# LiuZhu-CV/PAIF

Hardware: AMD Instinct MI355X
Metric: fused image-pairs/sec at 480x640 bs=8 per GPU (fusion-net forward) (higher is better)
Workload: dtype f16 (IEEE fp16 maps and conv weights, one fp16 MFMA per product, f32 accumulate; stems, guided filter and the last map fp32)

## Files before the change

### include/paif_hip.h

```cpp
#ifndef PAIF_HIP_H
#define PAIF_HIP_H

#include <stddef.h>
#include <stdint.h>

#ifdef __cplusplus
extern "C" {
#endif

#define PAIF_ABI_VERSION 1
#define PAIF_EINVAL (-1)
#define PAIF_ENOSUP (-2)

typedef void* paif_stream_t;

int paif_version(void);
const char* paif_last_error(void);
int paif_device_cus(void);


int paif_rgb2ycrcb_fwd(const float* rgb, float* ycc, int B, int H, int W, paif_stream_t stream);

int paif_ycrcb2rgb_fwd(const float* ycc, float* rgb, int B, int H, int W, paif_stream_t stream);

int paif_minmax_blocks(int B, int H, int W);
int paif_recompose_clamp_fwd(const float* fused, const float* ycc, float* rgb_out, float* minmax_partial,
                             int B, int H, int W, paif_stream_t stream);
int paif_fused_uint8_fwd(const float* rgb, const float* minmax_partial, int npartial, unsigned char* out, int B, int H, int W,
                         paif_stream_t stream);
int paif_minmax_normalize_fwd(const float* rgb, const float* minmax_partial, int npartial, float* out,
                              float* minmax_out, int B, int H, int W, paif_stream_t stream);


int paif_stem_fwd(const float* img, size_t img_bstride, const float* w, const float* prelu, float* feat, float* guide,
                  int B, int H, int W, paif_stream_t stream);
int paif_stem_fwd_twin(const float* img, size_t img_bstride, const float* w, const float* prelu, float* feat, float* feat_bf16,
                       float* guide, int B, int H, int W, paif_stream_t stream);
int paif_stem_fwd_twin_f16(const float* img, size_t img_bstride, const float* w, const float* prelu, float* feat, float* feat_f16,
                           float* guide, int B, int H, int W, paif_stream_t stream);
int paif_channel_residue_fwd(const float* x, float* guide, int B, int H, int W, paif_stream_t stream);

int paif_guided_filter_ab_fwd(const float* guide, const float* y, float* ab, float eps0, float eps1,
                              int B, int H, int W, paif_stream_t stream);
int paif_guided_filter_lf_fwd(const float* guide, const float* ab, float* lf, int B, int H, int W,
                              paif_stream_t stream);
int paif_guided_filter_taped_fits(int B, int H, int W);
int paif_guided_filter_taped_fwd(const float* guide, const float* y, float* mc, float* lf, float eps0, float eps1,
                                 float* workspace, int B, int H, int W, paif_stream_t stream);
size_t paif_guided_filter_fused_workspace_floats(int B, int H, int W);
int paif_guided_filter_fused_fwd(const float* guide, const float* y, float* lf, float eps0, float eps1, float* workspace,
                                 int B, int H, int W, paif_stream_t stream);
int paif_guided_filter_fused_fwd_bf16(const float* guide, const float* y, float* lf, float eps0, float eps1, float* workspace, int B,
                                      int H, int W, paif_stream_t stream);
int paif_guided_filter_fused_fwd_hf16(const float* guide, const float* y, float* hf, float eps0, float eps1, float* workspace, int B,
                                      int H, int W, paif_stream_t stream);

int paif_guided_filter_fused_fwd_hf16_y16(const float* guide, const float* y16, float* hf, float eps0, float eps1, float* workspace,
                                          int B, int H, int W, paif_stream_t stream);

typedef struct {
  const float* src[3];
  int nsrc;
  int cin;
  const float* wpk;
  int kh;
  int dil;
  int in_act;
  const float* in_prelu;
  const float* scale;
  const float* shift;
  int act;
  const float* prelu;
  float alpha;
  const float* res[3];
  float* out;
  int cout;
  float* pool_partial;
  int precision;
  float* aux_out;
  const float* in_aux;
  const float* in_scale;
  float in_alpha;
  const float* epi_aux;
  int epi_dact;
  int reverse_tiles;
  int storage;
  float* cpool;
} paif_conv_desc;
#define PAIF_ST_F32 0
#define PAIF_ST_BF16 1
#define PAIF_ST_F32_BF16 2
#define PAIF_ST_F16 3
#define PAIF_ST_F16_F32 4
#define PAIF_CONV_F32 0
#define PAIF_CONV_BF16X3 1
#define PAIF_CONV_BF16 2
#define PAIF_CONV_F16 4
#define PAIF_CONV_F16X2 5
#define PAIF_CONV_F16X3 6
#define PAIF_CONV_BF16X6 3

int paif_dwconv_fwd_bf16(const float* x, const float* w, float* out, int k, int dil, int in_relu, int B, int H, int W,
                         paif_stream_t stream);
int paif_channel_pool2_fwd_bf16(const float* ir, const float* vis, float* comp, int B, int H, int W, paif_stream_t stream);
int paif_spa_blend_fwd_bf16(const float* comp, const float* w, const float* ir, const float* vis, float* agg, int B, int H, int W,
                            paif_stream_t stream);
int paif_eca_finish_fwd_bf16(const float* o, const float* r, const float* pool_partial, const float* w1d, int k,
                             const float* prelu, float* gate, float* out, int B, int H, int W, paif_stream_t stream);
int paif_tail_fwd_bf16(const float* x, const float* w, const float* prelu, float* fused, int B, int H, int W, paif_stream_t stream);
int paif_add_fwd_bf16(const float* a, const float* b, float* out, size_t n, paif_stream_t stream);
int paif_cast_storage_fwd(const float* src, float* dst, size_t n, int mode, paif_stream_t stream);
int paif_dwconv_fwd_f16(const float* x, const float* w, float* out, int k, int dil, int in_relu, int B, int H, int W,
                        paif_stream_t stream);
int paif_channel_pool2_fwd_f16(const float* ir, const float* vis, float* comp, int B, int H, int W, paif_stream_t stream);
int paif_spa_blend_fwd_f16(const float* comp, const float* w, const float* ir, const float* vis, float* agg, int B, int H, int W,
                           paif_stream_t stream);
int paif_eca_finish_fwd_f16(const float* o, const float* r, const float* pool_partial, const float* w1d, int k,
                            const float* prelu, float* gate, float* out, int B, int H, int W, paif_stream_t stream);
int paif_tail_fwd_f16(const float* x, const float* w, const float* prelu, float* fused, int B, int H, int W, paif_stream_t stream);
int paif_eca_conv2_gated_fits(int B, int H, int W);
int paif_eca_conv2_gated_fwd_f16(const float* r, const float* wpk, const float* in_prelu, float* pool_partial, const float* w1d, int k,
                                 const float* prelu, float* gate, float* out, int B, int H, int W, paif_stream_t stream);
int paif_eca_conv2_staged_f16(const float* r, const float* wpk, const float* in_prelu, float* out, int B, int H, int W, paif_stream_t stream);
int paif_add_fwd_f16(const float* a, const float* b, float* out, size_t n, paif_stream_t stream);

int paif_conv2d_blocks(int B, int H, int W);
int paif_conv2d_fwd(const paif_conv_desc* d, int B, int H, int W, paif_stream_t stream);
int paif_conv2d_can_cpool(const paif_conv_desc* d, int B, int H, int W);
int paif_channel_pool1_fwd(const float* x, float* comp_off, int B, int H, int W, paif_stream_t stream);
int paif_channel_pool1_fwd_bf16(const float* x, float* comp_off, int B, int H, int W, paif_stream_t stream);
int paif_channel_pool1_fwd_f16(const float* x, float* comp_off, int B, int H, int W, paif_stream_t stream);
int paif_conv2d_is_persistent(const paif_conv_desc* d, int B, int H, int W);
int paif_conv2d_kernel_name(const paif_conv_desc* d, int B, int H, int W, char* buf, int buflen);
size_t paif_conv_wpk_floats(int nsrc, int cin, int kh);
int paif_pack_conv_weight(const float* w, float* wpk, int cout, int nsrc, int cin, int kh, paif_stream_t stream);
int paif_pack_conv_weight_bf16x3(const float* w, float* wpk, int cout, int nsrc, int kh, paif_stream_t stream);
int paif_pack_conv_weight_f16x2(const float* w, float* wpk, int cout, int nsrc, int kh, paif_stream_t stream);
int paif_pack_conv_weight_bf16x6(const float* w, float* wpk, int cout, int nsrc, int kh, paif_stream_t stream);
int paif_compose_dw_pw_weight(const float* dw, const float* pw, float* out, int cout, int cin, int kh, paif_stream_t stream);
int paif_compose_pw_conv_weight(const float* pw, const float* w, float* out, int cout, int cmid, int cin, int kh, paif_stream_t stream);

size_t paif_rdb_fused_wpk_floats(void);
int paif_rdb_fused_pack(const float* w1, const float* w2, const float* w3, float* wpk, int f16, paif_stream_t stream);
int paif_rdb_fused_fwd(const float* x, const float* wpk, const float* prelu, float alpha, const float* res0, const float* res1, float* out,
                       float* cpool, int f16, int reverse_tiles, int B, int H, int W, paif_stream_t stream);

int paif_stem_out_pack_floats(void);
int paif_stem_out_pack(const float* w1, const float* w2, float* wpk, paif_stream_t stream);
int paif_stem_out_fwd_bf16(const float* x, const float* wpk, const float* prelu, float* fused, int B, int H, int W, paif_stream_t stream);
int paif_stem_out_fwd_f32(const float* x, const float* wpk, const float* prelu, float* fused, int B, int H, int W, paif_stream_t stream);
int paif_stem_out_fwd_guard(const float* x, int f32in, const float* wpk, const float* prelu, float* fused, unsigned* flag, int B, int H, int W,
                            paif_stream_t stream);
int paif_pack_decomp1x1_weight_bf16x6(const float* w, float* wpk, paif_stream_t stream);
int paif_pack_decomp1x1_weight_bf16x3(const float* w, float* wpk, paif_stream_t stream);
int paif_pack_decomp1x1_hf_weight_f16x2(const float* w, float* wpk, paif_stream_t stream);
int paif_pack_decomp1x1_weight(const float* w, float* wpk, paif_stream_t stream);
int paif_bn_fold(const float* gamma, const float* beta, const float* mean, const float* var, float eps,
                 float* scale, float* shift, int C, paif_stream_t stream);

int paif_dwconv_fwd(const float* x, const float* w, float* out, int k, int dil, int in_relu,
                    int B, int H, int W, paif_stream_t stream);

int paif_channel_pool2_fwd(const float* ir, const float* vis, float* comp, int B, int H, int W, paif_stream_t stream);
int paif_spa_blend_fwd(const float* comp, const float* w, const float* ir, const float* vis, float* agg,
                       float* scale_out, int B, int H, int W, paif_stream_t stream);

int paif_eca_finish_fwd(const float* o, const float* r, const float* pool_partial, const float* w1d, int k,
                        const float* prelu, float* gate , float* out,
                        float* u_out ,
                        int B, int H, int W, paif_stream_t stream);

int paif_tail_fwd(const float* x, const float* w, const float* prelu, float* fused,
                  float* z_out ,
                  int B, int H, int W, paif_stream_t stream);

int paif_add_fwd(const float* a, const float* b, float* out, size_t n, paif_stream_t stream);



int paif_gemm_fwd(const float* A, int lda, const float* W, const float* scale, const float* shift, int act,
// ... 282 lines not shown
```

### paif_amd/_lib.py

```python
import ctypes
import os
from ctypes import POINTER, Structure, c_char_p, c_float, c_int, c_size_t, c_ulonglong, c_void_p

HERE = os.path.dirname(os.path.abspath(__file__))
LIB_PATH = os.environ.get("PAIF_LIB") or os.path.join(HERE, "lib", "libpaif_hip.so")

F = c_void_p


class ConvDesc(Structure):

    _fields_ = [
        ("src", F * 3), ("nsrc", c_int), ("cin", c_int), ("wpk", F), ("kh", c_int), ("dil", c_int),
        ("in_act", c_int), ("in_prelu", F), ("scale", F), ("shift", F), ("act", c_int), ("prelu", F),
        ("alpha", c_float), ("res", F * 3), ("out", F), ("cout", c_int), ("pool_partial", F),
        ("precision", c_int), ("aux_out", F), ("in_aux", F), ("in_scale", F), ("in_alpha", c_float), ("epi_aux", F),
        ("epi_dact", c_int), ("reverse_tiles", c_int), ("storage", c_int), ("cpool", F),
    ]


SIGNATURES = {
    "paif_version": (c_int, []),
    "paif_last_error": (c_char_p, []),
    "paif_device_cus": (c_int, []),
    "paif_rgb2ycrcb_fwd": (c_int, [F, F, c_int, c_int, c_int, F]),
    "paif_ycrcb2rgb_fwd": (c_int, [F, F, c_int, c_int, c_int, F]),
    "paif_minmax_blocks": (c_int, [c_int, c_int, c_int]),
    "paif_recompose_clamp_fwd": (c_int, [F, F, F, F, c_int, c_int, c_int, F]),
    "paif_fused_uint8_fwd": (c_int, [F, F, c_int, F, c_int, c_int, c_int, F]),
    "paif_minmax_normalize_fwd": (c_int, [F, F, c_int, F, F, c_int, c_int, c_int, F]),
    "paif_stem_fwd": (c_int, [F, c_size_t, F, F, F, F, c_int, c_int, c_int, F]),
    "paif_stem_fwd_twin": (c_int, [F, c_size_t, F, F, F, F, F, c_int, c_int, c_int, F]),
    "paif_stem_fwd_twin_f16": (c_int, [F, c_size_t, F, F, F, F, F, c_int, c_int, c_int, F]),
    "paif_channel_residue_fwd": (c_int, [F, F, c_int, c_int, c_int, F]),
    "paif_guided_filter_ab_fwd": (c_int, [F, F, F, c_float, c_float, c_int, c_int, c_int, F]),
    "paif_guided_filter_lf_fwd": (c_int, [F, F, F, c_int, c_int, c_int, F]),
    "paif_guided_filter_taped_fits": (c_int, [c_int, c_int, c_int]),
    "paif_guided_filter_taped_fwd": (c_int, [F, F, F, F, c_float, c_float, F, c_int, c_int, c_int, F]),
    "paif_guided_filter_fused_workspace_floats": (c_size_t, [c_int, c_int, c_int]),
    "paif_guided_filter_fused_fwd": (c_int, [F, F, F, c_float, c_float, F, c_int, c_int, c_int, F]),
    "paif_guided_filter_fused_fwd_bf16": (c_int, [F, F, F, c_float, c_float, F, c_int, c_int, c_int, F]),
    "paif_guided_filter_fused_fwd_hf16": (c_int, [F, F, F, c_float, c_float, F, c_int, c_int, c_int, F]),
    "paif_guided_filter_fused_fwd_hf16_y16": (c_int, [F, F, F, c_float, c_float, F, c_int, c_int, c_int, F]),
    "paif_conv2d_blocks": (c_int, [c_int, c_int, c_int]),
    "paif_conv2d_fwd": (c_int, [POINTER(ConvDesc), c_int, c_int, c_int, F]),
    "paif_conv2d_is_persistent": (c_int, [POINTER(ConvDesc), c_int, c_int, c_int]),
    "paif_conv2d_can_cpool": (c_int, [POINTER(ConvDesc), c_int, c_int, c_int]),
    "paif_rdb_fused_wpk_floats": (c_size_t, []),
    "paif_rdb_fused_pack": (c_int, [F, F, F, F, c_int, F]),
    "paif_rdb_fused_fwd": (c_int, [F, F, F, c_float, F, F, F, F, c_int, c_int, c_int, c_int, c_int, F]),
    "paif_channel_pool1_fwd": (c_int, [F, F, c_int, c_int, c_int, F]),
    "paif_channel_pool1_fwd_bf16": (c_int, [F, F, c_int, c_int, c_int, F]),
    "paif_channel_pool1_fwd_f16": (c_int, [F, F, c_int, c_int, c_int, F]),
    "paif_conv2d_kernel_name": (c_int, [POINTER(ConvDesc), c_int, c_int, c_int, c_char_p, c_int]),
    "paif_conv_wpk_floats": (c_size_t, [c_int, c_int, c_int]),
    "paif_pack_conv_weight": (c_int, [F, F, c_int, c_int, c_int, c_int, F]),
    "paif_pack_decomp1x1_weight": (c_int, [F, F, F]),
    "paif_pack_conv_weight_bf16x3": (c_int, [F, F, c_int, c_int, c_int, F]),
    "paif_pack_conv_weight_f16x2": (c_int, [F, F, c_int, c_int, c_int, F]),
    "paif_pack_conv_weight_bf16x6": (c_int, [F, F, c_int, c_int, c_int, F]),
    "paif_compose_dw_pw_weight": (c_int, [F, F, F, c_int, c_int, c_int, F]),
    "paif_compose_pw_conv_weight": (c_int, [F, F, F, c_int, c_int, c_int, c_int, F]),
    "paif_stem_out_pack_floats": (c_int, []),
    "paif_stem_out_pack": (c_int, [F, F, F, F]),
    "paif_stem_out_fwd_bf16": (c_int, [F, F, F, F, c_int, c_int, c_int, F]),
    "paif_stem_out_fwd_f32": (c_int, [F, F, F, F, c_int, c_int, c_int, F]),
    "paif_stem_out_fwd_guard": (c_int, [F, c_int, F, F, F, F, c_int, c_int, c_int, F]),
    "paif_pack_decomp1x1_weight_bf16x3": (c_int, [F, F, F]),
    "paif_pack_decomp1x1_hf_weight_f16x2": (c_int, [F, F, F]),
    "paif_pack_decomp1x1_weight_bf16x6": (c_int, [F, F, F]),
    "paif_bn_fold": (c_int, [F, F, F, F, c_float, F, F, c_int, F]),
    "paif_dwconv_fwd": (c_int, [F, F, F, c_int, c_int, c_int, c_int, c_int, c_int, F]),
    "paif_channel_pool2_fwd": (c_int, [F, F, F, c_int, c_int, c_int, F]),
    "paif_spa_blend_fwd": (c_int, [F, F, F, F, F, F, c_int, c_int, c_int, F]),
    "paif_eca_finish_fwd": (c_int, [F, F, F, F, c_int, F, F, F, F, c_int, c_int, c_int, F]),
    "paif_tail_fwd": (c_int, [F, F, F, F, F, c_int, c_int, c_int, F]),
    "paif_add_fwd": (c_int, [F, F, F, c_size_t, F]),
    "paif_gemm_fwd": (c_int, [F, c_int, F, F, F, c_int, F, c_int, F, c_int, c_int, c_int, c_int, c_int, F]),
    "paif_gemm_splitk_plan": (c_int, [c_int, c_int, c_int]),
    "paif_gemm_conv_fwd": (c_int, [F, c_int, c_int, c_int, c_int, c_int, c_int, c_int, F, F, F, c_int, F, c_int, F, c_int, c_int, c_int, c_int, F, F]),
    "paif_gemm_col2im_fwd": (c_int, [F, c_int, F, F, c_int, c_int, c_int, c_int, c_int, c_int, c_int, F]),
    "paif_timing_event_create": (c_int, [POINTER(c_void_p)]),
    "paif_timing_event_record": (c_int, [c_void_p, F]),
    "paif_timing_event_elapsed_ms": (c_int, [c_void_p, c_void_p, POINTER(c_float)]),
    "paif_timing_event_destroy": (c_int, [c_void_p]),
    "paif_gemm2_plan": (c_int, [c_int, c_int, c_int, c_int]),
    "paif_gemm2_packed_bytes": (c_size_t, [c_int, c_int, c_int]),
    "paif_gemm2_pack_weight": (c_int, [F, F, c_int, c_int, c_int, F]),
    "paif_gemm2_fwd": (c_int, [F, c_int, F, F, F, c_int, F, c_int, F, c_int, c_int, c_int, c_int, c_int, c_int, F]),
    "paif_conv2d_wgrad_workspace_floats": (c_size_t, [c_int, c_int, c_int, c_int]),
    "paif_conv2d_wgrad": (c_int, [POINTER(c_void_p), c_int, F, F, F, F, c_int, c_float, c_int, c_int, F, F, c_int, c_int, c_int, c_int, c_int, F]),
    "paif_gemm_wgrad_splits": (c_int, [c_int, c_int, c_int]),
    "paif_gemm_wgrad": (c_int, [F, c_int, F, c_int, F, F, c_int, c_int, c_int, c_int, F, c_int, F]),
    "paif_gemm_wgrad_p": (c_int, [F, c_int, F, c_int, F, F, c_int, c_int, c_int, c_int, F, c_int, c_int, c_float, F]),
    "paif_layernorm_wgrad_blocks": (c_int, [c_int]),
    "paif_layernorm_wgrad": (c_int, [F, F, F, F, F, c_int, c_int, c_float, c_int, F]),
    "paif_channel_affine_nchw_fwd": (c_int, [F, F, F, F, c_int, c_int, c_int, c_int, F]),
    "paif_image_loss_blocks": (c_int, []),
# ... 175 lines not shown
```

### paif_amd/core/model_fusion_auto.py

```python
import torch
import torch.nn as nn

from .. import ops
from ..operations_m import OPS, BasicConv, Conv2dParams, PReLUParams, _HipOp, _PackCache, grad_anchor


def RGB2YCrCb(input_im):
    ops.require_no_grad(input_im)
    return ops.rgb2ycrcb(input_im)


def YCrCb2RGB(input_im):
    ops.require_no_grad(input_im)
    return ops.ycrcb2rgb(input_im)


class MixedOp(nn.Module):

    def __init__(self, C, primitive):
        super().__init__()
        self._ops = nn.ModuleList()
        kernel = 3
        dilation = 1
        if primitive.find('attention') != -1:
            name = primitive.split('_')[0]
            kernel = int(primitive.split('_')[1])
        else:
            name = primitive.split('_')[0]
            kernel = int(primitive.split('_')[1])
            dilation = int(primitive.split('_')[2])
        self._op = OPS[name](C, kernel, dilation, False)

    def forward(self, x):
        return self._op(x)

    def forward_nhwc(self, x, res=(), tape=None, out_f32=False, cpool=None):
        if out_f32 and getattr(self._op, "takes_out_f32", False):
            return self._op.forward_nhwc(x, res, tape, out_f32=True)
        if cpool is not None and tape is None:
            if getattr(self._op, "takes_cpool", False):
                return self._op.forward_nhwc(x, res, tape, cpool=cpool)
            y = self._op.forward_nhwc(x, res, tape)
            ops.channel_pool1(y, *cpool)
            return y
        return self._op.forward_nhwc(x, res, tape)

    def backward_nhwc(self, g, t, wgrad=False, res=()):
        if res:
            return self._op.backward_nhwc(g, t, wgrad, res=res)
        return self._op.backward_nhwc(g, t, wgrad)

    @property
    def bwd_takes_res(self):
        return getattr(self._op, "bwd_takes_res", False)


class Cell_Chain(_HipOp):

    _tape_is_list = True

    def __init__(self, C, type, concat):
        super().__init__()
        op_names, indices = zip(*type)
        self._compile(C, op_names, indices, concat)

    def _compile(self, C, op_names, indices, concat):
        assert len(op_names) == len(indices)
        self._steps = len(op_names)
        self._concat = concat
        self.multiplier = len(concat)
        self._ops = nn.ModuleList()
        for name, index in zip(op_names, indices):
            self._ops += [MixedOp(C, name)]
        self._indices = indices

    def forward_nhwc(self, inp, res=(), tape=None, out_f32=False, cpool=None):
        s1 = inp
        for i in range(self._steps):
            last = i == self._steps - 1
            s1 = self._ops[i].forward_nhwc(s1, ((inp,) + tuple(res)) if last else (), tape, out_f32=out_f32 and last,
                                           cpool=cpool if last else None)
        return s1

    def backward_nhwc(self, g, tape, wgrad=False):
        d = g
        for i in range(self._steps - 1, 0, -1):
            d = self._ops[i].backward_nhwc(d, tape[i], wgrad)
        if self._ops[0].bwd_takes_res:
            return self._ops[0].backward_nhwc(d, tape[0], wgrad, res=(g,))
        return ops.add(self._ops[0].backward_nhwc(d, tape[0], wgrad), g)


class Cell_Decom(nn.Module):

    def __init__(self, C, types, concat):
        super().__init__()
        self._C = C
        self.radiux = [4]
        self.eps_list = [0.001, 0.0001]
        self._ops_1 = nn.ModuleList()
        self._ops_2 = nn.ModuleList()
        self.conv1x1_lf = Conv2dParams(C * 4, C, kernel_size=1, bias=True)
        self.conv1x1_hf = Conv2dParams(C * 4, C, kernel_size=1, bias=True)
        self._steps = len(concat)
        self.relu = PReLUParams()
        self.chain = Cell_Chain(C, types[0], concat)
        self.chain2 = Cell_Chain(C, types[1], concat)
        self._packs = _PackCache()
        if C != 32:
            raise NotImplementedError("the HIP kernels are built for C = 32 (the only width either entry script uses)")

    def get_residue(self, tensor):
        return ops.to_nchw_view(ops.channel_residue(ops.to_nhwc(tensor)).unsqueeze(-1))

    def decomposition_nhwc(self, x, guide=None, want_ab=False, out_bf16=False):
        if guide is None:
            guide = ops.channel_residue(x)
        return ops.guided_filter_pair(guide, x, tuple(self.eps_list), want_ab=want_ab, out_bf16=out_bf16)

    @staticmethod
    def _cat_lf_hf(x, lf):
        lf_cat, hf_cat = ops.decomp_cat(x, lf)
        return ops.to_nchw_view(lf_cat), ops.to_nchw_view(hf_cat)

    def decomposition(self, x, C=None):
        ops.require_no_grad(x)
        xn = ops.to_nhwc(x)
        return self._cat_lf_hf(xn, self.decomposition_nhwc(xn))

    def forward_nhwc(self, fir, fvis, g_ir=None, g_vis=None, tape=None, feats=None, comp=None):
        if g_ir is None:
            g_ir = ops.channel_residue(fir)
        if g_vis is None:
            g_vis = ops.channel_residue(fvis)
        lf16 = tape is None and feats is None and ops._ACT_BF16[0]
        if tape is None:
            lf_ir = self.decomposition_nhwc(fir, g_ir, out_bf16=lf16)
            lf_vis = self.decomposition_nhwc(fvis, g_vis, out_bf16=lf16)
        else:
            lf_ir, ab_ir = self.decomposition_nhwc(fir, g_ir, want_ab=True)
            lf_vis, ab_vis = self.decomposition_nhwc(fvis, g_vis, want_ab=True)
        pack1, pn = (ops.pack_decomp1x1_hf_weight, "_hf16") if lf16 is torch.float16 else (ops.pack_decomp1x1_weight, "")
        w_lf = self._packs.get("lf" + pn, [self.conv1x1_lf.weight], lambda: pack1(self.conv1x1_lf.weight))
        w_hf = self._packs.get("hf" + pn, [self.conv1x1_hf.weight], lambda: pack1(self.conv1x1_hf.weight))
        if feats is not None:
            feats.update(lf_ir=lf_ir, lf_vis=lf_vis, g_ir=g_ir, g_vis=g_vis)
        x_ir, x_vis = (ops.cast_storage(fir, True), ops.cast_storage(fvis, True)) if lf16 else (fir, fvis)
        lf = ops.conv2d([x_ir, lf_ir[0], lf_ir[1]], w_lf, 1, 1, shift=self.conv1x1_lf.bias)
        hf = ops.conv2d([x_vis, lf_vis[0], lf_vis[1]], w_hf, 1, 1, shift=self.conv1x1_hf.bias)
        t1 = None if tape is None else []
        t2 = None if tape is None else []
        cp = comp if tape is None else None
        ir_feature = self.chain.forward_nhwc(lf, (fir,), t1, cpool=None if cp is None else (cp, 0))
        vis_feature = self.chain2.forward_nhwc(hf, (fvis,), t2, cpool=None if cp is None else (cp, 2))
        if tape is not None:
            tape.update(fir=fir, fvis=fvis, g_ir=g_ir, g_vis=g_vis, ab_ir=ab_ir, ab_vis=ab_vis, chain=t1, chain2=t2)
            if ops.taping_wgrad():
                tape.update(lf_ir=lf_ir, lf_vis=lf_vis)
        return ir_feature, vis_feature

    def branch_nhwc(self, f, g, which, comp=None):
        lf16 = ops._ACT_BF16[0]
        lf = self.decomposition_nhwc(f, g, out_bf16=lf16)
        conv = self.conv1x1_lf if which == 0 else self.conv1x1_hf
        pack1, pn = (ops.pack_decomp1x1_hf_weight, "_hf16") if lf16 is torch.float16 else (ops.pack_decomp1x1_weight, "")
        w = self._packs.get(("lf" if which == 0 else "hf") + pn, [conv.weight], lambda: pack1(conv.weight))
        x = ops.cast_storage(f, True) if lf16 else f
        y = ops.conv2d([x, lf[0], lf[1]], w, 1, 1, shift=conv.bias)
        return (self.chain if which == 0 else self.chain2).forward_nhwc(y, (f,), None, cpool=None if comp is None else (comp, 2 * which))

    def _stream_backward(self, d_feat, chain, chain_tape, conv, name, feat, guide, ab, lf=None):
# ... 91 lines not shown


class Network_Fusion_Searched(nn.Module):

    def __init__(self, C, criterion, genotype_feature, steps=4, multiplier=3):
        super().__init__()
        self._C = C
        self._criterion = criterion
        self._steps = steps
        self._multiplier = multiplier
        self._genotype = genotype_feature
        self.stem_1 = nn.Sequential(Conv2dParams(1, C, 3, padding=1, bias=False), PReLUParams())
        self.stem_2 = nn.Sequential(Conv2dParams(1, C, 3, padding=1, bias=False), PReLUParams())
        self.stem_out = nn.Sequential(
            Conv2dParams(C, C // 2, 3, padding=1, bias=False),
            Conv2dParams(C // 2, 1, 3, padding=1, bias=False),
            PReLUParams(),
        )
        self.tanh = nn.Tanh()
        self.spa = spatial_attn_layer_M()
        self.decompation = self._decom_cls(C, [self._genotype.normal_1, self._genotype.normal_2], self._genotype.normal_1_concat)
        self.chain = Cell_Chain(C, self._genotype.normal_3, self._genotype.normal_1_concat)
        self._packs = _PackCache()

    _decom_cls = Cell_Decom

    def forward(self, ir, vis, inter=None):
        wg = ops.want_param_grads(self)
        if torch.is_grad_enabled() and (ir.requires_grad or vis.requires_grad or wg):
            return _FusionFn.apply(ir, vis, self, wg, grad_anchor(ir.device))
        want_feats = inter is not None and bool(inter.get("want_decomposition"))
        with torch.no_grad(), ops.bf16_activations(enable=not self.training and not want_feats):
            return self.forward_impl(ir, vis, inter=inter)

    def forward_impl(self, ir, vis, inter=None, tape=None):
        vis = vis[:, 0:1, :, :]
        ir = ir[:, 0:1, :, :]
        if tape is None and inter is None and ir.is_cuda and ops.CONFIG.get("two_stream", False):
            main = torch.cuda.current_stream()
            side = self.__dict__.get("_side_stream")
            if side is None or side.device != ir.device:
                side = self.__dict__["_side_stream"] = torch.cuda.Stream(device=ir.device)
            comp = self._new_comp(ir)
            side.wait_stream(main)
            with torch.cuda.stream(side):
                fvis, g_vis = ops.stem(vis, self.stem_2[0].weight, self.stem_2[1].weight)
                vis_feature = self.decompation.branch_nhwc(fvis, g_vis, 1, comp)
            fir, g_ir = ops.stem(ir, self.stem_1[0].weight, self.stem_1[1].weight)
            ir_feature = self.decompation.branch_nhwc(fir, g_ir, 0, comp)
            main.wait_stream(side)
            if not torch.cuda.is_current_stream_capturing():
                vis_feature.record_stream(main)
            del fvis, g_vis
            agg = self.spa.blend_nhwc(ir_feature, vis_feature, comp=comp)
            return self._tail_nhwc(self.chain.forward_nhwc(agg, (), None, out_f32=self._last_f32()))
        fir, g_ir = ops.stem(ir, self.stem_1[0].weight, self.stem_1[1].weight)
        fvis, g_vis = ops.stem(vis, self.stem_2[0].weight, self.stem_2[1].weight)
        t_dec = None if tape is None else {}
        feats = {} if (inter is not None and inter.get("want_decomposition")) else None
        comp = self._new_comp(ir) if tape is None else None
        ir_feature, vis_feature = self.decompation.forward_nhwc(fir, fvis, g_ir, g_vis, t_dec, feats, comp=comp)
        if feats is not None:
            inter.update(feats)
        t_chain = None if tape is None else []
        if tape is None:
            agg = self.spa.blend_nhwc(ir_feature, vis_feature, comp=comp)
        elif ops.taping_wgrad():
            agg, scale, comp = self.spa.blend_nhwc(ir_feature, vis_feature, want_scale=True, want_comp=True)
        else:
            agg, scale = self.spa.blend_nhwc(ir_feature, vis_feature, want_scale=True)
        feature2 = self.chain.forward_nhwc(agg, (), t_chain, out_f32=tape is None and self._last_f32())
        if tape is None:
            out = self._tail_nhwc(feature2)
        else:
            w0 = self._packs.get("so0", [self.stem_out[0].weight], lambda: ops.pack_conv_weight(self.stem_out[0].weight, 1, 32, 3))
            t16 = ops.conv2d([feature2], w0, 3, 1, cout=16)
            out, z = ops.tail(t16, self.stem_out[1].weight, self.stem_out[2].weight, save=True)
            tape.update(dec=t_dec, chain=t_chain, ir_feature=ir_feature, vis_feature=vis_feature, scale=scale, fused=out, z=z)
            if ops.taping_wgrad():
                tape.update(comp=comp, feature2=feature2, t16=t16, img_ir=ir, img_vis=vis)
        if inter is not None:
            inter.update(fir=fir, fvis=fvis, ir_feature=ir_feature, vis_feature=vis_feature, agg=agg, feature2=feature2)
        return out

    @staticmethod
    def _new_comp(img):
        if not ops.CONFIG.get("cpool_fused", True):
            return None
        B, _, H, W = img.shape
        return torch.empty((B, H, W, 4), device=img.device, dtype=torch.float32)

    @staticmethod
    def _last_f32():
        return ops._ACT_BF16[0] is torch.float16 and ops.CONFIG.get("f16_last_f32", True)

    def _tail_nhwc(self, feature2):
        so = self.stem_out
        if feature2.dtype == torch.float16:
            feature2 = ops.cast_storage(feature2, torch.float32)
        if feature2.dtype == torch.float32:
            fused_on = ops.CONFIG.get("stem_out_fused_f32", True) and ops.CONFIG["conv_precision"] == "bf16x3"
        else:
            fused_on = ops.CONFIG.get("stem_out_fused", True)
        if feature2.shape[1] >= 3 and feature2.shape[2] >= 3 and fused_on:
            wso = self._packs.get("so_fused", [so[0].weight, so[1].weight], lambda: ops.stem_out_pack(so[0].weight, so[1].weight))
            return ops.stem_out_fused(feature2, wso, so[2].weight)
        if ops._ACT_BF16[0] is torch.float16:
            ops.f16_guard_flag(feature2.device).bitwise_or_((~torch.isfinite(feature2).all()).to(torch.int32))
        if feature2.dtype == torch.float32:
            prec = ops.CONFIG["conv_precision"]
            w0 = self._packs.get("so0_" + prec, [so[0].weight], lambda: ops.pack_conv_weight(so[0].weight, 1, 32, 3, precision=prec))
        else:
            w0 = self._packs.get("so0", [so[0].weight], lambda: ops.pack_conv_weight(so[0].weight, 1, 32, 3))
        return ops.tail(ops.conv2d([feature2], w0, 3, 1, cout=16), so[1].weight, so[2].weight)

    def backward_impl(self, d_fused, tape, wgrad=False):
        from ..operations_m import check_positive_slope
        for prm, what in ((self.stem_1[1].weight, "stem_1"), (self.stem_2[1].weight, "stem_2")):
            check_positive_slope(prm, what)
        so = self.stem_out
        if wgrad:
            dz = ops.tail_dz(d_fused, tape["fused"], tape["z"], so[2].weight, ops.grad_of(so[2].weight))
            gw = ops.grad_of(so[1].weight)
            if gw is not None:
                ops.corr1_wgrad(dz, tape["t16"], 3, gw)
        d_t16 = ops.tail_bwd(d_fused, tape["fused"], tape["z"], so[1].weight, so[2].weight)
        if wgrad:
            gw = ops.grad_of(so[0].weight)
            if gw is not None:
                ops.conv2d_wgrad([tape["feature2"]], ops.pad_channels(d_t16, 32), 3, 1, out=gw, cout=16)
        w0t = self._packs.get("so0T", [so[0].weight], lambda: ops.pack_conv_dgrad_weight(so[0].weight, 0, 32))
        d_feat2 = ops.conv2d([d_t16], w0t, 3, 1, cin=16, cout=32)
        d_agg = self.chain.backward_nhwc(d_feat2, tape["chain"], wgrad)
        d_irf, d_visf = self.spa.blend_backward_nhwc(d_agg, tape["ir_feature"], tape["vis_feature"], tape["scale"],
                                                     tape["comp"] if wgrad else None)
        d_fir, d_fvis = self.decompation.backward_nhwc(d_irf, d_visf, tape["dec"], wgrad)
# ... 356 lines not shown
```

### paif_amd/csrc/conv_dma.h

```cpp
#pragma once
#include <hip/hip_runtime.h>

namespace paif_conv_dma {

struct Args {
  const void* src[3];
  const void* res[3];
  const void* wpk;
  const float* scale;
  const float* shift;
  const float* prelu;
  void* out;
  float alpha;
  int nsrc, nres, act, kh;
  int cout;
  int B, H, W, reverse;
  float* cpool;
  int f16;
  int dil;
  int in_relu;
  int out_f32;
};

enum Form { NONE, TILE, ONE_BY_ONE, ROWS };
Form classify(const Args& a);
bool can_cpool(const Args& a);
int launch(const Args& a, hipStream_t st);

}
```

### paif_amd/csrc/conv_dma.hip

```cpp
#include <stdint.h>
#include <stdlib.h>

#include <type_traits>

#include "conv_dma.h"
#include "conv_rows.h"

namespace paif_conv_dma {
namespace {

using namespace paif_rows;
constexpr int TW = 32, TH = 8;
#ifndef CD_PF
#define CD_PF 4
#endif
#ifndef CD_ST_AUX
#define CD_ST_AUX 2
#endif
#ifndef CD_EPI_SWAP
#define CD_EPI_SWAP 1
#endif
#ifndef CD_EPI_LINES
#define CD_EPI_LINES 1
#endif
#ifndef CD_EXP
#define CD_EXP 0
#endif
constexpr int PARK_WAVE = 2 * 32 * 32 * 4;
template <int DIL>
struct Geo {
  static constexpr int TWH = TW + 2 * DIL, THH = TH + 2 * DIL;
  static constexpr int NPIX = TWH * THH;
  static constexpr int DPW = (NPIX * 4 + 255) / 256;
  static constexpr int SLOT = 4 * DPW * 1024;
  static constexpr int PF = DIL == 1 ? CD_PF : 3;
  static constexpr int NSLOT = PF + 1;
  static constexpr int ROWB = TWH * 64;
  static constexpr int PARK_OFF = NSLOT * SLOT;
  static constexpr int lds_bytes(bool parked) { return PARK_OFF + (parked ? 4 * PARK_WAVE : 0); }
  static_assert(lds_bytes(true) <= 160 * 1024, "ring + transposition buffers exceed LDS");
  static_assert(4 * DPW * 64 >= NPIX * 4, "DMA instructions do not cover the halo tile");
  static __device__ __forceinline__ int base_row(int w) { return DIL == 1 ? 2 * w : (w >> 1) * 4 + (w & 1); }
};
constexpr int NSTORE = 4;
constexpr int VMCAP = 63;

#define CD_VMWAIT(n) ROWS_VMWAIT((n) > VMCAP ? VMCAP : (n))

template <int NSRC, int NRES, int PF, int DPW>
struct Sched {
  static constexpr int RL = 4 * NRES;
  static constexpr int smod(int x) { return ((x % NSRC) + NSRC) % NSRC; }
  static constexpr int R_STAGE = smod(1 - PF);
  static constexpr int D = (R_STAGE + PF - 1 - NSRC) / NSRC;
  static constexpr int U = D + (R_STAGE == 0 ? 2 : 1);
  static_assert(PF >= 2 && D >= 0 && U <= 4, "prefetch distance out of the range the tile loop lists");
  static constexpr int n1 = DPW * (PF - 1);
};

template <int NSRC, int NRES, int F, bool CP = false, int DIL = 1, int IA = 0>
__global__ __launch_bounds__(256, 1) void conv3x3_h16_dma(Args a, int ntiles, int tilesX, int tilesY) {
  typedef Geo<DIL> G;
  constexpr int TWH = G::TWH, NPIX = G::NPIX, DPW = G::DPW, SLOT = G::SLOT, PF = G::PF, NSLOT = G::NSLOT, ROWB = G::ROWB, PARK_OFF = G::PARK_OFF;
  typedef Sched<NSRC, NRES, PF, DPW> SC;
  constexpr bool SW = CD_EPI_SWAP && !CP && !(NRES == 3 && (NSRC == 3 || DIL == 2));
  constexpr int U = SW ? (SC::U + 1) & ~1 : SC::U, D = SC::D;
  constexpr int NACC = SW ? 2 : 1;
  __shared__ __attribute__((aligned(16))) unsigned char smem[G::lds_bytes(!SW)];
  asm volatile("" ::"v"((unsigned)(uintptr_t)(__attribute__((address_space(3))) unsigned char*)smem) : "memory");

  const int tid = threadIdx.x, l = tid & 63;
  const int w = __builtin_amdgcn_readfirstlane(tid >> 6);
  const int p = l & 31, hh = l >> 5;
  const int wb = G::base_row(w);

  const int xcd = blockIdx.x & 7, wg = blockIdx.x >> 3, nwg = gridDim.x >> 3;
  const int tpx = (ntiles + 7) >> 3;
  const int t_beg = xcd * tpx, t_end = min(ntiles, t_beg + tpx);
  const int cnt = t_beg + wg < t_end ? (t_end - t_beg - wg + nwg - 1) / nwg : 0;
  if (cnt == 0) return;
  const int H = a.H, W = a.W;
  auto pack_tile = [&](int k) -> unsigned {
    const int pos = wg + min(k, cnt - 1) * nwg;
    int t = a.reverse ? t_end - 1 - pos : t_beg + pos;
    const int tx = t % tilesX;
    t /= tilesX;
    const int ty = t % tilesY;
    return ((unsigned)(t / tilesY) << 22) | ((unsigned)ty << 11) | (unsigned)tx;
  };
  const unsigned tab0 = pack_tile(l), tab1 = pack_tile(l + 64);
  auto tile_of = [&](int k, int& b, int& y0, int& x0) -> bool {
    const bool ok = k >= 0 && k < cnt;
    const int kk = ok ? k : 0;
    const unsigned lo = __builtin_amdgcn_readlane(tab0, kk & 63), hi = __builtin_amdgcn_readlane(tab1, kk & 63);
    const unsigned pk = kk < 64 ? lo : hi;
    b = pk >> 22; y0 = ((pk >> 11) & 2047) * TH; x0 = (pk & 2047) * TW;
    return ok;
  };

  const int map_bytes = a.B * H * W * 64;
  __amdgpu_buffer_rsrc_t rs_src[NSRC];
#pragma unroll
  for (int s = 0; s < NSRC; ++s) rs_src[s] = __builtin_amdgcn_make_buffer_rsrc(const_cast<void*>(a.src[s]), 0, map_bytes, RSRC_W3);
  __amdgpu_buffer_rsrc_t rs_res[NRES > 0 ? NRES : 1];
#pragma unroll
  for (int r = 0; r < NRES; ++r) rs_res[r] = __builtin_amdgcn_make_buffer_rsrc(const_cast<void*>(a.res[r]), 0, map_bytes, RSRC_W3);
  const int opitch = a.cout * 2;
  const __amdgpu_buffer_rsrc_t rs_out = __builtin_amdgcn_make_buffer_rsrc(a.out, 0, a.B * H * W * opitch, RSRC_W3);
  const __amdgpu_buffer_rsrc_t rs_null = __builtin_amdgcn_make_buffer_rsrc(a.out, 0, 0, RSRC_W3);
  const __amdgpu_buffer_rsrc_t rs_cp = __builtin_amdgcn_make_buffer_rsrc(CP ? (void*)a.cpool : a.out, 0, CP ? a.B * H * W * 16 - 8 : 0, RSRC_W3);

  u32x4 bw[NSRC][9][2];
  {
    const __amdgpu_buffer_rsrc_t rs_w = __builtin_amdgcn_make_buffer_rsrc(const_cast<void*>(a.wpk), 0, NSRC * 9 * 2 * 2 * 1024, RSRC_W3);
#pragma unroll
    for (int s = 0; s < NSRC; ++s)
#pragma unroll
      for (int tap = 0; tap < 9; ++tap)
#pragma unroll
        for (int ks = 0; ks < 2; ++ks)
          bw[s][tap][ks] = __builtin_amdgcn_raw_buffer_load_b128(rs_w, (unsigned)l * 16u, (((s * 9 + tap) * 2 + ks) * 2) * 1024, 0);
  }
  constexpr int NEC = SW ? 16 : 8;
  float esc[NEC], esh[NEC];
#pragma unroll
  for (int j = 0; j < NEC; ++j) {
    const int c = SW ? ROWS_ACC_CHANNEL(j, hh) : 8 * (l & 3) + j;
    esc[j] = ((a.scale && c < a.cout) ? a.scale[c] : 1.f) * a.alpha;
    esh[j] = ((a.shift && c < a.cout) ? a.shift[c] : 0.f) * a.alpha;
// ... 578 lines not shown
    cur ^= 1;
  };
  auto drain = [&](auto aptag) {
    if constexpr (!SW) {
#pragma unroll
      for (int it = 0; it < 4; ++it) {
        ROWS_RD128(t[it][0], a_pr, it * 2048);
        ROWS_RD128(t[it][1], a_pr, it * 2048 + 16);
      }
      asm volatile("s_waitcnt lgkmcnt(0)"
                   : "+v"(t[0][0]), "+v"(t[0][1]), "+v"(t[1][0]), "+v"(t[1][1]), "+v"(t[2][0]), "+v"(t[2][1]), "+v"(t[3][0]), "+v"(t[3][1])::"memory");
    }
    int pb, py0, px0;
    const bool pok = tile_of(cnt - 1, pb, py0, px0);
#define CD_M(m) epi(std::integral_constant<int, m>{}, aptag, pok, pb, py0, px0);
    CD_M(0) CD_M(1) CD_M(2) CD_M(3) CD_M(4) CD_M(5) CD_M(6) CD_M(7) CD_M(8) CD_M(9) CD_M(10) CD_M(11)
    CD_M(12) CD_M(13) CD_M(14) CD_M(15) CD_M(16) CD_M(17) CD_M(18) CD_M(19) CD_M(20) CD_M(21) CD_M(22) CD_M(23)
    CD_M(24) CD_M(25) CD_M(26) CD_M(27) CD_M(28) CD_M(29) CD_M(30) CD_M(31) CD_M(32) CD_M(33) CD_M(34) CD_M(35)
#undef CD_M
  };
  typedef std::integral_constant<int, 0> T0;
  typedef std::integral_constant<int, 1> T1;
  if constexpr (SW) {
    for (int k = 0;; k += 2) {
      tile(T0{}, k);
      if (k + 1 >= cnt) { drain(T0{}); break; }
      tile(T1{}, k + 1);
      if (k + 2 >= cnt) { drain(T1{}); break; }
    }
  } else {
    for (int k = 0; k < cnt; ++k) tile(T0{}, k);
    drain(T0{});
  }
  CD_VMWAIT(0);
}

int launch_7(const Args& a, hipStream_t st) {
  const int tilesX = (a.W + TW - 1) / TW, tilesY = (a.H + TH - 1) / TH;
  if (a.f16) hipLaunchKernelGGL(conv7x7_h16_dma<2>, dim3(256), dim3(256), 0, st, a, a.B * tilesX * tilesY, tilesX, tilesY);
  else hipLaunchKernelGGL(conv7x7_h16_dma<1>, dim3(256), dim3(256), 0, st, a, a.B * tilesX * tilesY, tilesX, tilesY);
  hipError_t e = hipGetLastError();
  if (e != hipSuccess) {
    paif::set_error("conv2d(bf16 dma 7x7): launch failed: %s", hipGetErrorString(e));
    return (int)e;
  }
  return 0;
}

template <int NSRC, int NRES>
int launch_n(const Args& a, hipStream_t st) {
  const int tilesX = (a.W + TW - 1) / TW, tilesY = (a.H + TH - 1) / TH;
  if (a.cpool) {
    if constexpr (NSRC == 3 && (NRES == 1 || NRES == 3)) {
      if (a.f16) hipLaunchKernelGGL((conv3x3_h16_dma<NSRC, NRES, 2, true>), dim3(256), dim3(256), 0, st, a, a.B * tilesX * tilesY, tilesX, tilesY);
      else hipLaunchKernelGGL((conv3x3_h16_dma<NSRC, NRES, 1, true>), dim3(256), dim3(256), 0, st, a, a.B * tilesX * tilesY, tilesX, tilesY);
    } else {
      paif::set_error("conv2d(dma): the fused ChannelPool is built for 3 sources with 1 or 3 residual maps");
      return PAIF_ENOSUP;
    }
  } else if (a.f16) hipLaunchKernelGGL((conv3x3_h16_dma<NSRC, NRES, 2>), dim3(256), dim3(256), 0, st, a, a.B * tilesX * tilesY, tilesX, tilesY);
  else hipLaunchKernelGGL((conv3x3_h16_dma<NSRC, NRES, 1>), dim3(256), dim3(256), 0, st, a, a.B * tilesX * tilesY, tilesX, tilesY);
  hipError_t e = hipGetLastError();
  if (e != hipSuccess) {
    paif::set_error("conv2d(h16 dma): launch failed: %s", hipGetErrorString(e));
    return (int)e;
  }
  return 0;
}

template <int NRES, bool CP>
int launch_d2(const Args& a, hipStream_t st) {
  const int tilesX = (a.W + TW - 1) / TW, tilesY = (a.H + TH - 1) / TH;
  if (a.f16) hipLaunchKernelGGL((conv3x3_h16_dma<1, NRES, 2, CP, 2, 2>), dim3(256), dim3(256), 0, st, a, a.B * tilesX * tilesY, tilesX, tilesY);
  else hipLaunchKernelGGL((conv3x3_h16_dma<1, NRES, 1, CP, 2, 2>), dim3(256), dim3(256), 0, st, a, a.B * tilesX * tilesY, tilesX, tilesY);
  hipError_t e = hipGetLastError();
  if (e != hipSuccess) {
    paif::set_error("conv2d(h16 dma, dilation 2): launch failed: %s", hipGetErrorString(e));
    return (int)e;
  }
  return 0;
}

}

bool is_1x1(const Args& a);
int launch_1x1(const Args& a, hipStream_t st);
bool is_rows(const Args& a);
int launch_rows(const Args& a, hipStream_t st);

static bool is_tile(const Args& a) {
  static const bool on = [] {
    const char* e = getenv("PAIF_CONV_DMA");
    return !(e && e[0] == '0');
  }();
  static const bool on_d2 = [] {
    const char* e = getenv("PAIF_CONV_DMA_D2");
    return !(e && e[0] == '0');
  }();
  if (!on || a.out_f32 || !(a.alpha > 0.f)) return false;
  bool built;
  if (a.dil == 2)
    built = on_d2 && a.kh == 3 && a.cout == 32 && a.in_relu && a.nsrc == 1 && (a.nres == 1 || a.nres == 3);
  else if (a.in_relu || a.dil != 1)
    built = false;
  else if (a.kh == 3 && a.cout == 32)
    built = a.nsrc >= 1 && a.nsrc <= 3 && a.nres >= 0 && a.nres <= (a.nsrc == 1 ? 1 : 3);
  else
    built = ((a.kh == 3 && a.cout == 16) || (a.kh == 7 && a.cout == 32)) && a.nsrc == 1 && a.nres == 0;
  const long long tiles = (long long)a.B * ((a.H + TH - 1) / TH) * ((a.W + TW - 1) / TW);
  return built && tiles >= 1024 && tiles <= 128 * 256 && a.B < 1024 && a.H < 2048 * TH && a.W < 2048 * TW &&
         (long long)a.B * a.H * a.W * 64 < (1ll << 31);
}

Form classify(const Args& a) {
  if (is_1x1(a)) return ONE_BY_ONE;
  if (is_rows(a)) return ROWS;
  return is_tile(a) ? TILE : NONE;
}

bool can_cpool(const Args& a) {
  return a.kh == 3 && a.cout == 32 && (a.nres == 1 || a.nres == 3) && ((a.dil == 1 && a.nsrc == 3) || (a.dil == 2 && a.nsrc == 1));
}

int launch(const Args& a, hipStream_t st) {
  switch (classify(a)) {
    case ONE_BY_ONE: return launch_1x1(a, st);
    case ROWS: return launch_rows(a, st);
    case TILE: break;
    default:
      paif::set_error("conv2d(h16 dma): no LDS-DMA kernel is built for this descriptor and shape");
      return PAIF_ENOSUP;
  }
  if (a.cpool && !can_cpool(a)) {
    paif::set_error("conv2d(dma): no fused ChannelPool for this form");
    return PAIF_ENOSUP;
  }
  if (a.kh == 7) return launch_7(a, st);
  if (a.dil == 2) {
    if (a.nres == 1) return a.cpool ? launch_d2<1, true>(a, st) : launch_d2<1, false>(a, st);
    return a.cpool ? launch_d2<3, true>(a, st) : launch_d2<3, false>(a, st);
  }
  switch (a.nsrc * 10 + a.nres) {
    case 10: return launch_n<1, 0>(a, st);
    case 11: return launch_n<1, 1>(a, st);
    case 20: return launch_n<2, 0>(a, st);
    case 21: return launch_n<2, 1>(a, st);
    case 22: return launch_n<2, 2>(a, st);
    case 23: return launch_n<2, 3>(a, st);
    case 30: return launch_n<3, 0>(a, st);
    case 31: return launch_n<3, 1>(a, st);
    case 32: return launch_n<3, 2>(a, st);
    case 33: return launch_n<3, 3>(a, st);
    default: break;
  }
  paif::set_error("conv2d(bf16 dma): %d sources / %d residual maps not built", a.nsrc, a.nres);
  return PAIF_ENOSUP;
}

}
```

### paif_amd/csrc/conv_dma_1x1.hip

```cpp
#include <stdint.h>
#include <stdlib.h>

#include <type_traits>

#include "conv_dma.h"
#include "conv_rows.h"

namespace paif_conv_dma {
namespace {

using namespace paif_rows;

constexpr int TP = 64;
constexpr int SLOT = TP * 64;
constexpr int DPS = SLOT / 1024;
constexpr int NSLOT = 4, PF = NSLOT - 1;
constexpr int WAVE_LDS = NSLOT * SLOT + PARK;
constexpr int WAVES = 4;
constexpr int LDS_BYTES = WAVES * WAVE_LDS;
constexpr int GRID = 512;
static_assert(2 * LDS_BYTES <= 160 * 1024, "two workgroups per CU do not fit LDS");
static_assert(PF == 3, "a stage's DMA target is the same source of the next tile: PF must equal the source count");

#ifndef C1_LD_AUX
#define C1_LD_AUX 2
#endif
#ifndef C1_ST_AUX
#define C1_ST_AUX 0
#endif

template <int F>
__global__ __launch_bounds__(WAVES * 64, 2) void conv_h16_dma_1x1(Args a, int ntiles) {
  __shared__ __attribute__((aligned(16))) unsigned char smem[LDS_BYTES];
  asm volatile("" ::"v"((unsigned)(uintptr_t)(__attribute__((address_space(3))) unsigned char*)smem) : "memory");

  const int tid = threadIdx.x, l = tid & 63;
  const int w = __builtin_amdgcn_readfirstlane(tid >> 6);
  const int p = l & 31, hh = l >> 5;
  const int gw = blockIdx.x * WAVES + w, nw = gridDim.x * WAVES;
  if (gw >= ntiles) return;
  const int cnt = (ntiles - gw + nw - 1) / nw;

  const unsigned map_bytes = (unsigned)(a.B * a.H * a.W) * 64u;
  __amdgpu_buffer_rsrc_t rs_src[3];
#pragma unroll
  for (int s = 0; s < 3; ++s) rs_src[s] = __builtin_amdgcn_make_buffer_rsrc(const_cast<void*>(a.src[s]), 0, (int)map_bytes, RSRC_W3);
  const __amdgpu_buffer_rsrc_t rs_out = __builtin_amdgcn_make_buffer_rsrc(a.out, 0, (int)map_bytes, RSRC_W3);

  u32x4 bw[3][2];
  {
    const __amdgpu_buffer_rsrc_t rs_w = __builtin_amdgcn_make_buffer_rsrc(const_cast<void*>(a.wpk), 0, 3 * 2 * 2 * 1024, RSRC_W3);
#pragma unroll
    for (int s = 0; s < 3; ++s)
#pragma unroll
      for (int ks = 0; ks < 2; ++ks) bw[s][ks] = __builtin_amdgcn_raw_buffer_load_b128(rs_w, (unsigned)l * 16u, ((s * 2 + ks) * 2) * 1024, 0);
  }
  float esc[8], esh[8];
#pragma unroll
  for (int j = 0; j < 8; ++j) {
    const int c = 8 * (l & 3) + j;
    esc[j] = a.scale ? a.scale[c] : 1.f;
    esh[j] = a.shift ? a.shift[c] : 0.f;
  }
  const int act = a.act;
  const float slope = act == 1 ? *a.prelu : 0.f;
  const float alpha = a.alpha;

  const unsigned d_rel = ROWS_SWIZZLED(l >> 2, l & 3);
  const unsigned lds_w = (unsigned)(w * WAVE_LDS);
  unsigned a_rd[2];
#pragma unroll
  for (int ks = 0; ks < 2; ++ks) a_rd[ks] = lds_w + ROWS_SWIZZLED(p, 2 * ks + hh);
  const unsigned a_pw = ROWS_PARK_WR_ADDR(lds_w + NSLOT * SLOT, p, hh);
  const unsigned a_pr = ROWS_PARK_RD_ADDR(lds_w + NSLOT * SLOT, l);
  const unsigned e_lane = (unsigned)l * 16u;

  auto tile_byte = [&](int k) -> unsigned { return (unsigned)(gw + k * nw) * (unsigned)SLOT; };
  unsigned d_voff[DPS];
  auto target = [&](int k) {
    const unsigned tb = tile_byte(k);
#pragma unroll
    for (int i = 0; i < DPS; ++i) {
      const unsigned off = tb + d_rel + 1024u * i;
      d_voff[i] = (k < cnt && off < map_bytes) ? off : OOB;
    }
  };
  int cur = 0;
  auto issue = [&](auto stag, int slot) {
    constexpr int S = decltype(stag)::value;
#pragma unroll
    for (int i = 0; i < DPS; ++i) dma16<C1_LD_AUX>(rs_src[S], d_voff[i], lds_w + (unsigned)(slot * SLOT + i * 1024));
  };
// ... 37 lines not shown
      park_transpose(acc[sg], a_pw, a_pr, t);
#pragma unroll
      for (int it = 0; it < 2; ++it) {
        float ev[8];
#pragma unroll
        for (int j = 0; j < 8; ++j) {
          float v = __builtin_fmaf(__uint_as_float(t[it][j >> 2][j & 3]), esc[j], esh[j]);
          if (act == 1) v = paif::prelu_f(v, slope);
          else if (act == 2) v = fmaxf(v, 0.f);
          ev[j] = v * alpha;
        }
        const uint2 o0 = paif::f32_to_h4<F>(make_float4(ev[0], ev[1], ev[2], ev[3]));
        const uint2 o1 = paif::f32_to_h4<F>(make_float4(ev[4], ev[5], ev[6], ev[7]));
        u32x4 od = {o0.x, o0.y, o1.x, o1.y};
        const unsigned off = tb + (unsigned)(sg * 2048 + it * 1024) + e_lane;
        __builtin_amdgcn_raw_buffer_store_b128(od, rs_out, off < map_bytes ? off : OOB, 0, C1_ST_AUX);
        asm volatile("s_nop 2" : "+v"(od));
      }
    }
  };

  typedef std::integral_constant<int, 0> S0;
  typedef std::integral_constant<int, 1> S1;
  typedef std::integral_constant<int, 2> S2;
  target(0);
  issue(S0{}, 0);
  issue(S1{}, 1);
  issue(S2{}, 2);
  for (int k = 0; k < cnt; ++k) {
    target(k + 1);
    stage(S0{});
    stage(S1{});
    stage(S2{});
    finish(k);
  }
  ROWS_VMWAIT(0);
}

}

bool is_1x1(const Args& a) {
  static const bool on = [] {
    const char* e = getenv("PAIF_CONV_DMA1X1");
    const char* d = getenv("PAIF_CONV_DMA");
    return !(e && e[0] == '0') && !(d && d[0] == '0');
  }();
  return on && a.kh == 1 && a.dil == 1 && a.cout == 32 && !a.in_relu && !a.out_f32 && a.nsrc == 3 && a.nres == 0 &&
         (long long)a.B * a.H * a.W * 64 < (1ll << 31);
}

int launch_1x1(const Args& a, hipStream_t st) {
  const long long px = (long long)a.B * a.H * a.W;
  const int ntiles = (int)((px + TP - 1) / TP);
  if (a.f16) hipLaunchKernelGGL(conv_h16_dma_1x1<2>, dim3(GRID), dim3(WAVES * 64), 0, st, a, ntiles);
  else hipLaunchKernelGGL(conv_h16_dma_1x1<1>, dim3(GRID), dim3(WAVES * 64), 0, st, a, ntiles);
  hipError_t e = hipGetLastError();
  if (e != hipSuccess) {
    paif::set_error("conv2d(h16 dma 1x1): launch failed: %s", hipGetErrorString(e));
    return (int)e;
  }
  return 0;
}

}
```

### paif_amd/csrc/conv_mfma.hip

```cpp
#include <stdlib.h>

#include "conv_dma.h"
#include "paif_common.h"
#include <type_traits>

#ifndef PAIF_UB_HOOKS
#define PAIF_UB_HOOKS 3
#endif
#ifndef PAIF_UB
#define PAIF_UB 11
#endif

namespace {

typedef float f32x16 __attribute__((ext_vector_type(16)));

#ifndef PAIF_TH
#define PAIF_TH 8
#endif
constexpr int TH = PAIF_TH;
constexpr int TW = 32;
constexpr int NTHREADS = 256;
constexpr int SEGS_PER_WAVE = TH / 4;

// ... 1767 lines not shown
    if constexpr (KH == 1) switch (p.st) { PAIF_ST_CASE(2) PAIF_ST_CASE(5) default: break; }
    switch (p.st) { PAIF_ST_CASE(12) PAIF_ST_CASE(14) default: break; }
    if constexpr (KH == 1) switch (p.st) { PAIF_ST_CASE(9) default: break; }
    if constexpr (KH == 3 && DIL == 2) switch (p.st) { PAIF_ST_CASE(15) default: break; }
  }
#undef PAIF_ST_CASE
  paif::set_error("conv2d: storage %d is not built for the %dx%d dilation-%d kernel", a.st, KH, KH, DIL);
  return PAIF_ENOSUP;
}

template <ConvFamily F, int KH, int DIL>
int launch_k(const ConvPlan& p, const ConvArgs& a, hipStream_t st) {
  if constexpr (F == FAM_F32) return p.hooks ? launch_h<KH, DIL, 32, true>(a, st) : launch_h<KH, DIL, 32, false>(a, st);
  else if constexpr (F == FAM_BF16X6) return p.hooks ? launch_bf16x3_h<KH, DIL, true, 0, 3>(a, st) : launch_bf16x3_h<KH, DIL, false, 0, 3>(a, st);
  else if constexpr (F == FAM_F16X3) return p.hooks ? launch_bf16x3_h<KH, DIL, true, 0, 2, 1>(a, st) : launch_bf16x3_h<KH, DIL, false, 0, 2, 1>(a, st);
  else return launch_split<KH, DIL>(p, a, st);
}

template <ConvFamily F>
int launch_key(const ConvPlan& p, const ConvArgs& a, hipStream_t st) {
  constexpr bool WIDE_D2 = F == FAM_SPLIT || F == FAM_F32;
  switch (p.kh * 100 + p.dil * 10 + (p.cin == 32 ? 0 : 1)) {
    case 110: return launch_k<F, 1, 1>(p, a, st);
    case 310: return launch_k<F, 3, 1>(p, a, st);
    case 320: return launch_k<F, 3, 2>(p, a, st);
    case 510: return launch_k<F, 5, 1>(p, a, st);
    case 520:
      if constexpr (WIDE_D2) return launch_k<F, 5, 2>(p, a, st);
      break;
    case 710: return launch_k<F, 7, 1>(p, a, st);
    case 720:
      if constexpr (WIDE_D2) return launch_k<F, 7, 2>(p, a, st);
      break;
    case 311:
      if constexpr (F == FAM_F32) return p.hooks ? launch_h<3, 1, 16, true>(a, st) : launch_h<3, 1, 16, false>(a, st);
      break;
    default: break;
  }
  return not_built(p);
}

static int plan_launch(const ConvPlan& p, const ConvArgs& a, hipStream_t st) {
  switch (p.family) {
    case FAM_F16X3: return launch_key<FAM_F16X3>(p, a, st);
    case FAM_BF16X6: return launch_key<FAM_BF16X6>(p, a, st);
    case FAM_SPLIT:
      if (p.variant == CV_DMA || p.variant == CV_ROWS) return paif_conv_dma::launch(dma_args(a, p.kh, p.dil), st);
      return launch_key<FAM_SPLIT>(p, a, st);
    case FAM_F32: break;
  }
  return launch_key<FAM_F32>(p, a, st);
}

}

extern "C" {

int paif_conv2d_blocks(int B, int H, int W) { return B * ((H + TH - 1) / TH) * ((W + TW - 1) / TW); }

size_t paif_conv_wpk_floats(int nsrc, int cin, int kh) { return (size_t)nsrc * kh * kh * (cin / 8) * 256; }

int paif_conv2d_is_persistent(const paif_conv_desc* d, int B, int H, int W) {
  if (!d || B <= 0 || H <= 0 || W <= 0) return 0;
  return plan_conv(conv_args(d, B, H, W), d).variant == CV_WS ? 1 : 0;
}

int paif_conv2d_can_cpool(const paif_conv_desc* d, int B, int H, int W) {
  if (!d || B <= 0 || H <= 0 || W <= 0) return 0;
  return plan_conv(conv_args(d, B, H, W), d).can_cpool ? 1 : 0;
}

int paif_conv2d_kernel_name(const paif_conv_desc* d, int B, int H, int W, char* buf, int buflen) {
  PAIF_REQUIRE(d && buf && buflen > 0 && B > 0 && H > 0 && W > 0, PAIF_EINVAL, "conv2d_kernel_name: bad arguments");
  const ConvArgs a = conv_args(d, B, H, W);
  plan_name(plan_conv(a, d), a, buf, buflen);
  return 0;
}

int paif_conv2d_fwd(const paif_conv_desc* d, int B, int H, int W, paif_stream_t stream) {
  PAIF_REQUIRE(d && d->out && d->wpk, PAIF_EINVAL, "conv2d: null descriptor/out/wpk");
  PAIF_REQUIRE(d->nsrc >= 1 && d->nsrc <= 3, PAIF_EINVAL, "conv2d: nsrc=%d", d->nsrc);
  for (int s = 0; s < d->nsrc; ++s) PAIF_REQUIRE(d->src[s], PAIF_EINVAL, "conv2d: src[%d] null", s);
  PAIF_REQUIRE(d->cout == 32 || d->cout == 16, PAIF_ENOSUP, "conv2d: cout=%d", d->cout);
  PAIF_REQUIRE(B > 0 && H > 0 && W > 0, PAIF_EINVAL, "conv2d: empty shape %dx%dx%d", B, H, W);
  PAIF_REQUIRE(d->in_act != 1 || d->in_prelu, PAIF_EINVAL, "conv2d: in_act=PReLU without slope");
  PAIF_REQUIRE(d->act != 1 || d->prelu, PAIF_EINVAL, "conv2d: act=PReLU without slope");
  PAIF_REQUIRE(d->in_act >= 0 && d->in_act <= 5, PAIF_EINVAL, "conv2d: in_act=%d", d->in_act);
  PAIF_REQUIRE(!(d->in_act == 3 || d->in_act == 4) || (d->in_aux && d->nsrc == 1), PAIF_EINVAL,
               "conv2d: in_act=%d needs in_aux and a single source", d->in_act);
  PAIF_REQUIRE(d->in_act != 3 || d->in_prelu, PAIF_EINVAL, "conv2d: in_act=3 without slope");
  PAIF_REQUIRE(d->epi_dact >= 0 && d->epi_dact <= 2 && (!d->epi_dact || d->epi_aux), PAIF_EINVAL, "conv2d: epi_dact=%d", d->epi_dact);
  PAIF_REQUIRE(d->epi_dact != 1 || d->prelu, PAIF_EINVAL, "conv2d: epi_dact=PReLU without slope");
  PAIF_REQUIRE(d->storage >= 0 && d->storage <= 4, PAIF_EINVAL, "conv2d: storage=%d", d->storage);
  const bool st_bf = d->storage == PAIF_ST_BF16 || d->storage == PAIF_ST_F32_BF16, st_hf = d->storage == PAIF_ST_F16 || d->storage == PAIF_ST_F16_F32;
  PAIF_REQUIRE(!st_bf || ((d->precision == PAIF_CONV_BF16X3 || d->precision == PAIF_CONV_BF16) && d->cin == 32), PAIF_ENOSUP,
               "conv2d: bf16 storage needs the split-bf16 kernels (cin 32)");
  PAIF_REQUIRE(!st_hf || ((d->precision == PAIF_CONV_F16 || d->precision == PAIF_CONV_F16X2) && d->cin == 32), PAIF_ENOSUP,
               "conv2d: fp16 storage takes precision F16 / F16X2 (cin 32)");
  PAIF_REQUIRE(d->precision != PAIF_CONV_BF16 || st_bf, PAIF_ENOSUP, "conv2d: precision bf16 is built for bf16-stored maps only");
  PAIF_REQUIRE((d->precision != PAIF_CONV_F16 && d->precision != PAIF_CONV_F16X2) || st_hf, PAIF_ENOSUP,
               "conv2d: precision fp16 is built for fp16-stored maps only");
  PAIF_REQUIRE(d->storage != PAIF_ST_F16_F32 || d->precision == PAIF_CONV_F16, PAIF_ENOSUP, "conv2d: fp16 in / fp32 out takes plain fp16 weights");
  PAIF_REQUIRE(!d->cpool || paif_conv2d_can_cpool(d, B, H, W), PAIF_ENOSUP, "conv2d: no fused ChannelPool for this descriptor (paif_conv2d_can_cpool)");
  PAIF_REQUIRE(d->cin == 32 || d->cin == 16, PAIF_ENOSUP, "conv2d: cin=%d", d->cin);
  PAIF_REQUIRE(d->precision == PAIF_CONV_F32 || d->precision == PAIF_CONV_BF16X3 || d->precision == PAIF_CONV_BF16 ||
                   d->precision == PAIF_CONV_BF16X6 || d->precision == PAIF_CONV_F16 || d->precision == PAIF_CONV_F16X2 ||
                   d->precision == PAIF_CONV_F16X3, PAIF_EINVAL,
               "conv2d: precision=%d", d->precision);
  PAIF_REQUIRE((d->precision != PAIF_CONV_BF16X6 && d->precision != PAIF_CONV_F16X3) || d->cin == 32, PAIF_ENOSUP, "conv2d: bf16x6 / f16x3 need 32-channel sources");
  const ConvArgs a = conv_args(d, B, H, W);
  return plan_launch(plan_conv(a, d), a, paif::as_stream(stream));
}

int paif_pack_conv_weight_bf16x3(const float* w, float* wpk, int cout, int nsrc, int kh, paif_stream_t stream) {
  PAIF_REQUIRE(w && wpk, PAIF_EINVAL, "pack_conv_weight_bf16x3: null pointer");
  PAIF_REQUIRE(cout >= 1 && cout <= 32 && nsrc >= 1 && nsrc <= 3 && kh >= 1 && kh <= 7, PAIF_ENOSUP,
               "pack_conv_weight_bf16x3: cout=%d nsrc=%d kh=%d", cout, nsrc, kh);
  const int total = nsrc * kh * kh * 2048;
  hipLaunchKernelGGL(pack_weight_bf16x3_kernel, dim3((total + 255) / 256), dim3(256), 0, paif::as_stream(stream), w,
                     reinterpret_cast<unsigned short*>(wpk), cout, nsrc, kh);
  PAIF_LAUNCH_CHECK("pack_conv_weight_bf16x3");
  return 0;
}

int paif_pack_conv_weight_f16x2(const float* w, float* wpk, int cout, int nsrc, int kh, paif_stream_t stream) {
  PAIF_REQUIRE(w && wpk, PAIF_EINVAL, "pack_conv_weight_f16x2: null pointer");
  PAIF_REQUIRE(cout >= 1 && cout <= 32 && nsrc >= 1 && nsrc <= 3 && kh >= 1 && kh <= 7, PAIF_ENOSUP,
               "pack_conv_weight_f16x2: cout=%d nsrc=%d kh=%d", cout, nsrc, kh);
  const int total = nsrc * kh * kh * 2048;
  hipLaunchKernelGGL(pack_weight_f16x2_kernel, dim3((total + 255) / 256), dim3(256), 0, paif::as_stream(stream), w,
                     reinterpret_cast<unsigned short*>(wpk), cout, nsrc, kh);
  PAIF_LAUNCH_CHECK("pack_conv_weight_f16x2");
  return 0;
}

int paif_pack_decomp1x1_hf_weight_f16x2(const float* w, float* wpk, paif_stream_t stream) {
  PAIF_REQUIRE(w && wpk, PAIF_EINVAL, "pack_decomp1x1_hf_weight_f16x2: null pointer");
  hipLaunchKernelGGL(pack_decomp1x1_hf_f16x2_kernel, dim3(24), dim3(256), 0, paif::as_stream(stream), w,
                     reinterpret_cast<unsigned short*>(wpk));
  PAIF_LAUNCH_CHECK("pack_decomp1x1_hf_weight_f16x2");
  return 0;
}

int paif_pack_conv_weight_bf16x6(const float* w, float* wpk, int cout, int nsrc, int kh, paif_stream_t stream) {
  PAIF_REQUIRE(w && wpk, PAIF_EINVAL, "pack_conv_weight_bf16x6: null pointer");
  PAIF_REQUIRE(cout >= 1 && cout <= 32 && nsrc >= 1 && nsrc <= 3 && kh >= 1 && kh <= 7, PAIF_ENOSUP,
               "pack_conv_weight_bf16x6: cout=%d nsrc=%d kh=%d", cout, nsrc, kh);
  const int total = nsrc * kh * kh * 3072;
  hipLaunchKernelGGL(pack_weight_bf16x6_kernel, dim3((total + 255) / 256), dim3(256), 0, paif::as_stream(stream), w,
                     reinterpret_cast<unsigned short*>(wpk), cout, nsrc, kh);
  PAIF_LAUNCH_CHECK("pack_conv_weight_bf16x6");
  return 0;
}

int paif_compose_dw_pw_weight(const float* dw, const float* pw, float* out, int cout, int cin, int kh, paif_stream_t stream) {
  PAIF_REQUIRE(dw && pw && out && cout >= 1 && cin >= 1 && kh >= 1 && kh <= 7, PAIF_EINVAL, "compose_dw_pw_weight: bad arguments");
  const int total = cout * cin * kh * kh;
  hipLaunchKernelGGL(compose_dw_pw_kernel, dim3((total + 255) / 256), dim3(256), 0, paif::as_stream(stream), dw, pw, out, cout, cin, kh * kh);
  PAIF_LAUNCH_CHECK("compose_dw_pw_weight");
  return 0;
}

int paif_compose_pw_conv_weight(const float* pw, const float* w, float* out, int cout, int cmid, int cin, int kh, paif_stream_t stream) {
  PAIF_REQUIRE(pw && w && out && cout >= 1 && cmid >= 1 && cin >= 1 && kh >= 1 && kh <= 7, PAIF_EINVAL, "compose_pw_conv_weight: bad arguments");
// ... 51 lines not shown
```

### paif_amd/csrc/fusion_kernels.hip

```cpp
#include <stdarg.h>

#include "conv_eca_rows.h"
#include "paif_common.h"

namespace paif {
static thread_local char g_err[256] = "";
void set_error(const char* fmt, ...) {
  va_list ap;
  va_start(ap, fmt);
  vsnprintf(g_err, sizeof(g_err), fmt, ap);
  va_end(ap);
}
}

namespace {

constexpr int MAXGRID = 256 * 8;

inline int grid_for(size_t work_items, int per_block) {
  size_t g = (work_items + per_block - 1) / per_block;
  if (g > (size_t)MAXGRID) g = MAXGRID;
  if (g < 1) g = 1;
  return (int)g;
}

__global__ void rgb2ycrcb_kernel(const float* __restrict__ rgb, float* __restrict__ ycc, int B, size_t HW) {
  const size_t total = (size_t)B * HW;
  for (size_t i = (size_t)blockIdx.x * blockDim.x + threadIdx.x; i < total; i += (size_t)gridDim.x * blockDim.x) {
    const size_t b = i / HW, px = i - b * HW;
    const float* s = rgb + b * 3 * HW + px;
    const float R = s[0], G = s[HW], Bl = s[2 * HW];
    const float Y = __fadd_rn(__fadd_rn(__fmul_rn(0.299f, R), __fmul_rn(0.587f, G)), __fmul_rn(0.114f, Bl));
    const float Cr = __fadd_rn(__fmul_rn(__fsub_rn(R, Y), 0.713f), 0.5f);
    const float Cb = __fadd_rn(__fmul_rn(__fsub_rn(Bl, Y), 0.564f), 0.5f);
    float* d = ycc + b * 3 * HW + px;
    d[0] = Y; d[HW] = Cr; d[2 * HW] = Cb;
  }
}

__global__ void ycrcb2rgb_kernel(const float* __restrict__ ycc, float* __restrict__ rgb, int B, size_t HW) {
  const size_t total = (size_t)B * HW;
  for (size_t i = (size_t)blockIdx.x * blockDim.x + threadIdx.x; i < total; i += (size_t)gridDim.x * blockDim.x) {
    const size_t b = i / HW, px = i - b * HW;
    const float* s = ycc + b * 3 * HW + px;
    const float y0 = __fadd_rn(s[0], 0.0f);
    const float cr = __fadd_rn(s[HW], -0.5f);
    const float cb = __fadd_rn(s[2 * HW], -0.5f);
    float* d = rgb + b * 3 * HW + px;
    d[0] = fmaf(cb, 0.0f, fmaf(cr, 1.403f, y0 * 1.0f));
    d[HW] = fmaf(cb, -0.344f, fmaf(cr, -0.714f, y0 * 1.0f));
    d[2 * HW] = fmaf(cb, 1.773f, fmaf(cr, 0.0f, y0 * 1.0f));
  }
}

constexpr int STEM_CHUNK = 128;
#ifndef PAIF_STEM_GRID
#define PAIF_STEM_GRID 4096
#endif
constexpr int STEM_GRID = PAIF_STEM_GRID;
__global__ __launch_bounds__(256) void stem_kernel(const float* __restrict__ img, const float* __restrict__ w,
                                                   const float* __restrict__ prelu, float* __restrict__ feat,
                                                   float* __restrict__ guide, int B, int H, int W,
                                                   size_t img_bstride, int chunks, unsigned short* __restrict__ feat16, int twin_f16) {
  const int q = threadIdx.x & 7;
  float wr[4][9];
#pragma unroll
  for (int c = 0; c < 4; ++c)
#pragma unroll
    for (int k = 0; k < 9; ++k) wr[c][k] = w[(4 * q + c) * 9 + k];
  const float slope = *prelu;
  __shared__ float patch[2][3][STEM_CHUNK + 2];
  const int nitems = B * H * chunks;
  int par = 0;
  for (int item = blockIdx.x; item < nitems; item += gridDim.x, par ^= 1) {
  const int chunk = item % chunks;
  const int row = item / chunks;
  const int y = row % H, b = row / H;
  const float* base = img + (size_t)b * img_bstride;
  for (int i = threadIdx.x; i < 3 * (STEM_CHUNK + 2); i += 256) {
    const int r = i / (STEM_CHUNK + 2), c = i - r * (STEM_CHUNK + 2);
    const int yy = y + r - 1, xx = chunk * STEM_CHUNK + c - 1;
    const bool ok = yy >= 0 && yy < H && xx >= 0 && xx < W;
    const float v = base[(size_t)min(max(yy, 0), H - 1) * W + min(max(xx, 0), W - 1)];
    patch[par][r][c] = ok ? v : 0.f;
  }
  __syncthreads();
  float* frow = feat ? feat + (size_t)row * W * 32 : nullptr;
  unsigned short* frow16 = feat16 ? feat16 + (size_t)row * W * 32 : nullptr;
  float* grow = guide ? guide + (size_t)row * W : nullptr;
#pragma unroll
  for (int it = 0; it < STEM_CHUNK / 32; ++it) {
    const int xi = it * 32 + (threadIdx.x >> 3);
    const int x = chunk * STEM_CHUNK + xi;
    float v[9];
#pragma unroll
    for (int r = 0; r < 3; ++r)
#pragma unroll
      for (int c = 0; c < 3; ++c) v[r * 3 + c] = patch[par][r][xi + c];
    float o[4];
#pragma unroll
    for (int c = 0; c < 4; ++c) {
      float s = 0.f;
#pragma unroll
      for (int k = 0; k < 9; ++k) s = fmaf(v[k], wr[c][k], s);
      o[c] = paif::prelu_f(s, slope);
    }
    if (frow && x < W) paif::store_nt(frow + (size_t)x * 32 + q * 4, make_float4(o[0], o[1], o[2], o[3]));
    if (frow16 && x < W)
      *reinterpret_cast<uint2*>(frow16 + (size_t)x * 32 + q * 4) = twin_f16 ? paif::f32_to_f16x4(make_float4(o[0], o[1], o[2], o[3]))
                                                                             : paif::f32_to_bf16x4(make_float4(o[0], o[1], o[2], o[3]));
    if (grow) {
      float mx = fmaxf(fmaxf(o[0], o[1]), fmaxf(o[2], o[3]));
      float mn = fminf(fminf(o[0], o[1]), fminf(o[2], o[3]));
#pragma unroll
      for (int m = 1; m < 8; m <<= 1) {
        mx = fmaxf(mx, __shfl_xor(mx, m));
        mn = fminf(mn, __shfl_xor(mn, m));
      }
      if (q == 0 && x < W) grow[x] = mx - mn;
    }
  }
  }
}

template <int K, int DIL, int BF = 0>
__global__ __launch_bounds__(256) void dwconv_kernel(const float* __restrict__ x, const float* __restrict__ w,
                                                     float* __restrict__ out, int in_relu, int B, int H, int W) {
  constexpr int P = DIL * (K - 1) / 2;
  const int q = threadIdx.x & 7;
  float wr[4][K * K];
#pragma unroll
  for (int c = 0; c < 4; ++c)
#pragma unroll
    for (int k = 0; k < K * K; ++k) wr[c][k] = w[(4 * q + c) * K * K + k];
  const size_t npix = (size_t)B * H * W;
  for (size_t pix = (size_t)blockIdx.x * 32 + (threadIdx.x >> 3); pix < npix; pix += (size_t)gridDim.x * 32) {
    const int xx0 = (int)(pix % W);
    const size_t rowid = pix / W;
    const int yy0 = (int)(rowid % H);
    const size_t base = (rowid - yy0) * W * 32 + q * 4;
    float4 acc = make_float4(0.f, 0.f, 0.f, 0.f);
    constexpr int ROWS_IN_FLIGHT = K == 3 ? 3 : 1;
// ... 492 lines not shown
  }
}

}

extern "C" {

int paif_fused_uint8_fwd(const float* rgb, const float* minmax_partial, int npartial, unsigned char* out, int B, int H, int W,
                         paif_stream_t stream) {
  PAIF_REQUIRE(rgb && minmax_partial && out && npartial > 0 && B > 0 && H > 0 && W > 0, PAIF_EINVAL, "fused_uint8: bad arguments");
  const size_t HW = (size_t)H * W;
  hipLaunchKernelGGL(fused_uint8_kernel, dim3(grid_for((size_t)B * 3 * HW, 256)), dim3(256), 0, paif::as_stream(stream), rgb,
                     minmax_partial, npartial, out, B, HW);
  PAIF_LAUNCH_CHECK("fused_uint8");
  return 0;
}

int paif_version(void) { return PAIF_ABI_VERSION; }
const char* paif_last_error(void) { return paif::g_err; }

int paif_device_cus(void) {
  int dev = 0;
  hipDeviceProp_t prop;
  if (hipGetDevice(&dev) != hipSuccess || hipGetDeviceProperties(&prop, dev) != hipSuccess) {
    paif::set_error("device_cus: no HIP device");
    return PAIF_EINVAL;
  }
  return prop.multiProcessorCount;
}

int paif_rgb2ycrcb_fwd(const float* rgb, float* ycc, int B, int H, int W, paif_stream_t stream) {
  PAIF_REQUIRE(rgb && ycc && B > 0 && H > 0 && W > 0, PAIF_EINVAL, "rgb2ycrcb: bad arguments");
  const size_t HW = (size_t)H * W;
  hipLaunchKernelGGL(rgb2ycrcb_kernel, dim3(grid_for(B * HW, 256)), dim3(256), 0, paif::as_stream(stream), rgb, ycc, B, HW);
  PAIF_LAUNCH_CHECK("rgb2ycrcb");
  return 0;
}

int paif_ycrcb2rgb_fwd(const float* ycc, float* rgb, int B, int H, int W, paif_stream_t stream) {
  PAIF_REQUIRE(ycc && rgb && B > 0 && H > 0 && W > 0, PAIF_EINVAL, "ycrcb2rgb: bad arguments");
  const size_t HW = (size_t)H * W;
  hipLaunchKernelGGL(ycrcb2rgb_kernel, dim3(grid_for(B * HW, 256)), dim3(256), 0, paif::as_stream(stream), ycc, rgb, B, HW);
  PAIF_LAUNCH_CHECK("ycrcb2rgb");
  return 0;
}

static int stem_launch(const float* img, size_t img_bstride, const float* w, const float* prelu, float* feat, float* guide,
                       unsigned short* feat16, int twin_f16, int B, int H, int W, paif_stream_t stream) {
  PAIF_REQUIRE(img && w && prelu && (feat || feat16) && B > 0 && H > 0 && W > 0, PAIF_EINVAL, "stem: bad arguments");
  PAIF_REQUIRE(img_bstride >= (size_t)H * W, PAIF_EINVAL, "stem: batch stride %zu < H*W", img_bstride);
  const int chunks = (W + STEM_CHUNK - 1) / STEM_CHUNK;
  PAIF_REQUIRE((size_t)B * H * chunks < ((size_t)1 << 31), PAIF_EINVAL, "stem: %dx%dx%d is too large for one launch", B, H, W);
  hipLaunchKernelGGL(stem_kernel, dim3((unsigned)min(B * H * chunks, STEM_GRID)), dim3(256), 0, paif::as_stream(stream), img, w,
                     prelu, feat, guide, B, H, W, img_bstride, chunks, feat16, twin_f16);
  PAIF_LAUNCH_CHECK("stem");
  return 0;
}

int paif_stem_fwd(const float* img, size_t img_bstride, const float* w, const float* prelu, float* feat, float* guide,
                  int B, int H, int W, paif_stream_t stream) {
  return stem_launch(img, img_bstride, w, prelu, feat, guide, nullptr, 0, B, H, W, stream);
}

int paif_stem_fwd_twin(const float* img, size_t img_bstride, const float* w, const float* prelu, float* feat, float* feat_bf16,
                       float* guide, int B, int H, int W, paif_stream_t stream) {
  PAIF_REQUIRE(feat_bf16, PAIF_EINVAL, "stem_twin: null bf16 map");
  return stem_launch(img, img_bstride, w, prelu, feat, guide, reinterpret_cast<unsigned short*>(feat_bf16), 0, B, H, W, stream);
}

int paif_stem_fwd_twin_f16(const float* img, size_t img_bstride, const float* w, const float* prelu, float* feat, float* feat_f16,
                           float* guide, int B, int H, int W, paif_stream_t stream) {
  PAIF_REQUIRE(feat_f16, PAIF_EINVAL, "stem_twin: null fp16 map");
  return stem_launch(img, img_bstride, w, prelu, feat, guide, reinterpret_cast<unsigned short*>(feat_f16), 1, B, H, W, stream);
}

int paif_dwconv_fwd(const float* x, const float* w, float* out, int k, int dil, int in_relu, int B, int H, int W,
                    paif_stream_t stream) {
  PAIF_REQUIRE(x && w && out && B > 0 && H > 0 && W > 0, PAIF_EINVAL, "dwconv: bad arguments");
  const dim3 g(grid_for((size_t)B * H * W, 32)), blk(256);
  hipStream_t st = paif::as_stream(stream);
  const int key = k * 10 + dil;
  switch (key) {
    case 31: hipLaunchKernelGGL((dwconv_kernel<3, 1>), g, blk, 0, st, x, w, out, in_relu, B, H, W); break;
    case 32: hipLaunchKernelGGL((dwconv_kernel<3, 2>), g, blk, 0, st, x, w, out, in_relu, B, H, W); break;
    case 51: hipLaunchKernelGGL((dwconv_kernel<5, 1>), g, blk, 0, st, x, w, out, in_relu, B, H, W); break;
    case 52: hipLaunchKernelGGL((dwconv_kernel<5, 2>), g, blk, 0, st, x, w, out, in_relu, B, H, W); break;
    case 71: hipLaunchKernelGGL((dwconv_kernel<7, 1>), g, blk, 0, st, x, w, out, in_relu, B, H, W); break;
    case 72: hipLaunchKernelGGL((dwconv_kernel<7, 2>), g, blk, 0, st, x, w, out, in_relu, B, H, W); break;
    default:
      paif::set_error("dwconv: kernel %d dil %d not built", k, dil);
      return PAIF_ENOSUP;
  }
  PAIF_LAUNCH_CHECK("dwconv");
  return 0;
}

int paif_channel_pool2_fwd(const float* ir, const float* vis, float* comp, int B, int H, int W, paif_stream_t stream) {
  PAIF_REQUIRE(ir && vis && comp && B > 0 && H > 0 && W > 0, PAIF_EINVAL, "channel_pool2: bad arguments");
  const size_t npix = (size_t)B * H * W;
  hipLaunchKernelGGL(channel_pool2_kernel<0>, dim3(grid_for(npix, 32)), dim3(256), 0, paif::as_stream(stream), ir, vis, comp,
                     npix);
  PAIF_LAUNCH_CHECK("channel_pool2");
  return 0;
}

int paif_channel_residue_fwd(const float* x, float* guide, int B, int H, int W, paif_stream_t stream) {
  PAIF_REQUIRE(x && guide && B > 0 && H > 0 && W > 0, PAIF_EINVAL, "channel_residue: bad arguments");
  const size_t npix = (size_t)B * H * W;
// ... 266 lines not shown
```

### paif_amd/csrc/gf_mfma2.hip

```cpp
#include <stdint.h>
#include <type_traits>

#include "paif_common.h"

#ifndef GF2_NS
#define GF2_NS paif_gf2
#endif
namespace GF2_NS {

constexpr int R = 4;
#ifndef GF2_NW
#define GF2_NW 8
#endif
constexpr int NW = GF2_NW;
constexpr int SC = 8 * NW;
constexpr int SO = SC - 4 * R;
constexpr int PF = 6;
constexpr int NQ = 6;
#ifndef GF2_DP
#define GF2_DP (GF2_NW >= 12 ? 2 : 3)
#endif
#ifndef GF2_MINW
#define GF2_MINW (GF2_NW / 4)
#endif
// ... 53 lines not shown
__device__ __forceinline__ u32x2 band_operand(int m, int colbase) {
  u32x2 d = {0u, 0u};
  if ((m & 3) < 2) {
    const int oc = 2 * (m >> 2) + (m & 3);
    unsigned v = 0;
#pragma unroll
    for (int s = 0; s < 2; ++s) {
      const int col = colbase + s;
      if (oc - col <= R && col - oc <= R) v |= 0x3C00u << (16 * s);
    }
    d[0] = v; d[1] = v;
  }
  return d;
}

#ifndef GF2_PAIRED
#define GF2_PAIRED 1
#endif
#if GF2_EARLY_AB && !GF2_PAIRED
#error "GF2_EARLY_AB is written for the paired form"
#endif
typedef _Float16 half8 __attribute__((ext_vector_type(8)));
__device__ __forceinline__ u32x4 band_operand2(int m, int colbase) {
  const u32x2 d = band_operand((m & ~3) | (m & 1), colbase);
  return (m & 2) ? u32x4{0u, 0u, d[0], d[1]} : u32x4{d[0], d[1], 0u, 0u};
}
__device__ __forceinline__ f32x4 band_mfma2(u32x4 a_own, u32x4 b_own, u32x4 a_halo, u32x4 b_halo) {
  f32x4 acc = {0.f, 0.f, 0.f, 0.f};
  acc = __builtin_amdgcn_mfma_f32_16x16x32_f16(__builtin_bit_cast(half8, a_own), __builtin_bit_cast(half8, b_own), acc, 0, 0, 0);
  acc = __builtin_amdgcn_mfma_f32_16x16x32_f16(__builtin_bit_cast(half8, a_halo), __builtin_bit_cast(half8, b_halo), acc, 0, 0, 0);
  return acc;
}

struct Ring {
  f32x2 p[PF];
  f32x2 a1, a2;
};

template <int K>
__device__ __forceinline__ f32x2 ring_push(Ring& rg, f32x2 x) {
#ifdef GF2_NORING
  rg.a1 = rg.a1 + x; return rg.a1;
#endif
  const f32x2 p = (rg.a2 + rg.a1) + x;
  const f32x2 v = (p + rg.p[(K + 3) % PF]) + rg.p[K];
  rg.p[K] = p; rg.a2 = rg.a1; rg.a1 = x;
  return v;
}

template <int OM>
__global__ __launch_bounds__(64 * NW, GF2_MINW) void gf2_kernel(const float* __restrict__ guide, const float* __restrict__ y,
                                                     const float* __restrict__ planes, float* __restrict__ lf,
                                                     unsigned* __restrict__ flag, int B, int H, int W, int nstrip, int nslots,
                                                     int rows_per_slot, int total_rows) {
#if GF2_PAIRED
  __shared__ u32x4 hbuf[2][NQ / 2][NW + 2][64];
#else
  __shared__ u32x2 hbuf[2][NQ][NW + 2][64];
#endif
  __shared__ float rny_tab[MAXIT + 8];
  __shared__ float pbuf[2][5][SC];
  __shared__ float tbuf[NW][2][8][16];
  constexpr bool YDL = GF2_YD_LDS && OM >= 2;
  __shared__ f32x2 ydl[YDL ? 9 : 1][YDL ? 64 * NW : 1];

  const int tid = threadIdx.x, l = tid & 63;
  const int q = __builtin_amdgcn_readfirstlane(tid >> 6);
  const int c = l & 15, g = l >> 4;
  const int bid = blockIdx.x;
  const int chh = (bid >> 3) & 1;
  const int slot_id = (bid >> 4) * 8 + (bid & 7);
  if (slot_id >= nslots) return;
  int run_lo = slot_id * rows_per_slot;
  const int run_hi = min(total_rows, run_lo + rows_per_slot);
  const size_t npix = (size_t)B * H * W;
  const int lc0 = 8 * q + 2 * g;
  float vmax = 0.f;
#if GF2_PAIRED
  for (int i = tid; i < 2 * (NQ / 2) * 2 * 64; i += 64 * NW) {
    const int ln = i & 63, sl = (i >> 6) & 1, qq = (i >> 7) % (NQ / 2), par = i / (128 * (NQ / 2));
    hbuf[par][qq][sl ? NW + 1 : 0][ln] = u32x4{0u, 0u, 0u, 0u};
  }
#else
  for (int i = tid; i < 2 * NQ * 2 * 64; i += 64 * NW) {
    const int ln = i & 63, sl = (i >> 6) & 1, qq = (i >> 7) % NQ, par = i / (128 * NQ);
    hbuf[par][qq][sl ? NW + 1 : 0][ln] = u32x2{0u, 0u};
  }
#endif
  while (run_lo < run_hi) {
  const int sidx = run_lo / H;
  const int ybeg = run_lo - sidx * H, yend = min(H, ybeg + min(run_hi - run_lo, MAXIT - 32));
  run_lo += yend - ybeg;
  const int strip = sidx % nstrip, b = sidx / nstrip;
  const int X0 = strip * SO - 2 * R;
  const int col0 = X0 + lc0;
  const size_t img = (size_t)b * H * W;

  bool cin[2];
  float rnx[2];
#pragma unroll
  for (int i = 0; i < 2; ++i) {
    const int cc = col0 + i;
    cin[i] = cc >= 0 && cc < W;
    rnx[i] = cin[i] ? 1.0f / (float)(min(cc + R, W - 1) - max(cc - R, 0) + 1) : 0.f;
  }
  const bool outcol = lc0 >= 2 * R && lc0 < SC - 2 * R;
  constexpr bool BFO = OM != 0;
// ... 264 lines not shown
      }
#endif
    }
    vo0 += rowbytes_o;
    ++ro;
    GF2_ST(4);
    {
#ifdef GF2_NOLDS
      const u32x2 h_y = f_gy, h_gy = f_y;
#else
#if !GF2_PAIRED
      const u32x2 h_y = hbuf[par][0][rd_slot][rd_lane], h_gy = hbuf[par][1][rd_slot][rd_lane];
#endif
#endif
#if GF2_PAIRED
      const u32x4 h_yg = hbuf[par][0][rd_slot][rd_lane];
#if GF2_OWN_LDS
      const u32x4 o_yg = hbuf[par][0][q + 1][l];
#else
      const u32x4 o_yg = p_yg;
#endif
      const f32x4 s_yg = band_mfma2(a_own, o_yg, a_halo, h_yg);
      const f32x2 s_y = {s_yg[0], s_yg[1]}, s_gy = {s_yg[2], s_yg[3]};
#else
      const f32x2 s_y = band_mfma(a_own, f_y, a_halo, h_y);
      const f32x2 s_gy = band_mfma(a_own, f_gy, a_halo, h_gy);
#endif
      const f32x2 my = s_y * rn;
      const f32x2 cov = s_gy * rn - mg1 * my;
      const f32x2 A0 = cov * rd0, A1 = cov * rd1;
      wA0 = ring_push<k>(rA0, A0);
      wB0 = ring_push<k>(rB0, my - A0 * mg1);
      wA1 = ring_push<k>(rA1, A1);
      wB1 = ring_push<k>(rB1, my - A1 * mg1);
#if GF2_EARLY_AB
      const u32x2 f_a0 = split2(wA0, vmax), f_b0 = split2(wB0, vmax);
      hbuf[par ^ 1][1][q + 1][l] = u32x4{f_a0[0], f_a0[1], f_b0[0], f_b0[1]};
      const u32x2 f_a1 = split2(wA1, vmax), f_b1 = split2(wB1, vmax);
      hbuf[par ^ 1][2][q + 1][l] = u32x4{f_a1[0], f_a1[1], f_b1[0], f_b1[1]};
#endif
    }
    GF2_ST(5);
  };
  static_assert(PF == 6 && PF % DP == 0 && PF % DPL == 0, "the unrolled body lists PF = 6 steps");
  for (int itb = 0; itb < n_it; itb += PF) {
    step(std::integral_constant<int, 0>{}, itb);
    step(std::integral_constant<int, 1>{}, itb);
    step(std::integral_constant<int, 2>{}, itb);
    step(std::integral_constant<int, 3>{}, itb);
    step(std::integral_constant<int, 4>{}, itb);
    step(std::integral_constant<int, 5>{}, itb);
  }
  __syncthreads();
  }

#pragma unroll
  for (int m = 32; m >= 1; m >>= 1) vmax = fmaxf(vmax, __shfl_xor(vmax, m));
  if (l == 0 && !(vmax < 65000.f)) atomicOr(flag, 1u);
}

extern const int kStripOut = SO, kThreads = 64 * NW;

#if GF2_NW < 12
template __global__ void gf2_kernel<0>(const float*, const float*, const float*, float*, unsigned*, int, int, int, int, int, int, int);
template __global__ void gf2_kernel<1>(const float*, const float*, const float*, float*, unsigned*, int, int, int, int, int, int, int);
#endif
template __global__ void gf2_kernel<2>(const float*, const float*, const float*, float*, unsigned*, int, int, int, int, int, int, int);
template __global__ void gf2_kernel<3>(const float*, const float*, const float*, float*, unsigned*, int, int, int, int, int, int, int);

}
```

### paif_amd/csrc/guided_filter.hip

```cpp
#include <stdlib.h>
#include <string.h>

#include "paif_common.h"

namespace {

constexpr int R = 4;
constexpr int K = 2 * R + 1;
constexpr int NCOL = 32;
constexpr int OCOL = NCOL - 2 * R;
constexpr int ROWS_PER_SEG = 60;

__device__ __forceinline__ float4 f4add(float4 a, float4 b) { return make_float4(a.x + b.x, a.y + b.y, a.z + b.z, a.w + b.w); }
__device__ __forceinline__ float4 f4fma(float s, float4 a, float4 c) {
  return make_float4(fmaf(s, a.x, c.x), fmaf(s, a.y, c.y), fmaf(s, a.z, c.z), fmaf(s, a.w, c.w));
}

__global__ __launch_bounds__(256) void gf_ab_kernel(const float* __restrict__ guide, const float* __restrict__ y,
                                                    float* __restrict__ ab, float eps0, float eps1, int B, int H, int W,
                                                    int nstrip, int nseg) {
  __shared__ float4 sy[2][NCOL][8];
  __shared__ float4 sgy[2][NCOL][8];
  __shared__ float2 sg[2][NCOL];
  const int q = threadIdx.x & 7, xi = threadIdx.x >> 3;
// ... 135 lines not shown
        *reinterpret_cast<float4*>(out + px * 32 + q * 4) =
            make_float4(fmaf(ba.x / n, g, bb.x / n), fmaf(ba.y / n, g, bb.y / n), fmaf(ba.z / n, g, bb.z / n),
                        fmaf(ba.w / n, g, bb.w / n));
      }
    }
  }
}

}

extern "C" {

int paif_guided_filter_ab_fwd(const float* guide, const float* y, float* ab, float eps0, float eps1, int B, int H, int W,
                              paif_stream_t stream) {
  PAIF_REQUIRE(guide && y && ab && B > 0, PAIF_EINVAL, "guided_filter_ab: bad arguments");
  PAIF_REQUIRE(H > 2 * R + 1 && W > 2 * R + 1, PAIF_EINVAL, "guided_filter: H,W must exceed 2r+1 = %d (got %dx%d)", K, H, W);
  const int nstrip = (W + OCOL - 1) / OCOL, nseg = (H + ROWS_PER_SEG - 1) / ROWS_PER_SEG;
  hipLaunchKernelGGL(gf_ab_kernel, dim3(B * nstrip * nseg), dim3(256), 0, paif::as_stream(stream), guide, y, ab, eps0, eps1,
                     B, H, W, nstrip, nseg);
  PAIF_LAUNCH_CHECK("guided_filter_ab");
  return 0;
}

int paif_guided_filter_lf_fwd(const float* guide, const float* ab, float* lf, int B, int H, int W, paif_stream_t stream) {
  PAIF_REQUIRE(guide && ab && lf && B > 0, PAIF_EINVAL, "guided_filter_lf: bad arguments");
  PAIF_REQUIRE(H > 2 * R + 1 && W > 2 * R + 1, PAIF_EINVAL, "guided_filter: H,W must exceed 2r+1 = %d (got %dx%d)", K, H, W);
  const int nstrip = (W + OCOL - 1) / OCOL, nseg = (H + ROWS_PER_SEG - 1) / ROWS_PER_SEG;
  hipLaunchKernelGGL(gf_lf_kernel, dim3(B * nstrip * nseg, 2), dim3(256), 0, paif::as_stream(stream), guide, ab, lf, B, H,
                     W, nstrip, nseg);
  PAIF_LAUNCH_CHECK("guided_filter_lf");
  return 0;
}

}

namespace {

constexpr int FC = 64;
constexpr int FO = FC - 4 * R;
constexpr int PF = 3;

__device__ __forceinline__ void lds_barrier() {
  asm volatile("s_waitcnt lgkmcnt(0)" ::: "memory");
  __builtin_amdgcn_s_barrier();
  asm volatile("" ::: "memory");
}

constexpr int GT = 32, GH = GT + 2 * R;
__global__ __launch_bounds__(256) void gf_guide_stats_kernel(const float* __restrict__ guide, float* __restrict__ gs, unsigned* __restrict__ flag,
                                                             float eps0, float eps1, int B, int H, int W, int tilesX, int tilesY) {
  __shared__ float sG[GH][GH + 1];
  __shared__ float sH[GH][GT + 1], sH2[GH][GT + 1];
  int t = blockIdx.x;
  if (t == 0 && threadIdx.x == 0) *flag = 0u;
  const int tx = t % tilesX; t /= tilesX;
  const int ty = t % tilesY;
  const int b = t / tilesY;
  const int x0 = tx * GT - R, y0 = ty * GT - R;
  const float* base = guide + (size_t)b * H * W;
  for (int i = threadIdx.x; i < GH * GH; i += 256) {
    const int r = i / GH, c = i - r * GH;
    const int gy = y0 + r, gx = x0 + c;
    const float v = base[(size_t)min(max(gy, 0), H - 1) * W + min(max(gx, 0), W - 1)];
    sG[r][c] = (gy >= 0 && gy < H && gx >= 0 && gx < W) ? v : 0.f;
  }
  __syncthreads();
  for (int i = threadIdx.x; i < GH * GT; i += 256) {
    const int r = i / GT, c = i - r * GT;
    float s = 0.f, ss = 0.f;
#pragma unroll
    for (int j = 0; j < K; ++j) { const float g = sG[r][c + j]; s += g; ss = fmaf(g, g, ss); }
    sH[r][c] = s; sH2[r][c] = ss;
  }
  __syncthreads();
  const size_t npix = (size_t)B * H * W;
  for (int i = threadIdx.x; i < GT * GT; i += 256) {
    const int r = i / GT, c = i - r * GT;
    const int yy = ty * GT + r, xx = tx * GT + c;
    if (yy >= H || xx >= W) continue;
    float s = 0.f, ss = 0.f;
#pragma unroll
    for (int j = 0; j < K; ++j) { s += sH[r + j][c]; ss += sH2[r + j][c]; }
    const int cy = min(yy + R, H - 1) - max(yy - R, 0) + 1;
    const int cx = min(xx + R, W - 1) - max(xx - R, 0) + 1;
    const float rn = 1.0f / (float)(cy * cx);
    const float mg = s * rn;
    const float var = ss * rn - mg * mg;
    const size_t pix = (size_t)b * H * W + (size_t)yy * W + xx;
    gs[pix] = mg;
    gs[npix + pix] = 1.0f / (var + eps0);
    gs[2 * npix + pix] = 1.0f / (var + eps1);
    gs[3 * npix + pix] = rn;
  }
}

template <typename V> struct VecOps;
template <> struct VecOps<float4> {
  static constexpr int VW = 4;
  static __device__ __forceinline__ float4 zero() { return make_float4(0.f, 0.f, 0.f, 0.f); }
};
template <> struct VecOps<float2> {
  static constexpr int VW = 2;
  static __device__ __forceinline__ float2 zero() { return make_float2(0.f, 0.f); }
};
template <typename V> __device__ __forceinline__ V vadd(V a, V b) {
  V r; float* pr = reinterpret_cast<float*>(&r); const float* pa = reinterpret_cast<const float*>(&a); const float* pb = reinterpret_cast<const float*>(&b);
#pragma unroll
  for (int i = 0; i < VecOps<V>::VW; ++i) pr[i] = pa[i] + pb[i];
  return r;
}
template <typename V> __device__ __forceinline__ V vfma(float s, V a, V c) {
  V r; float* pr = reinterpret_cast<float*>(&r); const float* pa = reinterpret_cast<const float*>(&a); const float* pc = reinterpret_cast<const float*>(&c);
#pragma unroll
  for (int i = 0; i < VecOps<V>::VW; ++i) pr[i] = fmaf(s, pa[i], pc[i]);
  return r;
}

template <typename V, int NL>
__global__ __launch_bounds__(FC * NL) void gf_fused_kernel(const float* __restrict__ guide, const float* __restrict__ y,
                                                           const float* __restrict__ gs, const unsigned* __restrict__ only_if, float* __restrict__ lf,
                                                           int B, int H, int W, int nstrip, int nseg, int frows, int out_bf16) {
  constexpr int VW = VecOps<V>::VW;
  const bool y_f16 = out_bf16 == 3;
  if (y_f16) out_bf16 = 2;
  const unsigned short* const y16 = reinterpret_cast<const unsigned short*>(y) + (blockIdx.z * NL + threadIdx.x % NL) * VW;
  unsigned short* const lf16 = reinterpret_cast<unsigned short*>(lf);
  if (only_if != nullptr && *only_if == 0u) return;
  __shared__ V s_a[2][FC][NL];
  __shared__ V s_b[2][FC][NL];
  const int xi = threadIdx.x / NL;
  const int ql = threadIdx.x - xi * NL;
  y += (blockIdx.z * NL + ql) * VW;
  lf += (blockIdx.z * NL + ql) * VW;
  auto ldy = [&](size_t px) -> V {
    if (y_f16) {
      V r;
      float* pr = reinterpret_cast<float*>(&r);
#pragma unroll
      for (int i = 0; i < VW; ++i) pr[i] = (float)__builtin_bit_cast(_Float16, y16[px * 32 + i]);
      return r;
    }
    return *reinterpret_cast<const V*>(y + px * 32);
  };
  int t = blockIdx.x;
  const int strip = t % nstrip; t /= nstrip;
  const int seg = t % nseg;
  const int b = t / nseg;
  const int e = blockIdx.y;
  const int col = strip * FO - 2 * R + xi;
  const bool colin = col >= 0 && col < W;
  const int ybeg = seg * frows, yend = min(H, ybeg + frows);
  const size_t img = (size_t)b * H * W;
  float* out = lf + (size_t)e * ((size_t)B * H * W * 32);
  unsigned short* out16 = lf16 + (blockIdx.z * NL + ql) * VW + (size_t)e * ((size_t)B * H * W * 32);
  const float* gmean = gs;
  const float* grden = gs + (size_t)(1 + e) * ((size_t)B * H * W);

  const int cx = min(col + R, W - 1) - max(col - R, 0) + 1;
  float rnt[R + 1];
#pragma unroll
  for (int i = 0; i <= R; ++i) rnt[i] = 1.0f / (float)((K - i) * max(cx, 1));
  auto rn_of = [&](int row) -> float {
    const int miss = K - (min(row + R, H - 1) - max(row - R, 0) + 1);
    float r = rnt[0];
#pragma unroll
    for (int i = 1; i <= R; ++i) r = miss == i ? rnt[i] : r;
    return r;
  };

  V ry[K], tA[K], tB[K];
  float rg[K];
  V a1 = VecOps<V>::zero(), a2 = a1, b1 = a1, b2 = a1;
#pragma unroll
  for (int k = 0; k < K; ++k) { tA[k] = VecOps<V>::zero(); tB[k] = tA[k]; }
  const int r0 = ybeg - 2 * R, r1 = yend + 2 * R;
  const int colc = min(max(col, 0), W - 1);
  V pv[PF];
  float pg[PF];
  float2 ps[PF];
#pragma unroll
// ... 51 lines not shown
        for (int i = 0; i < VW; ++i) {
          const float my = pby[i] * rn;
          pA[i] = (pbgy[i] * rn - mg * my) * rden;
          pB[i] = my - pA[i] * mg;
        }
      }
      tA[k] = vadd(vadd(a2, a1), A);
      tB[k] = vadd(vadd(b2, b1), Bc);
      a2 = a1; a1 = A; b2 = b1; b1 = Bc;
      const int orow = irow - R;
      if (orow < ybeg) { lds_barrier(); continue; }
      {
        s_a[1][xi][ql] = vadd(vadd(tA[k], tA[(k + 6) % K]), tA[(k + 3) % K]);
        s_b[1][xi][ql] = vadd(vadd(tB[k], tB[(k + 6) % K]), tB[(k + 3) % K]);
      }
      lds_barrier();
      if (xi >= 2 * R && xi < FC - 2 * R && col < W) {
        V ba = VecOps<V>::zero(), bb = ba;
#pragma unroll
        for (int j = -R; j <= R; ++j) {
          ba = vadd(ba, s_a[1][xi + j][ql]);
          bb = vadd(bb, s_b[1][xi + j][ql]);
        }
        const float rn = rn_of(orow);
        const size_t px = img + (size_t)orow * W + col;
        const float g0 = rg[(k + 1) % K];
        V o;
        float* po = reinterpret_cast<float*>(&o);
        const float* pa = reinterpret_cast<const float*>(&ba);
        const float* pb = reinterpret_cast<const float*>(&bb);
#pragma unroll
        for (int i = 0; i < VW; ++i) po[i] = fmaf(pa[i] * rn, g0, pb[i] * rn);
        if (out_bf16 == 2) {
          const V yv = ldy(px);
          const float* py_ = reinterpret_cast<const float*>(&yv);
#pragma unroll
          for (int i = 0; i < VW; ++i) out16[px * 32 + i] = __builtin_bit_cast(unsigned short, (_Float16)(py_[i] - po[i]));
        } else if (out_bf16) {
#pragma unroll
          for (int i = 0; i < VW; ++i) out16[px * 32 + i] = __builtin_bit_cast(unsigned short, (__bf16)po[i]);
        } else {
          paif::store_nt(out + px * 32, o);
        }
      }
    }
  }
}

}

namespace paif_gf2 {
template <int OM>
__global__ void gf2_kernel(const float* __restrict__ guide, const float* __restrict__ y, const float* __restrict__ planes, float* __restrict__ lf,
                           unsigned* __restrict__ flag, int B, int H, int W, int nstrip, int nslots, int rows_per_slot, int total_rows);
extern const int kStripOut, kThreads;
extern template __global__ void gf2_kernel<0>(const float*, const float*, const float*, float*, unsigned*, int, int, int, int, int, int, int);
extern template __global__ void gf2_kernel<1>(const float*, const float*, const float*, float*, unsigned*, int, int, int, int, int, int, int);
extern template __global__ void gf2_kernel<2>(const float*, const float*, const float*, float*, unsigned*, int, int, int, int, int, int, int);
extern template __global__ void gf2_kernel<3>(const float*, const float*, const float*, float*, unsigned*, int, int, int, int, int, int, int);
}
namespace paif_gf2w12 {
template <int OM>
__global__ void gf2_kernel(const float* __restrict__ guide, const float* __restrict__ y, const float* __restrict__ planes, float* __restrict__ lf,
                           unsigned* __restrict__ flag, int B, int H, int W, int nstrip, int nslots, int rows_per_slot, int total_rows);
extern const int kStripOut, kThreads;
extern template __global__ void gf2_kernel<2>(const float*, const float*, const float*, float*, unsigned*, int, int, int, int, int, int, int);
extern template __global__ void gf2_kernel<3>(const float*, const float*, const float*, float*, unsigned*, int, int, int, int, int, int, int);
}

extern "C" __attribute__((visibility("hidden"))) int paifi_gf_guide_stats(const float* guide, float* workspace, float eps0, float eps1, int B,
                                                                          int H, int W, paif_stream_t stream) {
  const size_t npix = (size_t)B * H * W;
  const int gtx = (W + GT - 1) / GT, gty = (H + GT - 1) / GT;
  hipLaunchKernelGGL(gf_guide_stats_kernel, dim3(B * gtx * gty), dim3(256), 0, paif::as_stream(stream), guide, workspace,
                     reinterpret_cast<unsigned*>(workspace + 4 * npix), eps0, eps1, B, H, W, gtx, gty);
  PAIF_LAUNCH_CHECK("guided_filter(stats)");
  return 0;
}

extern "C" size_t paif_guided_filter_fused_workspace_floats(int B, int H, int W) { return (size_t)4 * B * H * W + 64; }

static int gf_fused_launch(const float* guide, const float* y, float* lf, float eps0, float eps1, float* workspace, int B, int H, int W,
                           int out_bf16, paif_stream_t stream) {
  PAIF_REQUIRE(guide && y && lf && workspace && B > 0, PAIF_EINVAL, "guided_filter_fused: bad arguments");
  PAIF_REQUIRE(H > 2 * R + 1 && W > 2 * R + 1, PAIF_EINVAL, "guided_filter: H,W must exceed 2r+1 = %d (got %dx%d)", K, H, W);
  const int nstrip = (W + FO - 1) / FO;
  const char* eng = getenv("PAIF_GF_ENGINE");
  PAIF_REQUIRE(!(eng && !strcmp(eng, "mfma")), PAIF_ENOSUP,
               "guided_filter: the round-3 matrix-core engine (PAIF_GF_ENGINE=mfma) left the library in round 6 (tools/parked/gf_mfma.hip)");
  int engine = (eng && !strcmp(eng, "valu")) ? 0 : 2;
  const char* nwe = getenv("PAIF_GF_NW");
  PAIF_REQUIRE(!nwe || !strcmp(nwe, "8") || !strcmp(nwe, "12"), PAIF_EINVAL, "PAIF_GF_NW must be 8 or 12 (got '%s')", nwe);
  const bool w12 = out_bf16 >= 2 && !(nwe && !strcmp(nwe, "8"));
  const int strip_out = w12 ? paif_gf2w12::kStripOut : paif_gf2::kStripOut, threads2 = w12 ? paif_gf2w12::kThreads : paif_gf2::kThreads;
  const int nstrip2 = (W + strip_out - 1) / strip_out;
  if (engine == 2 && ((size_t)(B + 1) * H * W * 128 >= 0x7FF00000ull || (size_t)B * nstrip2 * H >= 0x7FFFFFFFull)) engine = 0;
  static const int form = [] {
    const char* e = getenv("PAIF_GF_FORM");
    if (!e) return 0;
    return !strcmp(e, "4x4") ? 1 : !strcmp(e, "4x2") ? 2 : !strcmp(e, "2x16") ? 3 : 0;
  }();
  const int zgroups = form == 0 ? 1 : form == 1 ? 2 : form == 2 ? 4 : 1;
  const int resident = form == 0 ? 1 : form == 1 ? 2 : form == 2 ? 4 : 1;
  hipStream_t st = paif::as_stream(stream);
  const size_t npix = (size_t)B * H * W;
  unsigned* flag = reinterpret_cast<unsigned*>(workspace + 4 * npix);
  const int gtx = (W + GT - 1) / GT, gty = (H + GT - 1) / GT;
  hipLaunchKernelGGL(gf_guide_stats_kernel, dim3(B * gtx * gty), dim3(256), 0, st, guide, workspace, flag, eps0, eps1, B, H, W, gtx, gty);
  PAIF_LAUNCH_CHECK("guided_filter_fused(stats)");
  auto pick = [&](int warm, int res, int zg, int& nseg) {
    long best = -1;
    nseg = 1;
    for (int n = 1; n <= 16 && n <= H; ++n) {
      const int rows = (H + n - 1) / n;
      const long blocks = (long)B * nstrip * n * 2 * zg;
      const long cost = ((blocks + 256 * res - 1) / (256 * res)) * (rows + warm);
      if (best < 0 || cost < best) { best = cost; nseg = n; }
    }
  };
  if (engine == 2) {
    static const int cus = [] {
      int dev = 0, n = 256;
      if (hipGetDevice(&dev) == hipSuccess) (void)hipDeviceGetAttribute(&n, hipDeviceAttributeMultiprocessorCount, dev);
      return n > 1 ? n : 2;
    }();
    const long total_rows = (long)B * nstrip2 * H;
    int nslots = (int)(total_rows / 96);
    nslots = nslots < 1 ? 1 : (nslots > cus / 2 ? cus / 2 : nslots);
    const int rows_per_slot = (int)((total_rows + nslots - 1) / nslots);
    const int grid = (nslots + 7) / 8 * 16;
    if (w12 && out_bf16 == 3)
      hipLaunchKernelGGL((paif_gf2w12::gf2_kernel<3>), dim3(grid), dim3(threads2), 0, st, guide, y, workspace, lf, flag, B, H, W, nstrip2, nslots,
                         rows_per_slot, (int)total_rows);
    else if (w12)
      hipLaunchKernelGGL((paif_gf2w12::gf2_kernel<2>), dim3(grid), dim3(threads2), 0, st, guide, y, workspace, lf, flag, B, H, W, nstrip2, nslots,
                         rows_per_slot, (int)total_rows);
    else if (out_bf16 == 3)
      hipLaunchKernelGGL((paif_gf2::gf2_kernel<3>), dim3(grid), dim3(threads2), 0, st, guide, y, workspace, lf, flag, B, H, W, nstrip2, nslots,
                         rows_per_slot, (int)total_rows);
    else if (out_bf16 == 2)
      hipLaunchKernelGGL((paif_gf2::gf2_kernel<2>), dim3(grid), dim3(threads2), 0, st, guide, y, workspace, lf, flag, B, H, W, nstrip2, nslots,
                         rows_per_slot, (int)total_rows);
    else if (out_bf16)
      hipLaunchKernelGGL((paif_gf2::gf2_kernel<1>), dim3(grid), dim3(threads2), 0, st, guide, y, workspace, lf, flag, B, H, W, nstrip2, nslots,
                         rows_per_slot, (int)total_rows);
    else
      hipLaunchKernelGGL((paif_gf2::gf2_kernel<0>), dim3(grid), dim3(threads2), 0, st, guide, y, workspace, lf, flag, B, H, W, nstrip2, nslots,
                         rows_per_slot, (int)total_rows);
    PAIF_LAUNCH_CHECK("guided_filter_fused(mfma2)");
  }
  int nseg;
  pick(4 * R, resident, zgroups, nseg);
  const int frows = (H + nseg - 1) / nseg;
  const unsigned* only_if = engine == 2 ? flag : nullptr;
  const dim3 grid(B * nstrip * nseg, 2, zgroups);
  if (form == 0) hipLaunchKernelGGL((gf_fused_kernel<float4, 8>), grid, dim3(FC * 8), 0, st, guide, y, workspace, only_if, lf, B, H, W, nstrip, nseg, frows, out_bf16);
  else if (form == 1) hipLaunchKernelGGL((gf_fused_kernel<float4, 4>), grid, dim3(FC * 4), 0, st, guide, y, workspace, only_if, lf, B, H, W, nstrip, nseg, frows, out_bf16);
  else if (form == 2) hipLaunchKernelGGL((gf_fused_kernel<float4, 2>), grid, dim3(FC * 2), 0, st, guide, y, workspace, only_if, lf, B, H, W, nstrip, nseg, frows, out_bf16);
  else hipLaunchKernelGGL((gf_fused_kernel<float2, 16>), grid, dim3(FC * 16), 0, st, guide, y, workspace, only_if, lf, B, H, W, nstrip, nseg, frows, out_bf16);
  PAIF_LAUNCH_CHECK("guided_filter_fused");
  return 0;
}

extern "C" int paif_guided_filter_fused_fwd(const float* guide, const float* y, float* lf, float eps0, float eps1, float* workspace, int B,
                                            int H, int W, paif_stream_t stream) {
  return gf_fused_launch(guide, y, lf, eps0, eps1, workspace, B, H, W, 0, stream);
}

extern "C" int paif_guided_filter_fused_fwd_hf16(const float* guide, const float* y, float* hf, float eps0, float eps1, float* workspace, int B,
                                                 int H, int W, paif_stream_t stream) {
  return gf_fused_launch(guide, y, hf, eps0, eps1, workspace, B, H, W, 2, stream);
}

extern "C" int paif_guided_filter_fused_fwd_hf16_y16(const float* guide, const float* y16, float* hf, float eps0, float eps1, float* workspace,
                                                     int B, int H, int W, paif_stream_t stream) {
  return gf_fused_launch(guide, y16, hf, eps0, eps1, workspace, B, H, W, 3, stream);
}

extern "C" int paif_guided_filter_fused_fwd_bf16(const float* guide, const float* y, float* lf, float eps0, float eps1, float* workspace, int B,
                                                 int H, int W, paif_stream_t stream) {
  return gf_fused_launch(guide, y, lf, eps0, eps1, workspace, B, H, W, 1, stream);
}
```

### paif_amd/operations_m.py

```python
import torch
import torch.nn as nn

from . import ops


class _NeverCalled:
    def forward(self, *a, **k):
        raise RuntimeError("%s is a parameter holder; the HIP path must be used" % type(self).__name__)


class Conv2dParams(_NeverCalled, nn.Conv2d):
    pass


class Conv1dParams(_NeverCalled, nn.Conv1d):
    pass


class BatchNormParams(_NeverCalled, nn.BatchNorm2d):
    pass


class PReLUParams(_NeverCalled, nn.PReLU):
    pass
# ... 132 lines not shown
            return self._add_res(y, res)
        if self.groups != 1:
            raise NotImplementedError("grouped BasicConv other than depthwise")
        if C not in (32, 64, 96) or self.conv.out_channels != 32:
            raise NotImplementedError("BasicConv %d->%d: the HIP conv is built for 32-channel NAS cells" % (C, self.conv.out_channels))
        nsrc = C // 32
        srcs = [x] if nsrc == 1 else [x[..., 32 * i:32 * (i + 1)].contiguous() for i in range(nsrc)]
        scale = shift = None
        if self.bn is not None:
            scale, shift = _bn_scale_shift(self.bn, self._packs)
        act, slope = (ops.ACT_PRELU, self.relu.weight) if self.relu is not None else (ops.ACT_NONE, None)
        return ops.conv2d(srcs, self.wpk(nsrc, 32), self.kernel_size, self.dilation, scale=scale, shift=shift, act=act,
                          prelu=slope, res=res)


def conv3x3(in_planes, out_planes, stride=1):
    return Conv2dParams(in_planes, out_planes, kernel_size=3, stride=stride, padding=1, bias=False)


class ResidualDenseBlock(_HipOp):

    def __init__(self, in_channels, kernel_size, dialtions=1, bias=False):
        super().__init__()
        self.k, self.d = kernel_size, dialtions
        self.conv1 = BasicConv(in_channels, in_channels, kernel_size, dilation=dialtions, relu=False)
        self.conv2 = BasicConv(in_channels * 2, in_channels, kernel_size, dilation=dialtions, relu=False)
        self.conv3 = BasicConv(in_channels * 3, in_channels, kernel_size, dilation=dialtions, relu=False)
        self.lrelu = PReLUParams()

    takes_cpool = True

    def forward_nhwc(self, x, res=(), tape=None, cpool=None):
        a = self.lrelu.weight
        k, d = self.k, self.d
        kw = dict(act=ops.ACT_PRELU, prelu=a)
        if tape is not None and ops.taping_wgrad():
            x1, z1 = ops.conv2d([x], self.conv1.wpk(1, 32), k, d, want_aux=True, **kw)
            x2, z2 = ops.conv2d([x, x1], self.conv2.wpk(2, 32), k, d, want_aux=True, **kw)
            out, z3 = ops.conv2d([x, x1, x2], self.conv3.wpk(3, 32), k, d, alpha=0.333333, res=(x,) + tuple(res), want_aux=True, **kw)
            tape.append(dict(x=x, x1=x1, x2=x2, z1=z1, z2=z2, z3=z3))
            return out
        if (tape is None and x.dtype in ops.H16 and k == 3 and d == 1 and len(res) <= 2 and ops.CONFIG.get("rdb_fused", False)
                and x.shape[0] * ((x.shape[1] + 7) // 8) * ((x.shape[2] + 27) // 28) >= 512):
            ws = [self.conv1.conv.weight, self.conv2.conv.weight, self.conv3.conv.weight]
            wpk = self._packs.get("rdb_" + str(x.dtype), ws, lambda: ops.rdb_fused_pack(ws[0], ws[1], ws[2], x.dtype))
            return ops.rdb_fused(x, wpk, a, alpha=0.333333, res=tuple(res), cpool=cpool)
        x1 = ops.conv2d([x], self.conv1.wpk(1, 32), k, d, **kw)
        x2 = ops.conv2d([x, x1], self.conv2.wpk(2, 32), k, d, **kw)
        if tape is None:
            return ops.conv2d([x, x1, x2], self.conv3.wpk(3, 32), k, d, alpha=0.333333, res=(x,) + tuple(res), cpool=cpool, **kw)
        out, z3 = ops.conv2d([x, x1, x2], self.conv3.wpk(3, 32), k, d, alpha=0.333333, res=(x,) + tuple(res), want_aux=True, **kw)
        tape.append(dict(x1=x1, x2=x2, z3=z3))
        return out

    bwd_takes_res = True

    def backward_nhwc(self, g, t, wgrad=False, res=()):
        a = self.lrelu.weight
        k, d = self.k, self.d
        w1, w2, w3 = self.conv1.conv.weight, self.conv2.conv.weight, self.conv3.conv.weight
        s1, s2 = t.get("z1"), t.get("z2")
        if s1 is None:
            check_positive_slope(a, "ResidualDenseBlock")
            s1, s2 = t["x1"], t["x2"]
        ds = ops.grad_of(a) if wgrad else None
        t3 = ops.prelu_bwd(g, t["z3"], a, ds, want_dx=True, factor=0.333333)
        d_x = ops.conv2d([t3], self._dgrad_w("c3s0", w3, 0), k, d, alpha=0.333333, res=(g,))
        d_x1 = ops.conv2d([t3], self._dgrad_w("c3s1", w3, 32), k, d, alpha=0.333333)
        d_x2 = ops.conv2d([t3], self._dgrad_w("c3s2", w3, 64), k, d, alpha=0.333333)
        t2 = ops.prelu_bwd(d_x2, s2, a, ds, want_dx=True)
        d_x = ops.conv2d([t2], self._dgrad_w("c2s0", w2, 0), k, d, res=(d_x,))
        d_x1 = ops.conv2d([t2], self._dgrad_w("c2s1", w2, 32), k, d, res=(d_x1,))
        if wgrad:
            x, x1, x2 = t["x"], t["x1"], t["x2"]
            for w, srcs, dout, z, alpha in ((w3, [x, x1, x2], g, t["z3"], 0.333333), (w2, [x, x1], d_x2, t["z2"], 1.0),
                                            (w1, [x], d_x1, t["z1"], 1.0)):
                gw = ops.grad_of(w)
                if gw is not None:
                    ops.conv2d_wgrad(srcs, dout, k, d, z=z, act=ops.ACT_PRELU, prelu=a, alpha=alpha, out=gw)
            if ds is not None:
                ops.prelu_bwd(d_x1, t["z1"], a, ds, factor=1.0)
        return ops.conv2d([d_x1], self._dgrad_w("c1", w1, 0), k, d, res=(d_x,) + tuple(res), in_act=ops.IN_DPRELU, in_aux=s1, in_prelu=a)


class ResidualModule(_HipOp):

    def __init__(self, in_channels, kernel_size, dialtions=1, bias=False):
        super().__init__()
        self.k, self.d = kernel_size, dialtions
        self.op = nn.Sequential(
            BasicConv(in_channels, in_channels, kernel_size, dilation=dialtions, relu=False),
            Conv2dParams(in_channels, in_channels, kernel_size=3, stride=1, padding=2, dilation=2, bias=False),
            Conv2dParams(in_channels, in_channels, kernel_size=1, padding=0, bias=False),
            BatchNormParams(in_channels),
            PReLUParams(),
        )

    takes_out_f32 = True

    def forward_nhwc(self, x, res=(), tape=None, out_f32=False):
        op = self.op
        t1 = ops.conv2d([x], op[0].wpk(1, 32), self.k, self.d)
        if tape is None and not op[3].training and ops.CONFIG.get("resmod_compose", True):
            wc = self._packs.get("w23", [op[1].weight, op[2].weight],
                                 lambda: ops.pack_conv_weight(ops.compose_pw_conv_weight(op[2].weight, op[1].weight), 1, 32, 3))
            scale, shift = _bn_scale_shift(op[3], self._packs)
# ... 362 lines not shown
```

### paif_amd/ops.py

```python
import ctypes
import weakref
import os

import torch

from . import _lib

ACT_NONE, ACT_PRELU, ACT_RELU = 0, 1, 2
ACT_GELU = 1

def _env_switch(name, default="1"):
    v = os.environ.get(name, default)
    if v not in ("0", "1", "gemm"):
        raise ValueError("%s=%r: expected 0, 1 or gemm" % (name, v))
    return {"0": False, "1": True, "gemm": "gemm"}[v]


GEMM_PRECISIONS = ("f32", "bf16x3", "auto", "bf16x6", "auto6", "f16x3", "auto6h")


def _env_gemm_precision():
    v = os.environ.get("PAIF_GEMM_PRECISION", "auto")
    if v not in GEMM_PRECISIONS:
        raise ValueError("PAIF_GEMM_PRECISION=%r: expected one of %s" % (v, GEMM_PRECISIONS))
    return v


CONFIG = {"conv_precision": "bf16x3", "gemm_precision": _env_gemm_precision(), "serpentine": True, "attack_precision": "bf16x6", "storage": "f32",
          "two_stream": False,
          "cpool_fused": True, "f16_last_f32": True, "f16_decomp_split": False,
          "gf_in_f16": os.environ.get("PAIF_GF_IN_F16", "0") == "1",
          "rdb_fused": False, "gemm2": False, "timer_torch_events": os.environ.get("PAIF_TIMER_TORCH_EVENTS", "0") == "1", "infer_f16x3": os.environ.get("PAIF_INFER_F16X3", "1") != "0", "wgrad_f16x3": os.environ.get("PAIF_WGRAD_F16X3", "1") != "0", "_wgrad_scale": None, "gemm_split_min_m": 2048, "f16x3_min_k": int(os.environ.get("PAIF_F16X3_MIN_K", "32")), "attack_bwd_f16x3": _env_switch("PAIF_ATTACK_BWD_F16X3"),
          "attack_grad_scale_log2": (int(os.environ["PAIF_ATTACK_GSCALE"]) if "PAIF_ATTACK_GSCALE" in os.environ else None),
          "attack_fwd_f16x3": _env_switch("PAIF_ATTACK_FWD_F16X3"), "attn_x6": os.environ.get("PAIF_ATTN_X6", "1") != "0", "attn_f16x3": os.environ.get("PAIF_ATTN_F16X3", "1") != "0", "gemm_gather": os.environ.get("PAIF_GEMM_GATHER", "1") != "0"}
_ACT_BF16 = [False]
H16 = (torch.bfloat16, torch.float16)


STORAGE_MODES = ("f32", "bf16", "bf16_split", "f16")


def set_storage(mode):
    if mode not in STORAGE_MODES:
        raise ValueError("storage must be one of %s" % (STORAGE_MODES,))
    CONFIG["storage"] = mode


def pack_precision():
    return "f16" if _ACT_BF16[0] is torch.float16 else CONFIG["conv_precision"]


class bf16_activations:

    def __init__(self, enable=True):
        self.enable = enable

    def __enter__(self):
        self.old = _ACT_BF16[0]
        on = self.enable and CONFIG["storage"] in ("bf16", "bf16_split", "f16") and CONFIG["conv_precision"] == "bf16x3"
        _ACT_BF16[0] = (torch.float16 if CONFIG["storage"] == "f16" else torch.bfloat16) if on else False

    def __exit__(self, et, *a):
        was_f16 = _ACT_BF16[0] is torch.float16
        _ACT_BF16[0] = self.old
        if not self.old:
            _TWINS.clear()
        if was_f16 and et is None and _F16_GUARD and not torch.cuda.is_current_stream_capturing():
            _f16_guard_poll(torch.cuda.current_device())


_F16_GUARD = {}


def f16_guard_flag(device):
    g = _F16_GUARD.get(device.index)
    if g is None:
        g = _F16_GUARD[device.index] = dict(flag=torch.zeros(1, device=device, dtype=torch.int32),
                                            host=torch.zeros(1, dtype=torch.int32).pin_memory(), event=None, dirty=False)
    g["dirty"] = True
    return g["flag"]


# ... 350 lines not shown
    ycc = ycc.contiguous()
    B, _, H, W = ycc.shape
    L = lib()
    partial = torch.empty(2 * L.paif_minmax_blocks(B, H, W), device=ycc.device, dtype=torch.float32)
    rgb = torch.empty_like(ycc)
    _lib.check(L.paif_recompose_clamp_fwd(_p(fused), _p(ycc), _p(rgb), _p(partial), B, H, W, _stream()), "recompose_clamp")
    return rgb, partial


def fused_to_uint8(fused, ycc):
    rgb, partial = recompose_clamp(fused, ycc)
    B, _, H, W = rgb.shape
    out = torch.empty((B, H, W, 3), device=rgb.device, dtype=torch.uint8)
    _lib.check(lib().paif_fused_uint8_fwd(_p(rgb), _p(partial), partial.numel() // 2, ctypes.c_void_p(out.data_ptr()), B, H, W, _stream()),
               "fused_uint8")
    return out


def seg_input_from_fused(fused, ycc, return_minmax=False, minmax_sync=None):
    fused = fused.contiguous()
    ycc = ycc.contiguous()
    B, _, H, W = ycc.shape
    L = lib()
    nblk = L.paif_minmax_blocks(B, H, W)
    partial = torch.empty(2 * nblk, device=ycc.device, dtype=torch.float32)
    rgb = torch.empty_like(ycc)
    _lib.check(L.paif_recompose_clamp_fwd(_p(fused), _p(ycc), _p(rgb), _p(partial), B, H, W, _stream()), "recompose_clamp")
    if minmax_sync is not None:
        mn, mx = minmax_sync(partial[:nblk].min(), partial[nblk:].max())
        partial, nblk = torch.stack([mn.reshape(()), mx.reshape(())]).contiguous(), 1
    mm = torch.empty(2, device=ycc.device, dtype=torch.float32)
    _lib.check(L.paif_minmax_normalize_fwd(_p(rgb), _p(partial), nblk, _p(rgb), _p(mm), B, H, W, _stream()),
               "minmax_normalize")
    return (rgb, mm) if return_minmax else rgb


def u8_to_planes(src):
    if src.dim() == 3:
        src = src.unsqueeze(-1)
    assert src.dtype == torch.uint8 and src.is_cuda and src.is_contiguous()
    B, H, W, C = src.shape
    out = torch.empty((B, C, H, W), device=src.device, dtype=torch.float32)
    _lib.check(lib().paif_u8_to_planes_fwd(ctypes.c_void_p(src.data_ptr()), _p(out), B, H * W, C, _stream()), "u8_to_planes")
    return out


def u8_to_i64(src):
    assert src.dtype == torch.uint8 and src.is_cuda and src.is_contiguous()
    out = torch.empty(src.shape, device=src.device, dtype=torch.int64)
    _lib.check(lib().paif_u8_to_i64_fwd(ctypes.c_void_p(src.data_ptr()), ctypes.c_void_p(out.data_ptr()), src.numel(), _stream()), "u8_to_i64")
    return out


def stem(img, w, prelu, want_guide=True):
    B, _, H, W = img.shape
    if img.stride(3) != 1 or img.stride(2) != W:
        img = img.contiguous()
    bstride = img.stride(0) if B > 1 else H * W
    feat = None if (_ACT_BF16[0] is torch.float16 and CONFIG["gf_in_f16"]) else torch.empty((B, H, W, 32), device=img.device, dtype=torch.float32)
    guide = torch.empty((B, H, W), device=img.device, dtype=torch.float32) if want_guide else None
    if img.dtype != torch.float32 or not img.is_cuda:
        raise RuntimeError("stem: need a float32 CUDA tensor")
    if _ACT_BF16[0] is torch.float16 and CONFIG["gf_in_f16"]:
        twin = torch.empty((B, H, W, 32), device=img.device, dtype=torch.float16)
        _lib.check(lib().paif_stem_fwd_twin_f16(ctypes.c_void_p(img.data_ptr()), bstride, _p(w), _p(prelu), None, _pa(twin), _p(guide),
                                                B, H, W, _stream()), "stem")
        return twin, guide
    if _ACT_BF16[0]:
        twin = torch.empty((B, H, W, 32), device=img.device, dtype=_ACT_BF16[0])
        fn = lib().paif_stem_fwd_twin_f16 if _ACT_BF16[0] is torch.float16 else lib().paif_stem_fwd_twin
        _lib.check(fn(ctypes.c_void_p(img.data_ptr()), bstride, _p(w), _p(prelu), _p(feat), _pa(twin), _p(guide),
                      B, H, W, _stream()), "stem")
        _TWINS[feat.data_ptr()] = (feat, twin)
        return feat, guide
    _lib.check(lib().paif_stem_fwd(ctypes.c_void_p(img.data_ptr()), bstride, _p(w), _p(prelu), _p(feat), _p(guide),
                                   B, H, W, _stream()), "stem")
    return feat, guide


def channel_residue(x):
    B, H, W, C = x.shape
    assert C == 32
    g = torch.empty((B, H, W), device=x.device, dtype=torch.float32)
    _lib.check(lib().paif_channel_residue_fwd(_p(x), _p(g), B, H, W, _stream()), "channel_residue")
    return g


class GfTape:
    __slots__ = ("mc", "stats")

    def __init__(self, mc, stats):
        self.mc, self.stats = mc, stats


def guided_filter_pair(guide, y, eps=(0.001, 0.0001), want_ab=False, out_bf16=False, tape=None):
    hf16 = out_bf16 is torch.float16
    out_bf16 = bool(out_bf16)
    B, H, W, C = y.shape
    assert C == 32
    assert H > 9 and W > 9, "guided filter needs H, W > 2r+1 = 9"
    L = lib()
    if not want_ab and CONFIG.get("gf_fused", True):
        lf = torch.empty((2, B, H, W, 32), device=y.device, dtype=torch.float16 if hf16 else torch.bfloat16 if out_bf16 else torch.float32)
        ws = torch.empty(L.paif_guided_filter_fused_workspace_floats(B, H, W), device=y.device, dtype=torch.float32)
        import os
        eng = os.environ.get("PAIF_GF_ENGINE")
        tag = ("gf_fused_kernel" if eng == "valu" else "gf2_kernel") + " (+ gf_guide_stats_kernel)"
        e0 = TIMER.start(tag) if TIMER is not None else None
        y16 = y.dtype == torch.float16
        if y16 and not hf16:
            raise NotImplementedError("guided filter: an fp16 target map is built for the fp16 configuration's high-frequency output only")
        fn = (L.paif_guided_filter_fused_fwd_hf16_y16 if y16 else L.paif_guided_filter_fused_fwd_hf16 if hf16 else
              L.paif_guided_filter_fused_fwd_bf16 if out_bf16 else L.paif_guided_filter_fused_fwd)
        _lib.check(fn(_p(guide), _pa(y) if y16 else _p(y), _pa(lf), eps[0], eps[1], _p(ws), B, H, W, _stream()), "guided_filter_fused")
        if e0 is not None:
            TIMER.stop(tag, e0, 650 * B * H * W * 32, B * H * W * (4 + (2 if y16 else 4) * 32 + (2 if out_bf16 else 4) * 64))
        return lf
    assert not out_bf16, "bf16 low-frequency maps are an inference (fused-form) output"
    lf = torch.empty((2, B, H, W, 32), device=y.device, dtype=torch.float32)
    import os
    assert tape in (None, "mc", "ab"), tape
    if tape is None:
        tape = os.environ.get("PAIF_GF_TAPE")
        if tape not in (None, "mc", "ab"):
            raise ValueError("PAIF_GF_TAPE must be 'mc' or 'ab', got %r" % tape)
    if tape is None:
        tape = "mc" if os.environ.get("PAIF_GF_BWD") != "v1" and L.paif_guided_filter_taped_fits(B, H, W) else "ab"
    if want_ab and tape == "mc":
        mc = torch.empty((2, B, H, W, 32), device=y.device, dtype=torch.float32)
        stats = torch.empty(L.paif_guided_filter_fused_workspace_floats(B, H, W), device=y.device, dtype=torch.float32)
        _lib.check(L.paif_guided_filter_taped_fwd(_p(guide), _p(y), _p(mc), _p(lf), eps[0], eps[1], _p(stats), B, H, W, _stream()),
                   "guided_filter_taped")
        return lf, GfTape(mc, stats)
    ab = torch.empty((4, B, H, W, 32), device=y.device, dtype=torch.float32)
    _lib.check(L.paif_guided_filter_ab_fwd(_p(guide), _p(y), _p(ab), eps[0], eps[1], B, H, W, _stream()), "guided_filter_ab")
    _lib.check(L.paif_guided_filter_lf_fwd(_p(guide), _p(ab), _p(lf), B, H, W, _stream()), "guided_filter_lf")
    return (lf, ab) if want_ab else lf


def pack_conv_weight(w, nsrc, cin, kh, precision=None):
    cout = w.shape[0]
    assert tuple(w.shape) == (cout, nsrc * cin, kh, kh), (tuple(w.shape), nsrc, cin, kh)
    precision = precision or pack_precision()
    if cin != 32:
        precision = "f32"
    L = lib()
    nfl = L.paif_conv_wpk_floats(nsrc, cin, kh)
    wpk = torch.empty(nfl * 3 // 2 if precision == "bf16x6" else nfl, device=w.device, dtype=torch.float32)
    wc = w.detach().contiguous()
    if precision in ("f16", "f16x2"):
        _lib.check(L.paif_pack_conv_weight_f16x2(_p(wc), _p(wpk), cout, nsrc, kh, _stream()), "pack_conv_weight_f16x2")
    elif precision == "f16x3":
        _lib.check(L.paif_pack_conv_weight_f16x2(_p(wc * F16X3_WSCALE), _p(wpk), cout, nsrc, kh, _stream()), "pack_conv_weight_f16x2")
    elif precision == "bf16x6":
        _lib.check(L.paif_pack_conv_weight_bf16x6(_p(wc), _p(wpk), cout, nsrc, kh, _stream()), "pack_conv_weight_bf16x6")
    elif precision == "bf16x3":
        _lib.check(L.paif_pack_conv_weight_bf16x3(_p(wc), _p(wpk), cout, nsrc, kh, _stream()), "pack_conv_weight_bf16x3")
    else:
        _lib.check(L.paif_pack_conv_weight(_p(wc), _p(wpk), cout, nsrc, cin, kh, _stream()), "pack_conv_weight")
    return PackedWeight(wpk, precision)


def compose_dw_pw_weight(dw, pw):
    C, _, k, _ = dw.shape
    Co = pw.shape[0]
    assert tuple(dw.shape) == (C, 1, k, k) and tuple(pw.shape) == (Co, C, 1, 1)
    out = torch.empty((Co, C, k, k), device=dw.device, dtype=torch.float32)
    _lib.check(lib().paif_compose_dw_pw_weight(_p(dw.detach().contiguous()), _p(pw.detach().contiguous()), _p(out), Co, C, k, _stream()),
               "compose_dw_pw_weight")
    return out

# ... 37 lines not shown
    return PackedWeight(wpk, "rdb_f16" if dtype == torch.float16 else "rdb_bf16")


def rdb_fused(x, wpk, prelu, alpha=0.333333, res=(), cpool=None):
    B, H, W, C = x.shape
    assert C == 32 and x.dtype in H16 and x.is_contiguous() and len(res) <= 2
    assert wpk.precision == ("rdb_f16" if x.dtype == torch.float16 else "rdb_bf16")
    res = [cast_storage(r, x.dtype) for r in res]
    out = torch.empty_like(x)
    cp = None
    if cpool is not None:
        comp, coff = cpool
        assert comp.dtype == torch.float32 and tuple(comp.shape) == (B, H, W, 4) and comp.is_contiguous() and coff in (0, 2)
        cp = ctypes.c_void_p(comp.data_ptr() + 4 * coff)
    if CONFIG.get("serpentine", True):
        _SERP[0] ^= 1
    tag = "rdb_fused_kernel"
    e0 = TIMER.start(tag) if TIMER is not None else None
    _lib.check(lib().paif_rdb_fused_fwd(_pa(x), _p(wpk.data), _p(prelu), float(alpha), _pa(res[0]) if len(res) > 0 else None,
                                        _pa(res[1]) if len(res) > 1 else None, _pa(out), cp, int(x.dtype == torch.float16),
                                        _SERP[0] if CONFIG.get("serpentine", True) else 0, B, H, W, _stream()), "rdb_fused")
    if e0 is not None:
        px = B * H * W
        TIMER.stop(tag, e0, 2 * px * 9 * 32 * 32 * 6, px * 2 * 32 * 9, px * 2 * 32 * len(res))
    return out


def pack_decomp1x1_hf_weight(w):
    assert tuple(w.shape) == (32, 128, 1, 1)
    L = lib()
    wpk = torch.empty(L.paif_conv_wpk_floats(3, 32, 1), device=w.device, dtype=torch.float32)
    _lib.check(L.paif_pack_decomp1x1_hf_weight_f16x2(_p(w.detach().contiguous()), _p(wpk), _stream()), "pack_decomp1x1_hf_weight_f16x2")
    return PackedWeight(wpk, "f16x2" if CONFIG.get("f16_decomp_split", False) else "f16")


def bn_fold(weight, bias, mean, var, eps):
    C = weight.shape[0]
    scale = torch.empty(C, device=weight.device, dtype=torch.float32)
    shift = torch.empty(C, device=weight.device, dtype=torch.float32)
    _lib.check(lib().paif_bn_fold(_p(weight.detach()), _p(bias.detach()), _p(mean), _p(var), eps, _p(scale), _p(shift), C, _stream()),
               "bn_fold")
    return scale, shift


IN_DPRELU, IN_DRELU, IN_SCALE = 3, 4, 5


def conv2d_kernel_name(desc, B, H, W):
    buf = ctypes.create_string_buffer(96)
    _lib.check(lib().paif_conv2d_kernel_name(ctypes.byref(desc), B, H, W, buf, len(buf)), "conv2d_kernel_name")
    return buf.value.decode()


def conv2d(srcs, wpk, kh, dil=1, cin=32, cout=32, in_act=ACT_NONE, in_prelu=None, scale=None, shift=None,
           act=ACT_NONE, prelu=None, alpha=1.0, res=(), pool=False, want_aux=False, in_aux=None, in_scale=None,
           in_alpha=1.0, epi_dact=0, epi_aux=None, out=None, out_f32=False, cpool=None):
    B, H, W, C = srcs[0].shape
    assert C == cin and 1 <= len(srcs) <= 3
    res = [r for r in res if r is not None]
    extra = res[3:]
    res = res[:3]
    sdt = srcs[0].dtype
    src16 = sdt in H16
    assert all(s_.dtype == sdt for s_ in srcs), "mixed source storage"
    if out is not None:
        odt = out.dtype
    elif src16:
        want32 = (out_f32 and sdt == torch.float16 and kh == 3 and dil == 2 and len(srcs) == 1 and in_act == ACT_NONE and not pool and cout == 32
                  and wpk.precision == "f16")
        odt = torch.float32 if want32 else sdt
    else:
        odt = torch.bfloat16 if (_ACT_BF16[0] is torch.bfloat16 and kh == 1 and not want_aux and in_act < 3 and not epi_dact) else torch.float32
    out16 = odt in H16
    if src16:
        storage = (3 if out16 else 4) if sdt == torch.float16 else 1
        if not out16 and sdt != torch.float16:
            raise NotImplementedError("bf16 sources with an fp32 output are not built")
    else:
        storage = 0 if not out16 else 2
        if odt == torch.float16:
            raise NotImplementedError("fp32 sources with an fp16 output are not built (the fp16 forward hands the 1x1 fp16 maps)")
    if storage and (want_aux or in_act >= 3 or epi_dact or in_aux is not None):
        raise NotImplementedError("16-bit activation storage is built for the inference forward (no gradient hooks)")
    if wpk.precision == "f16x3" and storage:
        raise NotImplementedError("the fp16-pair conv arithmetic is built for fp32 maps")
    if (sdt == torch.float16) != (wpk.precision in ("f16", "f16x2")):
        raise RuntimeError("conv2d: fp16 maps need an fp16 weight pack and vice versa (sources %s, pack %s)" % (sdt, wpk.precision))
    if out is None:
        out = torch.empty((B, H, W, cout), device=srcs[0].device, dtype=odt)
    else:
        assert tuple(out.shape) == (B, H, W, cout) and out.is_contiguous()
    rdt = sdt if storage == 4 else odt
    res = [cast_storage(r, rdt) for r in res]
    extra = [cast_storage(r, odt) for r in extra]
    src_bf, out_bf = src16, out16
    L = lib()
    d = _lib.ConvDesc()
    d.storage = storage
    for i in range(3):
        d.src[i] = _pa(srcs[i]) if i < len(srcs) else None
        d.res[i] = _pa(res[i]) if i < len(res) else None
    for r in res:
        assert tuple(r.shape) == (B, H, W, cout)
    d.nsrc, d.cin, d.wpk, d.kh, d.dil = len(srcs), cin, _p(wpk.data), kh, dil
    d.precision = _PREC_CODE[wpk.precision]
    if storage in (1, 2) and wpk.precision == "bf16x3" and CONFIG["storage"] == "bf16":
        d.precision = PREC_BF16
    d.in_act, d.in_prelu = in_act, _p(in_prelu)
    d.scale, d.shift = _p(scale), _p(shift)
    d.act, d.prelu, d.alpha = act, _p(prelu), alpha
    d.out, d.cout = _pa(out), cout
    partial = None
    if pool:
        partial = torch.empty((L.paif_conv2d_blocks(B, H, W), 32), device=out.device, dtype=torch.float32)
    d.pool_partial = _p(partial)
    aux = torch.empty_like(out) if want_aux else None
    d.aux_out, d.in_aux, d.in_scale, d.in_alpha = _p(aux), _p(in_aux), _p(in_scale), in_alpha
    d.epi_aux, d.epi_dact = _p(epi_aux), epi_dact
    pool_after = None
    if cpool is not None:
        comp, coff = cpool
        assert cout == 32 and comp.dtype == torch.float32 and tuple(comp.shape) == (B, H, W, 4) and comp.is_contiguous() and coff in (0, 2)
        if not extra and CONFIG.get("cpool_fused", True) and L.paif_conv2d_can_cpool(ctypes.byref(d), B, H, W):
            d.cpool = ctypes.c_void_p(comp.data_ptr() + 4 * coff)
        else:
            pool_after = (comp, coff)
    if CONFIG.get("serpentine", True):
        _SERP[0] ^= 1
        d.reverse_tiles = _SERP[0]
    e0 = None
    if TIMER is not None:
        tag = conv2d_kernel_name(d, B, H, W)
        e0 = TIMER.start(tag)
    _lib.check(L.paif_conv2d_fwd(ctypes.byref(d), B, H, W, _stream()), "conv2d")
    if e0 is not None:
        px = B * H * W
        eb_in, eb_out = (2 if src_bf else 4), (2 if out_bf else 4)
        eb_res = 2 if (res and res[0].dtype in H16) else 4
        TIMER.stop(tag, e0, 2 * px * kh * kh * cin * len(srcs) * cout, px * (eb_in * cin * len(srcs) + eb_out * cout), px * eb_res * cout * len(res))
    for r in extra:
        out = add(out, r)
    if pool_after is not None:
        channel_pool1(out, *pool_after)
    if pool and want_aux:
        return out, partial, aux
    if want_aux:
        return out, aux
    return (out, partial) if pool else out


def pack_conv_dgrad_weight(w, coff, cs, precision=None):
    Co, Ctot, k, _ = w.shape
    wt = torch.empty((cs, Co, k, k), device=w.device, dtype=torch.float32)
    _lib.check(lib().paif_conv_weight_dgrad(_p(w.detach().contiguous()), _p(wt), Co, Ctot, k, coff, cs, _stream()), "conv_weight_dgrad")
    return pack_conv_weight(wt, 1, Co, k, precision)


def fold_decomp1x1_weight(w):
    wf = torch.empty((32, 96, 1, 1), device=w.device, dtype=torch.float32)
    _lib.check(lib().paif_fold_decomp1x1_weight(_p(w.detach().contiguous()), _p(wf), _stream()), "fold_decomp1x1_weight")
    return wf


def dwconv(x, w, k, dil, in_relu):
    B, H, W, C = x.shape
    assert C == 32
    out = torch.empty_like(x)
    fn = {torch.bfloat16: lib().paif_dwconv_fwd_bf16, torch.float16: lib().paif_dwconv_fwd_f16}.get(x.dtype, lib().paif_dwconv_fwd)
    _lib.check(fn(_pa(x), _p(w.detach().contiguous()), _pa(out), k, dil, int(in_relu), B, H, W, _stream()), "dwconv")
    return out


def channel_pool2(ir, vis):
    B, H, W, _ = ir.shape
    comp = torch.empty((B, H, W, 4), device=ir.device, dtype=torch.float32)
    assert ir.dtype == vis.dtype
    fn = {torch.bfloat16: lib().paif_channel_pool2_fwd_bf16, torch.float16: lib().paif_channel_pool2_fwd_f16}.get(ir.dtype, lib().paif_channel_pool2_fwd)
    _lib.check(fn(_pa(ir), _pa(vis), _p(comp), B, H, W, _stream()), "channel_pool2")
    return comp


def channel_pool1(x, comp, coff):
    B, H, W, C = x.shape
    assert C == 32 and tuple(comp.shape) == (B, H, W, 4) and comp.dtype == torch.float32 and coff in (0, 2)
    fn = {torch.bfloat16: lib().paif_channel_pool1_fwd_bf16, torch.float16: lib().paif_channel_pool1_fwd_f16}.get(x.dtype, lib().paif_channel_pool1_fwd)
    _lib.check(fn(_pa(x), ctypes.c_void_p(comp.data_ptr() + 4 * coff), B, H, W, _stream()), "channel_pool1")
    return comp


def spa_blend(comp, w, ir, vis, want_scale=False):
    B, H, W, _ = ir.shape
    agg = torch.empty_like(ir)
# ... 1305 lines not shown
```

Before: 2690.

## Batch the IR and visible branches into paired kernel launches

```diff
diff --git a/include/paif_hip.h b/include/paif_hip.h
--- a/include/paif_hip.h
+++ b/include/paif_hip.h
@@ -38,6 +38,9 @@
                        float* guide, int B, int H, int W, paif_stream_t stream);
 int paif_stem_fwd_twin_f16(const float* img, size_t img_bstride, const float* w, const float* prelu, float* feat, float* feat_f16,
                            float* guide, int B, int H, int W, paif_stream_t stream);
+int paif_stem_fwd_pair(const float* img0, size_t img_bstride0, const float* w0, const float* prelu0, const float* img1, size_t img_bstride1,
+                       const float* w1, const float* prelu1, float* feat, float* feat16, int twin, float* guide, int B, int H, int W,
+                       paif_stream_t stream);
 int paif_channel_residue_fwd(const float* x, float* guide, int B, int H, int W, paif_stream_t stream);
 
 int paif_guided_filter_ab_fwd(const float* guide, const float* y, float* ab, float eps0, float eps1,
@@ -57,6 +60,10 @@
 
 int paif_guided_filter_fused_fwd_hf16_y16(const float* guide, const float* y16, float* hf, float eps0, float eps1, float* workspace,
                                           int B, int H, int W, paif_stream_t stream);
+
+int paif_guided_filter_fused_joint_fits(int B, int H, int W);
+int paif_guided_filter_fused_fwd_joint(const float* guide, const float* y, float* out, float eps0, float eps1, float* workspace, int B,
+                                       int bsplit, int H, int W, int out_mode, paif_stream_t stream);
 
 typedef struct {
   const float* src[3];
@@ -126,6 +133,8 @@
 
 int paif_conv2d_blocks(int B, int H, int W);
 int paif_conv2d_fwd(const paif_conv_desc* d, int B, int H, int W, paif_stream_t stream);
+int paif_conv2d_pair_kernel_name(const paif_conv_desc* d0, const paif_conv_desc* d1, int B, int H, int W, char* buf, int buflen);
+int paif_conv2d_fwd_pair(const paif_conv_desc* d0, const paif_conv_desc* d1, int B, int H, int W, paif_stream_t stream);
 int paif_conv2d_can_cpool(const paif_conv_desc* d, int B, int H, int W);
 int paif_channel_pool1_fwd(const float* x, float* comp_off, int B, int H, int W, paif_stream_t stream);
 int paif_channel_pool1_fwd_bf16(const float* x, float* comp_off, int B, int H, int W, paif_stream_t stream);
diff --git a/paif_amd/_lib.py b/paif_amd/_lib.py
--- a/paif_amd/_lib.py
+++ b/paif_amd/_lib.py
@@ -32,6 +32,7 @@
     "paif_stem_fwd": (c_int, [F, c_size_t, F, F, F, F, c_int, c_int, c_int, F]),
     "paif_stem_fwd_twin": (c_int, [F, c_size_t, F, F, F, F, F, c_int, c_int, c_int, F]),
     "paif_stem_fwd_twin_f16": (c_int, [F, c_size_t, F, F, F, F, F, c_int, c_int, c_int, F]),
+    "paif_stem_fwd_pair": (c_int, [F, c_size_t, F, F, F, c_size_t, F, F, F, F, c_int, F, c_int, c_int, c_int, F]),
     "paif_channel_residue_fwd": (c_int, [F, F, c_int, c_int, c_int, F]),
     "paif_guided_filter_ab_fwd": (c_int, [F, F, F, c_float, c_float, c_int, c_int, c_int, F]),
     "paif_guided_filter_lf_fwd": (c_int, [F, F, F, c_int, c_int, c_int, F]),
@@ -42,8 +43,12 @@
     "paif_guided_filter_fused_fwd_bf16": (c_int, [F, F, F, c_float, c_float, F, c_int, c_int, c_int, F]),
     "paif_guided_filter_fused_fwd_hf16": (c_int, [F, F, F, c_float, c_float, F, c_int, c_int, c_int, F]),
     "paif_guided_filter_fused_fwd_hf16_y16": (c_int, [F, F, F, c_float, c_float, F, c_int, c_int, c_int, F]),
+    "paif_guided_filter_fused_joint_fits": (c_int, [c_int, c_int, c_int]),
+    "paif_guided_filter_fused_fwd_joint": (c_int, [F, F, F, c_float, c_float, F, c_int, c_int, c_int, c_int, c_int, F]),
     "paif_conv2d_blocks": (c_int, [c_int, c_int, c_int]),
     "paif_conv2d_fwd": (c_int, [POINTER(ConvDesc), c_int, c_int, c_int, F]),
+    "paif_conv2d_pair_kernel_name": (c_int, [POINTER(ConvDesc), POINTER(ConvDesc), c_int, c_int, c_int, c_char_p, c_int]),
+    "paif_conv2d_fwd_pair": (c_int, [POINTER(ConvDesc), POINTER(ConvDesc), c_int, c_int, c_int, F]),
     "paif_conv2d_is_persistent": (c_int, [POINTER(ConvDesc), c_int, c_int, c_int]),
     "paif_conv2d_can_cpool": (c_int, [POINTER(ConvDesc), c_int, c_int, c_int]),
     "paif_rdb_fused_wpk_floats": (c_size_t, []),
diff --git a/paif_amd/core/model_fusion_auto.py b/paif_amd/core/model_fusion_auto.py
--- a/paif_amd/core/model_fusion_auto.py
+++ b/paif_amd/core/model_fusion_auto.py
@@ -2,7 +2,7 @@
 import torch.nn as nn
 
 from .. import ops
-from ..operations_m import OPS, BasicConv, Conv2dParams, PReLUParams, _HipOp, _PackCache, grad_anchor
+from ..operations_m import OPS, BasicConv, Conv2dParams, PReLUParams, ResidualDenseBlock, _HipOp, _PackCache, grad_anchor
 
 
 def RGB2YCrCb(input_im):
@@ -74,9 +74,9 @@
             self._ops += [MixedOp(C, name)]
         self._indices = indices
 
-    def forward_nhwc(self, inp, res=(), tape=None, out_f32=False, cpool=None):
-        s1 = inp
-        for i in range(self._steps):
+    def forward_nhwc(self, inp, res=(), tape=None, out_f32=False, cpool=None, first=None):
+        s1 = inp if first is None else first
+        for i in range(0 if first is None else 1, self._steps):
             last = i == self._steps - 1
             s1 = self._ops[i].forward_nhwc(s1, ((inp,) + tuple(res)) if last else (), tape, out_f32=out_f32 and last,
                                            cpool=cpool if last else None)
@@ -113,10 +113,31 @@
     def get_residue(self, tensor):
         return ops.to_nchw_view(ops.channel_residue(ops.to_nhwc(tensor)).unsqueeze(-1))
 
-    def decomposition_nhwc(self, x, guide=None, want_ab=False, out_bf16=False):
+    def decomposition_nhwc(self, x, guide=None, want_ab=False, out_bf16=False, bsplit=None):
         if guide is None:
             guide = ops.channel_residue(x)
-        return ops.guided_filter_pair(guide, x, tuple(self.eps_list), want_ab=want_ab, out_bf16=out_bf16)
+        return ops.guided_filter_pair(guide, x, tuple(self.eps_list), want_ab=want_ab, out_bf16=out_bf16, bsplit=bsplit)
+
+    def pair_capable(self):
+        firsts = [c._ops[0]._op for c in (self.chain, self.chain2) if c._steps > 0]
+        return len(firsts) == 2 and all(isinstance(o, ResidualDenseBlock) and (o.k, o.d) == (3, 1) for o in firsts)
+
+    def forward_pair_nhwc(self, feat, guide, fir, fvis, comp=None):
+        B = fir.shape[0]
+        lf16 = ops._ACT_BF16[0]
+        lf = self.decomposition_nhwc(feat, guide, out_bf16=lf16, bsplit=B)
+        (lf_ir0, lf_vis0), (lf_ir1, lf_vis1) = ops.pair_halves(lf[0], B), ops.pair_halves(lf[1], B)
+        pack1, pn = (ops.pack_decomp1x1_hf_weight, "_hf16") if lf16 is torch.float16 else (ops.pack_decomp1x1_weight, "")
+        w_lf = self._packs.get("lf" + pn, [self.conv1x1_lf.weight], lambda: pack1(self.conv1x1_lf.weight))
+        w_hf = self._packs.get("hf" + pn, [self.conv1x1_hf.weight], lambda: pack1(self.conv1x1_hf.weight))
+        lfm, hfm = ops.conv2d_pair(dict(srcs=[ops.cast_storage(fir, True), lf_ir0, lf_ir1], wpk=w_lf, kh=1, dil=1, shift=self.conv1x1_lf.bias),
+                                   dict(srcs=[ops.cast_storage(fvis, True), lf_vis0, lf_vis1], wpk=w_hf, kh=1, dil=1, shift=self.conv1x1_hf.bias))
+        f_ir = f_vis = None
+        if self.chain._steps > 1 and self.chain2._steps > 1 and not ops.CONFIG.get("rdb_fused", False):
+            f_ir, f_vis = ResidualDenseBlock.forward_pair_nhwc(self.chain._ops[0]._op, lfm, self.chain2._ops[0]._op, hfm)
+        ir_feature = self.chain.forward_nhwc(lfm, (fir,), None, cpool=None if comp is None else (comp, 0), first=f_ir)
+        vis_feature = self.chain2.forward_nhwc(hfm, (fvis,), None, cpool=None if comp is None else (comp, 2), first=f_vis)
+        return ir_feature, vis_feature
 
     @staticmethod
     def _cat_lf_hf(x, lf):
@@ -314,8 +335,14 @@
             if not torch.cuda.is_current_stream_capturing():
                 vis_feature.record_stream(main)
             del fvis, g_vis
-            agg = self.spa.blend_nhwc(ir_feature, vis_feature, comp=comp)
-            return self._tail_nhwc(self.chain.forward_nhwc(agg, (), None, out_f32=self._last_f32()))
+            return self._blend_tail_nhwc(ir_feature, vis_feature, comp)
+        if self._pair_path(tape, inter, ir.is_cuda) and ops.guided_filter_joint_fits(2 * ir.shape[0], ir.shape[2], ir.shape[3]):
+            feat, guide, (fir, fvis) = ops.stem_pair(ir, self.stem_1[0].weight, self.stem_1[1].weight,
+                                                     vis, self.stem_2[0].weight, self.stem_2[1].weight)
+            comp = self._new_comp(ir)
+            ir_feature, vis_feature = self.decompation.forward_pair_nhwc(feat, guide, fir, fvis, comp)
+            del feat, guide
+            return self._blend_tail_nhwc(ir_feature, vis_feature, comp)
         fir, g_ir = ops.stem(ir, self.stem_1[0].weight, self.stem_1[1].weight)
         fvis, g_vis = ops.stem(vis, self.stem_2[0].weight, self.stem_2[1].weight)
         t_dec = None if tape is None else {}
@@ -344,6 +371,14 @@
         if inter is not None:
             inter.update(fir=fir, fvis=fvis, ir_feature=ir_feature, vis_feature=vis_feature, agg=agg, feature2=feature2)
         return out
+
+    def _blend_tail_nhwc(self, ir_feature, vis_feature, comp):
+        agg = self.spa.blend_nhwc(ir_feature, vis_feature, comp=comp)
+        return self._tail_nhwc(self.chain.forward_nhwc(agg, (), None, out_f32=self._last_f32()))
+
+    def _pair_path(self, tape, inter, is_cuda):
+        return (tape is None and inter is None and is_cuda and bool(ops._ACT_BF16[0]) and not ops.CONFIG.get("two_stream", False)
+                and ops.CONFIG.get("stream_pair", True) and self.decompation.pair_capable())
 
     @staticmethod
     def _new_comp(img):
diff --git a/paif_amd/csrc/conv_dma.h b/paif_amd/csrc/conv_dma.h
--- a/paif_amd/csrc/conv_dma.h
+++ b/paif_amd/csrc/conv_dma.h
@@ -23,6 +23,19 @@
 };
 
 enum Form { NONE, TILE, ONE_BY_ONE, ROWS };
+
+struct Prob {
+  const void* src[3];
+  const void* res[3];
+  const void* wpk;
+  const float* scale;
+  const float* shift;
+  const float* prelu;
+  void* out;
+  float alpha;
+};
+bool pair_capable(const Args& a);
+int launch_pair(const Args& a0, const Args& a1, hipStream_t st);
 Form classify(const Args& a);
 bool can_cpool(const Args& a);
 int launch(const Args& a, hipStream_t st);
diff --git a/paif_amd/csrc/conv_dma.hip b/paif_amd/csrc/conv_dma.hip
--- a/paif_amd/csrc/conv_dma.hip
+++ b/paif_amd/csrc/conv_dma.hip
@@ -59,7 +59,7 @@
 };
 
 template <int NSRC, int NRES, int F, bool CP = false, int DIL = 1, int IA = 0>
-__global__ __launch_bounds__(256, 1) void conv3x3_h16_dma(Args a, int ntiles, int tilesX, int tilesY) {
+__global__ __launch_bounds__(256, 1) void conv3x3_h16_dma(Args a, int ntiles, int tilesX, int tilesY, Prob p1, int pair) {
   typedef Geo<DIL> G;
   constexpr int TWH = G::TWH, NPIX = G::NPIX, DPW = G::DPW, SLOT = G::SLOT, PF = G::PF, NSLOT = G::NSLOT, ROWB = G::ROWB, PARK_OFF = G::PARK_OFF;
   typedef Sched<NSRC, NRES, PF, DPW> SC;
@@ -74,7 +74,17 @@
   const int p = l & 31, hh = l >> 5;
   const int wb = G::base_row(w);
 
-  const int xcd = blockIdx.x & 7, wg = blockIdx.x >> 3, nwg = gridDim.x >> 3;
+  const int xcd = blockIdx.x & 7;
+  int wg = blockIdx.x >> 3, nwg = gridDim.x >> 3;
+  if (!CP && DIL == 1 && pair) {
+    nwg >>= 1;
+    if (wg >= nwg) {
+      wg -= nwg;
+#pragma unroll
+      for (int s = 0; s < 3; ++s) { a.src[s] = p1.src[s]; a.res[s] = p1.res[s]; }
+      a.wpk = p1.wpk; a.scale = p1.scale; a.shift = p1.shift; a.prelu = p1.prelu; a.out = p1.out; a.alpha = p1.alpha;
+    }
+  }
   const int tpx = (ntiles + 7) >> 3;
   const int t_beg = xcd * tpx, t_end = min(ntiles, t_beg + tpx);
   const int cnt = t_beg + wg < t_end ? (t_end - t_beg - wg + nwg - 1) / nwg : 0;
@@ -759,14 +769,14 @@
   const int tilesX = (a.W + TW - 1) / TW, tilesY = (a.H + TH - 1) / TH;
   if (a.cpool) {
     if constexpr (NSRC == 3 && (NRES == 1 || NRES == 3)) {
-      if (a.f16) hipLaunchKernelGGL((conv3x3_h16_dma<NSRC, NRES, 2, true>), dim3(256), dim3(256), 0, st, a, a.B * tilesX * tilesY, tilesX, tilesY);
-      else hipLaunchKernelGGL((conv3x3_h16_dma<NSRC, NRES, 1, true>), dim3(256), dim3(256), 0, st, a, a.B * tilesX * tilesY, tilesX, tilesY);
+      if (a.f16) hipLaunchKernelGGL((conv3x3_h16_dma<NSRC, NRES, 2, true>), dim3(256), dim3(256), 0, st, a, a.B * tilesX * tilesY, tilesX, tilesY, Prob{}, 0);
+      else hipLaunchKernelGGL((conv3x3_h16_dma<NSRC, NRES, 1, true>), dim3(256), dim3(256), 0, st, a, a.B * tilesX * tilesY, tilesX, tilesY, Prob{}, 0);
     } else {
       paif::set_error("conv2d(dma): the fused ChannelPool is built for 3 sources with 1 or 3 residual maps");
       return PAIF_ENOSUP;
     }
-  } else if (a.f16) hipLaunchKernelGGL((conv3x3_h16_dma<NSRC, NRES, 2>), dim3(256), dim3(256), 0, st, a, a.B * tilesX * tilesY, tilesX, tilesY);
-  else hipLaunchKernelGGL((conv3x3_h16_dma<NSRC, NRES, 1>), dim3(256), dim3(256), 0, st, a, a.B * tilesX * tilesY, tilesX, tilesY);
+  } else if (a.f16) hipLaunchKernelGGL((conv3x3_h16_dma<NSRC, NRES, 2>), dim3(256), dim3(256), 0, st, a, a.B * tilesX * tilesY, tilesX, tilesY, Prob{}, 0);
+  else hipLaunchKernelGGL((conv3x3_h16_dma<NSRC, NRES, 1>), dim3(256), dim3(256), 0, st, a, a.B * tilesX * tilesY, tilesX, tilesY, Prob{}, 0);
   hipError_t e = hipGetLastError();
   if (e != hipSuccess) {
     paif::set_error("conv2d(h16 dma): launch failed: %s", hipGetErrorString(e));
@@ -775,11 +785,32 @@
   return 0;
 }
 
+static Prob prob_of(const Args& a) {
+  Prob p{};
+  for (int s = 0; s < 3; ++s) { p.src[s] = a.src[s]; p.res[s] = a.res[s]; }
+  p.wpk = a.wpk; p.scale = a.scale; p.shift = a.shift; p.prelu = a.prelu; p.out = a.out; p.alpha = a.alpha;
+  return p;
+}
+
+template <int NSRC, int NRES>
+int launch_n_pair(const Args& a0, const Args& a1, hipStream_t st) {
+  const int tilesX = (a0.W + TW - 1) / TW, tilesY = (a0.H + TH - 1) / TH;
+  const Prob p1 = prob_of(a1);
+  if (a0.f16) hipLaunchKernelGGL((conv3x3_h16_dma<NSRC, NRES, 2>), dim3(256), dim3(256), 0, st, a0, a0.B * tilesX * tilesY, tilesX, tilesY, p1, 1);
+  else hipLaunchKernelGGL((conv3x3_h16_dma<NSRC, NRES, 1>), dim3(256), dim3(256), 0, st, a0, a0.B * tilesX * tilesY, tilesX, tilesY, p1, 1);
+  hipError_t e = hipGetLastError();
+  if (e != hipSuccess) {
+    paif::set_error("conv2d(h16 dma, pair): launch failed: %s", hipGetErrorString(e));
+    return (int)e;
+  }
+  return 0;
+}
+
 template <int NRES, bool CP>
 int launch_d2(const Args& a, hipStream_t st) {
   const int tilesX = (a.W + TW - 1) / TW, tilesY = (a.H + TH - 1) / TH;
-  if (a.f16) hipLaunchKernelGGL((conv3x3_h16_dma<1, NRES, 2, CP, 2, 2>), dim3(256), dim3(256), 0, st, a, a.B * tilesX * tilesY, tilesX, tilesY);
-  else hipLaunchKernelGGL((conv3x3_h16_dma<1, NRES, 1, CP, 2, 2>), dim3(256), dim3(256), 0, st, a, a.B * tilesX * tilesY, tilesX, tilesY);
+  if (a.f16) hipLaunchKernelGGL((conv3x3_h16_dma<1, NRES, 2, CP, 2, 2>), dim3(256), dim3(256), 0, st, a, a.B * tilesX * tilesY, tilesX, tilesY, Prob{}, 0);
+  else hipLaunchKernelGGL((conv3x3_h16_dma<1, NRES, 1, CP, 2, 2>), dim3(256), dim3(256), 0, st, a, a.B * tilesX * tilesY, tilesX, tilesY, Prob{}, 0);
   hipError_t e = hipGetLastError();
   if (e != hipSuccess) {
     paif::set_error("conv2d(h16 dma, dilation 2): launch failed: %s", hipGetErrorString(e));
@@ -825,6 +856,32 @@
   return is_tile(a) ? TILE : NONE;
 }
 
+bool pair_capable(const Args& a) {
+  switch (classify(a)) {
+    case ONE_BY_ONE: return true;
+    case TILE: break;
+    default: return false;
+  }
+  const long long tiles = (long long)a.B * ((a.H + TH - 1) / TH) * ((a.W + TW - 1) / TW);
+  const int key = a.nsrc * 10 + a.nres;
+  return a.kh == 3 && a.dil == 1 && a.cout == 32 && !a.cpool && (key == 10 || key == 20 || key == 31) && tiles <= 128 * 128;
+}
+
+int launch_1x1_pair(const Args& a0, const Prob& p1, hipStream_t st);
+
+int launch_pair(const Args& a0, const Args& a1, hipStream_t st) {
+  if (!pair_capable(a0) || !pair_capable(a1) || classify(a0) != classify(a1) || a0.nsrc != a1.nsrc || a0.nres != a1.nres) {
+    paif::set_error("conv2d(h16 dma, pair): no pair kernel for these two descriptors");
+    return PAIF_ENOSUP;
+  }
+  if (classify(a0) == ONE_BY_ONE) return launch_1x1_pair(a0, prob_of(a1), st);
+  switch (a0.nsrc * 10 + a0.nres) {
+    case 10: return launch_n_pair<1, 0>(a0, a1, st);
+    case 20: return launch_n_pair<2, 0>(a0, a1, st);
+    default: return launch_n_pair<3, 1>(a0, a1, st);
+  }
+}
+
 bool can_cpool(const Args& a) {
   return a.kh == 3 && a.cout == 32 && (a.nres == 1 || a.nres == 3) && ((a.dil == 1 && a.nsrc == 3) || (a.dil == 2 && a.nsrc == 1));
 }
diff --git a/paif_amd/csrc/conv_dma_1x1.hip b/paif_amd/csrc/conv_dma_1x1.hip
--- a/paif_amd/csrc/conv_dma_1x1.hip
+++ b/paif_amd/csrc/conv_dma_1x1.hip
@@ -30,14 +30,24 @@
 #endif
 
 template <int F>
-__global__ __launch_bounds__(WAVES * 64, 2) void conv_h16_dma_1x1(Args a, int ntiles) {
+__global__ __launch_bounds__(WAVES * 64, 2) void conv_h16_dma_1x1(Args a, int ntiles, Prob p1, int pair) {
   __shared__ __attribute__((aligned(16))) unsigned char smem[LDS_BYTES];
   asm volatile("" ::"v"((unsigned)(uintptr_t)(__attribute__((address_space(3))) unsigned char*)smem) : "memory");
 
   const int tid = threadIdx.x, l = tid & 63;
   const int w = __builtin_amdgcn_readfirstlane(tid >> 6);
   const int p = l & 31, hh = l >> 5;
-  const int gw = blockIdx.x * WAVES + w, nw = gridDim.x * WAVES;
+  int bid = blockIdx.x, nblk = gridDim.x;
+  if (pair) {
+    nblk >>= 1;
+    if (bid >= nblk) {
+      bid -= nblk;
+#pragma unroll
+      for (int s = 0; s < 3; ++s) a.src[s] = p1.src[s];
+      a.wpk = p1.wpk; a.scale = p1.scale; a.shift = p1.shift; a.prelu = p1.prelu; a.out = p1.out; a.alpha = p1.alpha;
+    }
+  }
+  const int gw = bid * WAVES + w, nw = nblk * WAVES;
   if (gw >= ntiles) return;
   const int cnt = (ntiles - gw + nw - 1) / nw;
 
@@ -181,8 +191,8 @@
 int launch_1x1(const Args& a, hipStream_t st) {
   const long long px = (long long)a.B * a.H * a.W;
   const int ntiles = (int)((px + TP - 1) / TP);
-  if (a.f16) hipLaunchKernelGGL(conv_h16_dma_1x1<2>, dim3(GRID), dim3(WAVES * 64), 0, st, a, ntiles);
-  else hipLaunchKernelGGL(conv_h16_dma_1x1<1>, dim3(GRID), dim3(WAVES * 64), 0, st, a, ntiles);
+  if (a.f16) hipLaunchKernelGGL(conv_h16_dma_1x1<2>, dim3(GRID), dim3(WAVES * 64), 0, st, a, ntiles, Prob{}, 0);
+  else hipLaunchKernelGGL(conv_h16_dma_1x1<1>, dim3(GRID), dim3(WAVES * 64), 0, st, a, ntiles, Prob{}, 0);
   hipError_t e = hipGetLastError();
   if (e != hipSuccess) {
     paif::set_error("conv2d(h16 dma 1x1): launch failed: %s", hipGetErrorString(e));
@@ -191,4 +201,17 @@
   return 0;
 }
 
-}
+int launch_1x1_pair(const Args& a, const Prob& p1, hipStream_t st) {
+  const long long px = (long long)a.B * a.H * a.W;
+  const int ntiles = (int)((px + TP - 1) / TP);
+  if (a.f16) hipLaunchKernelGGL(conv_h16_dma_1x1<2>, dim3(GRID), dim3(WAVES * 64), 0, st, a, ntiles, p1, 1);
+  else hipLaunchKernelGGL(conv_h16_dma_1x1<1>, dim3(GRID), dim3(WAVES * 64), 0, st, a, ntiles, p1, 1);
+  hipError_t e = hipGetLastError();
+  if (e != hipSuccess) {
+    paif::set_error("conv2d(h16 dma 1x1, pair): launch failed: %s", hipGetErrorString(e));
+    return (int)e;
+  }
+  return 0;
+}
+
+}
diff --git a/paif_amd/csrc/conv_mfma.hip b/paif_amd/csrc/conv_mfma.hip
--- a/paif_amd/csrc/conv_mfma.hip
+++ b/paif_amd/csrc/conv_mfma.hip
@@ -1843,6 +1843,15 @@
   return launch_key<FAM_F32>(p, a, st);
 }
 
+static bool plan_pair(const ConvPlan& p0, const ConvArgs& a0, const ConvPlan& p1, const ConvArgs& a1) {
+  if (p0.family != FAM_SPLIT || p1.family != FAM_SPLIT || p0.variant != CV_DMA || p1.variant != CV_DMA) return false;
+  if (p0.kh != p1.kh || p0.dil != p1.dil || p0.cin != p1.cin || p0.nres != p1.nres || p0.fmt != p1.fmt || p0.st != p1.st) return false;
+  if (a0.nsrc != a1.nsrc || a0.act != a1.act || a0.in_act != a1.in_act || a0.cout != a1.cout || a0.st != a1.st || a0.wl0 != a1.wl0) return false;
+  if (a0.cpool || a1.cpool || a0.pool_partial || a1.pool_partial) return false;
+  if ((a0.scale == nullptr) != (a1.scale == nullptr) || (a0.shift == nullptr) != (a1.shift == nullptr)) return false;
+  return paif_conv_dma::pair_capable(dma_args(a0, p0.kh, p0.dil)) && paif_conv_dma::pair_capable(dma_args(a1, p1.kh, p1.dil));
+}
+
 }
 
 extern "C" {
@@ -1868,7 +1877,7 @@
   return 0;
 }
 
-int paif_conv2d_fwd(const paif_conv_desc* d, int B, int H, int W, paif_stream_t stream) {
+static int check_desc(const paif_conv_desc* d, int B, int H, int W) {
   PAIF_REQUIRE(d && d->out && d->wpk, PAIF_EINVAL, "conv2d: null descriptor/out/wpk");
   PAIF_REQUIRE(d->nsrc >= 1 && d->nsrc <= 3, PAIF_EINVAL, "conv2d: nsrc=%d", d->nsrc);
   for (int s = 0; s < d->nsrc; ++s) PAIF_REQUIRE(d->src[s], PAIF_EINVAL, "conv2d: src[%d] null", s);
@@ -1899,8 +1908,31 @@
                    d->precision == PAIF_CONV_F16X3, PAIF_EINVAL,
                "conv2d: precision=%d", d->precision);
   PAIF_REQUIRE((d->precision != PAIF_CONV_BF16X6 && d->precision != PAIF_CONV_F16X3) || d->cin == 32, PAIF_ENOSUP, "conv2d: bf16x6 / f16x3 need 32-channel sources");
+  return 0;
+}
+
+int paif_conv2d_fwd(const paif_conv_desc* d, int B, int H, int W, paif_stream_t stream) {
+  if (const int rc = check_desc(d, B, H, W)) return rc;
   const ConvArgs a = conv_args(d, B, H, W);
   return plan_launch(plan_conv(a, d), a, paif::as_stream(stream));
+}
+
+int paif_conv2d_pair_kernel_name(const paif_conv_desc* d0, const paif_conv_desc* d1, int B, int H, int W, char* buf, int buflen) {
+  PAIF_REQUIRE(d0 && d1 && buf && buflen > 0 && B > 0 && H > 0 && W > 0, PAIF_EINVAL, "conv2d_pair_kernel_name: bad arguments");
+  const ConvArgs a0 = conv_args(d0, B, H, W), a1 = conv_args(d1, B, H, W);
+  const ConvPlan p0 = plan_conv(a0, d0), p1 = plan_conv(a1, d1);
+  PAIF_REQUIRE(plan_pair(p0, a0, p1, a1), PAIF_ENOSUP, "conv2d_pair: the two descriptors do not plan to one pair-capable kernel");
+  plan_name(p0, a0, buf, buflen);
+  return 0;
+}
+
+int paif_conv2d_fwd_pair(const paif_conv_desc* d0, const paif_conv_desc* d1, int B, int H, int W, paif_stream_t stream) {
+  if (const int rc = check_desc(d0, B, H, W)) return rc;
+  if (const int rc = check_desc(d1, B, H, W)) return rc;
+  const ConvArgs a0 = conv_args(d0, B, H, W), a1 = conv_args(d1, B, H, W);
+  const ConvPlan p0 = plan_conv(a0, d0), p1 = plan_conv(a1, d1);
+  PAIF_REQUIRE(plan_pair(p0, a0, p1, a1), PAIF_ENOSUP, "conv2d_pair: the two descriptors do not plan to one pair-capable kernel");
+  return paif_conv_dma::launch_pair(dma_args(a0, p0.kh, p0.dil), dma_args(a1, p1.kh, p1.dil), paif::as_stream(stream));
 }
 
 int paif_pack_conv_weight_bf16x3(const float* w, float* wpk, int cout, int nsrc, int kh, paif_stream_t stream) {
diff --git a/paif_amd/csrc/fusion_kernels.hip b/paif_amd/csrc/fusion_kernels.hip
--- a/paif_amd/csrc/fusion_kernels.hip
+++ b/paif_amd/csrc/fusion_kernels.hip
@@ -61,8 +61,15 @@
 __global__ __launch_bounds__(256) void stem_kernel(const float* __restrict__ img, const float* __restrict__ w,
                                                    const float* __restrict__ prelu, float* __restrict__ feat,
                                                    float* __restrict__ guide, int B, int H, int W,
-                                                   size_t img_bstride, int chunks, unsigned short* __restrict__ feat16, int twin_f16) {
+                                                   size_t img_bstride, int chunks, unsigned short* __restrict__ feat16, int twin_f16,
+                                                   const float* __restrict__ img1, const float* __restrict__ w1,
+                                                   const float* __restrict__ prelu1, size_t img_bstride1) {
   const int q = threadIdx.x & 7;
+  int bid = blockIdx.x, nblk = gridDim.x, row_off = 0;
+  if (img1 != nullptr) {
+    nblk >>= 1;
+    if (bid >= nblk) { bid -= nblk; img = img1; w = w1; prelu = prelu1; img_bstride = img_bstride1; row_off = B * H; }
+  }
   float wr[4][9];
 #pragma unroll
   for (int c = 0; c < 4; ++c)
@@ -72,7 +79,7 @@
   __shared__ float patch[2][3][STEM_CHUNK + 2];
   const int nitems = B * H * chunks;
   int par = 0;
-  for (int item = blockIdx.x; item < nitems; item += gridDim.x, par ^= 1) {
+  for (int item = bid; item < nitems; item += nblk, par ^= 1) {
   const int chunk = item % chunks;
   const int row = item / chunks;
   const int y = row % H, b = row / H;
@@ -85,9 +92,10 @@
     patch[par][r][c] = ok ? v : 0.f;
   }
   __syncthreads();
-  float* frow = feat ? feat + (size_t)row * W * 32 : nullptr;
-  unsigned short* frow16 = feat16 ? feat16 + (size_t)row * W * 32 : nullptr;
-  float* grow = guide ? guide + (size_t)row * W : nullptr;
+  const int orow = row + row_off;
+  float* frow = feat ? feat + (size_t)orow * W * 32 : nullptr;
+  unsigned short* frow16 = feat16 ? feat16 + (size_t)orow * W * 32 : nullptr;
+  float* grow = guide ? guide + (size_t)orow * W : nullptr;
 #pragma unroll
   for (int it = 0; it < STEM_CHUNK / 32; ++it) {
     const int xi = it * 32 + (threadIdx.x >> 3);
@@ -686,8 +694,25 @@
   const int chunks = (W + STEM_CHUNK - 1) / STEM_CHUNK;
   PAIF_REQUIRE((size_t)B * H * chunks < ((size_t)1 << 31), PAIF_EINVAL, "stem: %dx%dx%d is too large for one launch", B, H, W);
   hipLaunchKernelGGL(stem_kernel, dim3((unsigned)min(B * H * chunks, STEM_GRID)), dim3(256), 0, paif::as_stream(stream), img, w,
-                     prelu, feat, guide, B, H, W, img_bstride, chunks, feat16, twin_f16);
+                     prelu, feat, guide, B, H, W, img_bstride, chunks, feat16, twin_f16, nullptr, nullptr, nullptr, (size_t)0);
   PAIF_LAUNCH_CHECK("stem");
+  return 0;
+}
+
+int paif_stem_fwd_pair(const float* img0, size_t img_bstride0, const float* w0, const float* prelu0, const float* img1, size_t img_bstride1,
+                       const float* w1, const float* prelu1, float* feat, float* feat16, int twin, float* guide, int B, int H, int W,
+                       paif_stream_t stream) {
+  PAIF_REQUIRE(img0 && w0 && prelu0 && img1 && w1 && prelu1 && (feat || feat16) && B > 0 && H > 0 && W > 0, PAIF_EINVAL,
+               "stem_pair: bad arguments");
+  PAIF_REQUIRE((twin == 0) == (feat16 == nullptr) && twin >= 0 && twin <= 2, PAIF_EINVAL,
+               "stem_pair: twin must be 0 (none, feat16 NULL), 1 (bf16) or 2 (fp16)");
+  PAIF_REQUIRE(img_bstride0 >= (size_t)H * W && img_bstride1 >= (size_t)H * W, PAIF_EINVAL, "stem_pair: batch stride < H*W");
+  const int chunks = (W + STEM_CHUNK - 1) / STEM_CHUNK;
+  PAIF_REQUIRE((size_t)2 * B * H * chunks < ((size_t)1 << 31), PAIF_EINVAL, "stem_pair: 2x%dx%dx%d is too large for one launch", B, H, W);
+  const int per = min(B * H * chunks, STEM_GRID / 2);
+  hipLaunchKernelGGL(stem_kernel, dim3((unsigned)(2 * per)), dim3(256), 0, paif::as_stream(stream), img0, w0, prelu0, feat, guide, B, H, W,
+                     img_bstride0, chunks, reinterpret_cast<unsigned short*>(feat16), twin == 2 ? 1 : 0, img1, w1, prelu1, img_bstride1);
+  PAIF_LAUNCH_CHECK("stem_pair");
   return 0;
 }
 
diff --git a/paif_amd/csrc/gf_mfma2.hip b/paif_amd/csrc/gf_mfma2.hip
--- a/paif_amd/csrc/gf_mfma2.hip
+++ b/paif_amd/csrc/gf_mfma2.hip
@@ -129,7 +129,7 @@
 __global__ __launch_bounds__(64 * NW, GF2_MINW) void gf2_kernel(const float* __restrict__ guide, const float* __restrict__ y,
                                                      const float* __restrict__ planes, float* __restrict__ lf,
                                                      unsigned* __restrict__ flag, int B, int H, int W, int nstrip, int nslots,
-                                                     int rows_per_slot, int total_rows) {
+                                                     int rows_per_slot, int total_rows, int bsplit) {
 #if GF2_PAIRED
   __shared__ u32x4 hbuf[2][NQ / 2][NW + 2][64];
 #else
@@ -500,20 +500,20 @@
     step(std::integral_constant<int, 5>{}, itb);
   }
   __syncthreads();
-  }
-
 #pragma unroll
   for (int m = 32; m >= 1; m >>= 1) vmax = fmaxf(vmax, __shfl_xor(vmax, m));
-  if (l == 0 && !(vmax < 65000.f)) atomicOr(flag, 1u);
+  if (l == 0 && !(vmax < 65000.f)) atomicOr(flag + (b >= bsplit ? 1 : 0), 1u);
+  vmax = 0.f;
+  }
 }
 
 extern const int kStripOut = SO, kThreads = 64 * NW;
 
 #if GF2_NW < 12
-template __global__ void gf2_kernel<0>(const float*, const float*, const float*, float*, unsigned*, int, int, int, int, int, int, int);
-template __global__ void gf2_kernel<1>(const float*, const float*, const float*, float*, unsigned*, int, int, int, int, int, int, int);
-#endif
-template __global__ void gf2_kernel<2>(const float*, const float*, const float*, float*, unsigned*, int, int, int, int, int, int, int);
-template __global__ void gf2_kernel<3>(const float*, const float*, const float*, float*, unsigned*, int, int, int, int, int, int, int);
-
-}
+template __global__ void gf2_kernel<0>(const float*, const float*, const float*, float*, unsigned*, int, int, int, int, int, int, int, int);
+template __global__ void gf2_kernel<1>(const float*, const float*, const float*, float*, unsigned*, int, int, int, int, int, int, int, int);
+#endif
+template __global__ void gf2_kernel<2>(const float*, const float*, const float*, float*, unsigned*, int, int, int, int, int, int, int, int);
+template __global__ void gf2_kernel<3>(const float*, const float*, const float*, float*, unsigned*, int, int, int, int, int, int, int, int);
+
+}
diff --git a/paif_amd/csrc/guided_filter.hip b/paif_amd/csrc/guided_filter.hip
--- a/paif_amd/csrc/guided_filter.hip
+++ b/paif_amd/csrc/guided_filter.hip
@@ -211,7 +211,7 @@
   __shared__ float sG[GH][GH + 1];
   __shared__ float sH[GH][GT + 1], sH2[GH][GT + 1];
   int t = blockIdx.x;
-  if (t == 0 && threadIdx.x == 0) *flag = 0u;
+  if (t == 0 && threadIdx.x < 2) flag[threadIdx.x] = 0u;
   const int tx = t % tilesX; t /= tilesX;
   const int ty = t % tilesY;
   const int b = t / tilesY;
@@ -278,13 +278,13 @@
 template <typename V, int NL>
 __global__ __launch_bounds__(FC * NL) void gf_fused_kernel(const float* __restrict__ guide, const float* __restrict__ y,
                                                            const float* __restrict__ gs, const unsigned* __restrict__ only_if, float* __restrict__ lf,
-                                                           int B, int H, int W, int nstrip, int nseg, int frows, int out_bf16) {
+                                                           int B, int H, int W, int nstrip, int nseg, int frows, int out_bf16, int bsplit) {
   constexpr int VW = VecOps<V>::VW;
   const bool y_f16 = out_bf16 == 3;
   if (y_f16) out_bf16 = 2;
   const unsigned short* const y16 = reinterpret_cast<const unsigned short*>(y) + (blockIdx.z * NL + threadIdx.x % NL) * VW;
   unsigned short* const lf16 = reinterpret_cast<unsigned short*>(lf);
-  if (only_if != nullptr && *only_if == 0u) return;
+  if (only_if != nullptr && only_if[(int)(blockIdx.x / (unsigned)(nstrip * nseg)) >= bsplit ? 1 : 0] == 0u) return;
   __shared__ V s_a[2][FC][NL];
   __shared__ V s_b[2][FC][NL];
   const int xi = threadIdx.x / NL;
@@ -442,20 +442,20 @@
 namespace paif_gf2 {
 template <int OM>
 __global__ void gf2_kernel(const float* __restrict__ guide, const float* __restrict__ y, const float* __restrict__ planes, float* __restrict__ lf,
-                           unsigned* __restrict__ flag, int B, int H, int W, int nstrip, int nslots, int rows_per_slot, int total_rows);
+                           unsigned* __restrict__ flag, int B, int H, int W, int nstrip, int nslots, int rows_per_slot, int total_rows, int bsplit);
 extern const int kStripOut, kThreads;
-extern template __global__ void gf2_kernel<0>(const float*, const float*, const float*, float*, unsigned*, int, int, int, int, int, int, int);
-extern template __global__ void gf2_kernel<1>(const float*, const float*, const float*, float*, unsigned*, int, int, int, int, int, int, int);
-extern template __global__ void gf2_kernel<2>(const float*, const float*, const float*, float*, unsigned*, int, int, int, int, int, int, int);
-extern template __global__ void gf2_kernel<3>(const float*, const float*, const float*, float*, unsigned*, int, int, int, int, int, int, int);
+extern template __global__ void gf2_kernel<0>(const float*, const float*, const float*, float*, unsigned*, int, int, int, int, int, int, int, int);
+extern template __global__ void gf2_kernel<1>(const float*, const float*, const float*, float*, unsigned*, int, int, int, int, int, int, int, int);
+extern template __global__ void gf2_kernel<2>(const float*, const float*, const float*, float*, unsigned*, int, int, int, int, int, int, int, int);
+extern template __global__ void gf2_kernel<3>(const float*, const float*, const float*, float*, unsigned*, int, int, int, int, int, int, int, int);
 }
 namespace paif_gf2w12 {
 template <int OM>
 __global__ void gf2_kernel(const float* __restrict__ guide, const float* __restrict__ y, const float* __restrict__ planes, float* __restrict__ lf,
-                           unsigned* __restrict__ flag, int B, int H, int W, int nstrip, int nslots, int rows_per_slot, int total_rows);
+                           unsigned* __restrict__ flag, int B, int H, int W, int nstrip, int nslots, int rows_per_slot, int total_rows, int bsplit);
 extern const int kStripOut, kThreads;
-extern template __global__ void gf2_kernel<2>(const float*, const float*, const float*, float*, unsigned*, int, int, int, int, int, int, int);
-extern template __global__ void gf2_kernel<3>(const float*, const float*, const float*, float*, unsigned*, int, int, int, int, int, int, int);
+extern template __global__ void gf2_kernel<2>(const float*, const float*, const float*, float*, unsigned*, int, int, int, int, int, int, int, int);
+extern template __global__ void gf2_kernel<3>(const float*, const float*, const float*, float*, unsigned*, int, int, int, int, int, int, int, int);
 }
 
 extern "C" __attribute__((visibility("hidden"))) int paifi_gf_guide_stats(const float* guide, float* workspace, float eps0, float eps1, int B,
@@ -471,8 +471,9 @@
 extern "C" size_t paif_guided_filter_fused_workspace_floats(int B, int H, int W) { return (size_t)4 * B * H * W + 64; }
 
 static int gf_fused_launch(const float* guide, const float* y, float* lf, float eps0, float eps1, float* workspace, int B, int H, int W,
-                           int out_bf16, paif_stream_t stream) {
+                           int out_bf16, paif_stream_t stream, int bsplit = -1) {
   PAIF_REQUIRE(guide && y && lf && workspace && B > 0, PAIF_EINVAL, "guided_filter_fused: bad arguments");
+  if (bsplit < 0) bsplit = B;
   PAIF_REQUIRE(H > 2 * R + 1 && W > 2 * R + 1, PAIF_EINVAL, "guided_filter: H,W must exceed 2r+1 = %d (got %dx%d)", K, H, W);
   const int nstrip = (W + FO - 1) / FO;
   const char* eng = getenv("PAIF_GF_ENGINE");
@@ -503,7 +504,7 @@
     nseg = 1;
     for (int n = 1; n <= 16 && n <= H; ++n) {
       const int rows = (H + n - 1) / n;
-      const long blocks = (long)B * nstrip * n * 2 * zg;
+      const long blocks = (long)bsplit * nstrip * n * 2 * zg;
       const long cost = ((blocks + 256 * res - 1) / (256 * res)) * (rows + warm);
       if (best < 0 || cost < best) { best = cost; nseg = n; }
     }
@@ -521,22 +522,22 @@
     const int grid = (nslots + 7) / 8 * 16;
     if (w12 && out_bf16 == 3)
       hipLaunchKernelGGL((paif_gf2w12::gf2_kernel<3>), dim3(grid), dim3(threads2), 0, st, guide, y, workspace, lf, flag, B, H, W, nstrip2, nslots,
-                         rows_per_slot, (int)total_rows);
+                         rows_per_slot, (int)total_rows, bsplit);
     else if (w12)
       hipLaunchKernelGGL((paif_gf2w12::gf2_kernel<2>), dim3(grid), dim3(threads2), 0, st, guide, y, workspace, lf, flag, B, H, W, nstrip2, nslots,
-                         rows_per_slot, (int)total_rows);
+                         rows_per_slot, (int)total_rows, bsplit);
     else if (out_bf16 == 3)
       hipLaunchKernelGGL((paif_gf2::gf2_kernel<3>), dim3(grid), dim3(threads2), 0, st, guide, y, workspace, lf, flag, B, H, W, nstrip2, nslots,
-                         rows_per_slot, (int)total_rows);
+                         rows_per_slot, (int)total_rows, bsplit);
     else if (out_bf16 == 2)
       hipLaunchKernelGGL((paif_gf2::gf2_kernel<2>), dim3(grid), dim3(threads2), 0, st, guide, y, workspace, lf, flag, B, H, W, nstrip2, nslots,
-                         rows_per_slot, (int)total_rows);
+                         rows_per_slot, (int)total_rows, bsplit);
     else if (out_bf16)
       hipLaunchKernelGGL((paif_gf2::gf2_kernel<1>), dim3(grid), dim3(threads2), 0, st, guide, y, workspace, lf, flag, B, H, W, nstrip2, nslots,
-                         rows_per_slot, (int)total_rows);
+                         rows_per_slot, (int)total_rows, bsplit);
     else
       hipLaunchKernelGGL((paif_gf2::gf2_kernel<0>), dim3(grid), dim3(threads2), 0, st, guide, y, workspace, lf, flag, B, H, W, nstrip2, nslots,
-                         rows_per_slot, (int)total_rows);
+                         rows_per_slot, (int)total_rows, bsplit);
     PAIF_LAUNCH_CHECK("guided_filter_fused(mfma2)");
   }
   int nseg;
@@ -544,10 +545,10 @@
   const int frows = (H + nseg - 1) / nseg;
   const unsigned* only_if = engine == 2 ? flag : nullptr;
   const dim3 grid(B * nstrip * nseg, 2, zgroups);
-  if (form == 0) hipLaunchKernelGGL((gf_fused_kernel<float4, 8>), grid, dim3(FC * 8), 0, st, guide, y, workspace, only_if, lf, B, H, W, nstrip, nseg, frows, out_bf16);
-  else if (form == 1) hipLaunchKernelGGL((gf_fused_kernel<float4, 4>), grid, dim3(FC * 4), 0, st, guide, y, workspace, only_if, lf, B, H, W, nstrip, nseg, frows, out_bf16);
-  else if (form == 2) hipLaunchKernelGGL((gf_fused_kernel<float4, 2>), grid, dim3(FC * 2), 0, st, guide, y, workspace, only_if, lf, B, H, W, nstrip, nseg, frows, out_bf16);
-  else hipLaunchKernelGGL((gf_fused_kernel<float2, 16>), grid, dim3(FC * 16), 0, st, guide, y, workspace, only_if, lf, B, H, W, nstrip, nseg, frows, out_bf16);
+  if (form == 0) hipLaunchKernelGGL((gf_fused_kernel<float4, 8>), grid, dim3(FC * 8), 0, st, guide, y, workspace, only_if, lf, B, H, W, nstrip, nseg, frows, out_bf16, bsplit);
+  else if (form == 1) hipLaunchKernelGGL((gf_fused_kernel<float4, 4>), grid, dim3(FC * 4), 0, st, guide, y, workspace, only_if, lf, B, H, W, nstrip, nseg, frows, out_bf16, bsplit);
+  else if (form == 2) hipLaunchKernelGGL((gf_fused_kernel<float4, 2>), grid, dim3(FC * 2), 0, st, guide, y, workspace, only_if, lf, B, H, W, nstrip, nseg, frows, out_bf16, bsplit);
+  else hipLaunchKernelGGL((gf_fused_kernel<float2, 16>), grid, dim3(FC * 16), 0, st, guide, y, workspace, only_if, lf, B, H, W, nstrip, nseg, frows, out_bf16, bsplit);
   PAIF_LAUNCH_CHECK("guided_filter_fused");
   return 0;
 }
@@ -571,3 +572,17 @@
                                                  int H, int W, paif_stream_t stream) {
   return gf_fused_launch(guide, y, lf, eps0, eps1, workspace, B, H, W, 1, stream);
 }
+
+extern "C" int paif_guided_filter_fused_joint_fits(int B, int H, int W) {
+  if (B < 2 || H <= 2 * R + 1 || W <= 2 * R + 1) return 0;
+  const int so = paif_gf2::kStripOut < paif_gf2w12::kStripOut ? paif_gf2::kStripOut : paif_gf2w12::kStripOut;
+  const size_t ns = (size_t)(W + so - 1) / so;
+  return ((size_t)(B + 1) * H * W * 128 < 0x7FF00000ull && (size_t)B * ns * H < 0x7FFFFFFFull) ? 1 : 0;
+}
+
+extern "C" int paif_guided_filter_fused_fwd_joint(const float* guide, const float* y, float* out, float eps0, float eps1, float* workspace,
+                                                  int B, int bsplit, int H, int W, int out_mode, paif_stream_t stream) {
+  PAIF_REQUIRE(out_mode >= 0 && out_mode <= 3 && bsplit > 0 && B == 2 * bsplit, PAIF_EINVAL,
+               "guided_filter_fused_joint: out_mode %d / bsplit %d of %d images (two problems of bsplit images each)", out_mode, bsplit, B);
+  return gf_fused_launch(guide, y, out, eps0, eps1, workspace, B, H, W, out_mode, stream, bsplit);
+}
diff --git a/paif_amd/operations_m.py b/paif_amd/operations_m.py
--- a/paif_amd/operations_m.py
+++ b/paif_amd/operations_m.py
@@ -208,6 +208,15 @@
         out, z3 = ops.conv2d([x, x1, x2], self.conv3.wpk(3, 32), k, d, alpha=0.333333, res=(x,) + tuple(res), want_aux=True, **kw)
         tape.append(dict(x1=x1, x2=x2, z3=z3))
         return out
+
+    @staticmethod
+    def forward_pair_nhwc(b0, x0, b1, x1):
+        k0 = dict(kh=3, dil=1, act=ops.ACT_PRELU, prelu=b0.lrelu.weight)
+        k1 = dict(kh=3, dil=1, act=ops.ACT_PRELU, prelu=b1.lrelu.weight)
+        y0, y1 = ops.conv2d_pair(dict(srcs=[x0], wpk=b0.conv1.wpk(1, 32), **k0), dict(srcs=[x1], wpk=b1.conv1.wpk(1, 32), **k1))
+        z0, z1 = ops.conv2d_pair(dict(srcs=[x0, y0], wpk=b0.conv2.wpk(2, 32), **k0), dict(srcs=[x1, y1], wpk=b1.conv2.wpk(2, 32), **k1))
+        return ops.conv2d_pair(dict(srcs=[x0, y0, z0], wpk=b0.conv3.wpk(3, 32), alpha=0.333333, res=(x0,), **k0),
+                               dict(srcs=[x1, y1, z1], wpk=b1.conv3.wpk(3, 32), alpha=0.333333, res=(x1,), **k1))
 
     bwd_takes_res = True
 
diff --git a/paif_amd/ops.py b/paif_amd/ops.py
--- a/paif_amd/ops.py
+++ b/paif_amd/ops.py
@@ -28,6 +28,7 @@
 
 CONFIG = {"conv_precision": "bf16x3", "gemm_precision": _env_gemm_precision(), "serpentine": True, "attack_precision": "bf16x6", "storage": "f32",
           "two_stream": False,
+          "stream_pair": True,
           "cpool_fused": True, "f16_last_f32": True, "f16_decomp_split": False,
           "gf_in_f16": os.environ.get("PAIF_GF_IN_F16", "0") == "1",
           "rdb_fused": False, "gemm2": False, "timer_torch_events": os.environ.get("PAIF_TIMER_TORCH_EVENTS", "0") == "1", "infer_f16x3": os.environ.get("PAIF_INFER_F16X3", "1") != "0", "wgrad_f16x3": os.environ.get("PAIF_WGRAD_F16X3", "1") != "0", "_wgrad_scale": None, "gemm_split_min_m": 2048, "f16x3_min_k": int(os.environ.get("PAIF_F16X3_MIN_K", "32")), "attack_bwd_f16x3": _env_switch("PAIF_ATTACK_BWD_F16X3"),
@@ -484,15 +485,20 @@
     return out
 
 
+def _plane_view(img):
+    B, _, H, W = img.shape
+    if img.dtype != torch.float32 or not img.is_cuda:
+        raise RuntimeError("stem: need a float32 CUDA tensor")
+    if img.stride(3) != 1 or img.stride(2) != W:
+        img = img.contiguous()
+    return img, (img.stride(0) if B > 1 else H * W)
+
+
 def stem(img, w, prelu, want_guide=True):
     B, _, H, W = img.shape
-    if img.stride(3) != 1 or img.stride(2) != W:
-        img = img.contiguous()
-    bstride = img.stride(0) if B > 1 else H * W
+    img, bstride = _plane_view(img)
     feat = None if (_ACT_BF16[0] is torch.float16 and CONFIG["gf_in_f16"]) else torch.empty((B, H, W, 32), device=img.device, dtype=torch.float32)
     guide = torch.empty((B, H, W), device=img.device, dtype=torch.float32) if want_guide else None
-    if img.dtype != torch.float32 or not img.is_cuda:
-        raise RuntimeError("stem: need a float32 CUDA tensor")
     if _ACT_BF16[0] is torch.float16 and CONFIG["gf_in_f16"]:
         twin = torch.empty((B, H, W, 32), device=img.device, dtype=torch.float16)
         _lib.check(lib().paif_stem_fwd_twin_f16(ctypes.c_void_p(img.data_ptr()), bstride, _p(w), _p(prelu), None, _pa(twin), _p(guide),
@@ -510,6 +516,36 @@
     return feat, guide
 
 
+def pair_halves(joint, B):
+    return joint[:B], joint[B:]
+
+
+def register_twin_halves(feat, twin, B):
+    halves = pair_halves(feat, B)
+    for h, t in zip(halves, pair_halves(twin, B)):
+        _TWINS[h.data_ptr()] = (h, t)
+    return halves
+
+
+def stem_pair(img0, w0, prelu0, img1, w1, prelu1):
+    if img0.shape != img1.shape:
+        raise ValueError("stem_pair: the two images differ in shape: %s / %s" % (tuple(img0.shape), tuple(img1.shape)))
+    B, _, H, W = img0.shape
+    img0, bs0 = _plane_view(img0)
+    img1, bs1 = _plane_view(img1)
+    dev, st = img0.device, _ACT_BF16[0]
+    only16 = st is torch.float16 and CONFIG["gf_in_f16"]
+    feat = None if only16 else torch.empty((2 * B, H, W, 32), device=dev, dtype=torch.float32)
+    twin = torch.empty((2 * B, H, W, 32), device=dev, dtype=st) if st else None
+    guide = torch.empty((2 * B, H, W), device=dev, dtype=torch.float32)
+    _lib.check(lib().paif_stem_fwd_pair(ctypes.c_void_p(img0.data_ptr()), bs0, _p(w0), _p(prelu0), ctypes.c_void_p(img1.data_ptr()), bs1,
+                                        _p(w1), _p(prelu1), _p(feat), _pa(twin), 0 if twin is None else 2 if st is torch.float16 else 1,
+                                        _p(guide), B, H, W, _stream()), "stem_pair")
+    if only16:
+        return twin, guide, pair_halves(twin, B)
+    return feat, guide, (register_twin_halves(feat, twin, B) if twin is not None else pair_halves(feat, B))
+
+
 def channel_residue(x):
     B, H, W, C = x.shape
     assert C == 32
@@ -525,7 +561,11 @@
         self.mc, self.stats = mc, stats
 
 
-def guided_filter_pair(guide, y, eps=(0.001, 0.0001), want_ab=False, out_bf16=False, tape=None):
+def guided_filter_joint_fits(B2, H, W):
+    return H > 9 and W > 9 and bool(lib().paif_guided_filter_fused_joint_fits(B2, H, W))
+
+
+def guided_filter_pair(guide, y, eps=(0.001, 0.0001), want_ab=False, out_bf16=False, tape=None, bsplit=None):
     hf16 = out_bf16 is torch.float16
     out_bf16 = bool(out_bf16)
     B, H, W, C = y.shape
@@ -544,11 +584,16 @@
             raise NotImplementedError("guided filter: an fp16 target map is built for the fp16 configuration's high-frequency output only")
         fn = (L.paif_guided_filter_fused_fwd_hf16_y16 if y16 else L.paif_guided_filter_fused_fwd_hf16 if hf16 else
               L.paif_guided_filter_fused_fwd_bf16 if out_bf16 else L.paif_guided_filter_fused_fwd)
-        _lib.check(fn(_p(guide), _pa(y) if y16 else _p(y), _pa(lf), eps[0], eps[1], _p(ws), B, H, W, _stream()), "guided_filter_fused")
+        if bsplit is not None:
+            _lib.check(L.paif_guided_filter_fused_fwd_joint(_p(guide), _pa(y) if y16 else _p(y), _pa(lf), eps[0], eps[1], _p(ws), B, bsplit, H, W,
+                                                            3 if y16 else 2 if hf16 else 1 if out_bf16 else 0, _stream()), "guided_filter_fused")
+        else:
+            _lib.check(fn(_p(guide), _pa(y) if y16 else _p(y), _pa(lf), eps[0], eps[1], _p(ws), B, H, W, _stream()), "guided_filter_fused")
         if e0 is not None:
             TIMER.stop(tag, e0, 650 * B * H * W * 32, B * H * W * (4 + (2 if y16 else 4) * 32 + (2 if out_bf16 else 4) * 64))
         return lf
     assert not out_bf16, "bf16 low-frequency maps are an inference (fused-form) output"
+    assert bsplit is None, "the joint batch of two problems is an inference (fused-form) call"
     lf = torch.empty((2, B, H, W, 32), device=y.device, dtype=torch.float32)
     import os
     assert tape in (None, "mc", "ab"), tape
@@ -692,9 +737,44 @@
     return buf.value.decode()
 
 
+def _launch_convs(pend):
+    L = lib()
+    if len(pend) == 2 and pend[0][1] == pend[1][1] and CONFIG.get("stream_pair", True):
+        (d0, (B, H, W), w0, _), (d1, _, w1, _) = pend
+        buf = ctypes.create_string_buffer(96)
+        if L.paif_conv2d_pair_kernel_name(ctypes.byref(d0), ctypes.byref(d1), B, H, W, buf, len(buf)) == 0:
+            tag = buf.value.decode()
+            e0 = TIMER.start(tag) if TIMER is not None else None
+            _lib.check(L.paif_conv2d_fwd_pair(ctypes.byref(d0), ctypes.byref(d1), B, H, W, _stream()), "conv2d_pair")
+            if e0 is not None:
+                TIMER.stop(tag, e0, w0[0] + w1[0], w0[1] + w1[1], w0[2] + w1[2])
+            return True
+    for d, (B, H, W), work, _ in pend:
+        e0 = None
+        if TIMER is not None:
+            tag = conv2d_kernel_name(d, B, H, W)
+            e0 = TIMER.start(tag)
+        _lib.check(L.paif_conv2d_fwd(ctypes.byref(d), B, H, W, _stream()), "conv2d")
+        if e0 is not None:
+            TIMER.stop(tag, e0, *work)
+    return False
+
+
+def conv2d_pair(kw0, kw1):
+    pend = []
+    o0 = conv2d(_defer=pend, **kw0)
+    n0 = len(pend)
+    o1 = conv2d(_defer=pend, **kw1)
+    if n0 == 1 and len(pend) == 2:
+        _launch_convs(pend)
+    elif pend:
+        _launch_convs(pend)
+    return o0, o1
+
+
 def conv2d(srcs, wpk, kh, dil=1, cin=32, cout=32, in_act=ACT_NONE, in_prelu=None, scale=None, shift=None,
            act=ACT_NONE, prelu=None, alpha=1.0, res=(), pool=False, want_aux=False, in_aux=None, in_scale=None,
-           in_alpha=1.0, epi_dact=0, epi_aux=None, out=None, out_f32=False, cpool=None):
+           in_alpha=1.0, epi_dact=0, epi_aux=None, out=None, out_f32=False, cpool=None, _defer=None):
     B, H, W, C = srcs[0].shape
     assert C == cin and 1 <= len(srcs) <= 3
     res = [r for r in res if r is not None]
@@ -768,16 +848,14 @@
     if CONFIG.get("serpentine", True):
         _SERP[0] ^= 1
         d.reverse_tiles = _SERP[0]
-    e0 = None
-    if TIMER is not None:
-        tag = conv2d_kernel_name(d, B, H, W)
-        e0 = TIMER.start(tag)
-    _lib.check(L.paif_conv2d_fwd(ctypes.byref(d), B, H, W, _stream()), "conv2d")
-    if e0 is not None:
-        px = B * H * W
-        eb_in, eb_out = (2 if src_bf else 4), (2 if out_bf else 4)
-        eb_res = 2 if (res and res[0].dtype in H16) else 4
-        TIMER.stop(tag, e0, 2 * px * kh * kh * cin * len(srcs) * cout, px * (eb_in * cin * len(srcs) + eb_out * cout), px * eb_res * cout * len(res))
+    px = B * H * W
+    eb_in, eb_out = (2 if src_bf else 4), (2 if out_bf else 4)
+    eb_res = 2 if (res and res[0].dtype in H16) else 4
+    work = (2 * px * kh * kh * cin * len(srcs) * cout, px * (eb_in * cin * len(srcs) + eb_out * cout), px * eb_res * cout * len(res))
+    if _defer is not None and not extra and pool_after is None and not pool and not want_aux:
+        _defer.append((d, (B, H, W), work, (srcs, res, out, wpk, scale, shift, prelu, in_prelu)))
+        return out
+    _launch_convs([(d, (B, H, W), work, None)])
     for r in extra:
         out = add(out, r)
     if pool_after is not None:
```

Result: faster. 2753, median of 6 (+2.4%).
